# DeepNeuralAI313/Arabic-text-image-generation-RepText

Measured on AMD Instinct MI355X. Metric: images/sec (whole node), FLUX.1-dev+RepText CN, 1024^2, 28 steps, higher is better.
Workload: dtype bf16; 1 GPU; FLUX.1-dev (19+38 blocks) + RepText ControlNet (6+0), 1024x1024, 28 steps, 1 text line(s), batch 1/GPU on rank 0, denoise loop + VAE decode to uint8, random-init weights; tower blocks evaluated 5 of 6 (the last sample is never read, Q5); global_batch=1, conditioning=one prompt, hint and mask per image, parallelism=batch-shard x1, one broadcast

## Files before the change

### arabic-text-image-generation-reptext_amd/controlnet.py

```python
from __future__ import annotations

from dataclasses import dataclass
from typing import Any, Dict, List, Optional, Sequence, Tuple, Union

import torch
import torch.nn as nn

from . import mmdit, ops
from .config import Config
from .modules import Lin
from .ops import LinearProblem as P
from .transformer import StaticEmbeds, _MMDiTBase


@dataclass
class FluxControlNetOutput:
    controlnet_block_samples: Optional[List[torch.Tensor]]
    controlnet_single_block_samples: Optional[List[torch.Tensor]]

    def __iter__(self):
        yield self.controlnet_block_samples
        yield self.controlnet_single_block_samples


class FluxControlNetModel(_MMDiTBase):
    _supports_gradient_checkpointing = False

    def __init__(self, patch_size: int = 1, in_channels: int = 64, num_layers: int = 19, num_single_layers: int = 38,
                 attention_head_dim: int = 128, num_attention_heads: int = 24, joint_attention_dim: int = 4096,
                 pooled_projection_dim: int = 768, guidance_embeds: bool = False, axes_dims_rope=(16, 56, 56),
                 num_mode: Optional[int] = None, extra_conditioning_channels: int = 0, extra_condition_channels: int = 0,
                 device=None, dtype=None):
        super().__init__()
        self.config = Config(patch_size=patch_size, in_channels=in_channels, num_layers=num_layers,
                             num_single_layers=num_single_layers, attention_head_dim=attention_head_dim,
                             num_attention_heads=num_attention_heads, joint_attention_dim=joint_attention_dim,
                             pooled_projection_dim=pooled_projection_dim, guidance_embeds=guidance_embeds,
                             axes_dims_rope=list(axes_dims_rope), num_mode=num_mode,
                             extra_conditioning_channels=extra_conditioning_channels,
                             extra_condition_channels=extra_condition_channels)
        self.out_channels = in_channels
        self._build_trunk(self.config, device, dtype)
        d = self.inner_dim
        kw = dict(device=device, dtype=dtype)
        self.controlnet_blocks = nn.ModuleList([Lin(d, d, **kw) for _ in range(num_layers)])
        self.controlnet_single_blocks = nn.ModuleList([Lin(d, d, **kw) for _ in range(num_single_layers)])
        self.union = num_mode is not None
        if self.union:
            self.controlnet_mode_embedder = nn.Embedding(num_mode, d, **kw)
        self.controlnet_x_embedder = Lin(in_channels + extra_condition_channels, d, **kw)
        self.gradient_checkpointing = False

    def zero_init_controlnet_(self):
        for m in list(self.controlnet_blocks) + list(self.controlnet_single_blocks) + [self.controlnet_x_embedder]:
            m.weight.data.zero_()
            m.bias.data.zero_()
        return self

    @property
    def attn_processors(self) -> Dict[str, Any]:
        names = [f"transformer_blocks.{i}.attn.processor" for i in range(len(self.transformer_blocks))]
        names += [f"single_transformer_blocks.{i}.attn.processor" for i in range(len(self.single_transformer_blocks))]
        return {n: "HipFlashAttention" for n in names}

    def set_attn_processor(self, processor):
        count = len(self.attn_processors)
        if isinstance(processor, dict) and len(processor) != count:
            raise ValueError(
                f"A dict of processors was passed, but the number of processors {len(processor)} does not match the"
                f" number of attention layers: {count}. Please make sure to pass {count} processor classes.")
        raise NotImplementedError("the MI355X path has a single fused attention kernel; custom processors are not supported")

    @classmethod
    def from_transformer(cls, transformer, num_layers: int = 4, num_single_layers: int = 10, attention_head_dim: int = 128,
                         num_attention_heads: int = 24, extra_condition_channels: int = 0,
                         load_weights_from_transformer: bool = True):
        cfg = dict(transformer.config)
        cfg.pop("out_channels", None)
        cfg.update(num_layers=num_layers, num_single_layers=num_single_layers, attention_head_dim=attention_head_dim,
                   num_attention_heads=num_attention_heads, extra_condition_channels=extra_condition_channels)
        cn = cls(**cfg, device=transformer.device, dtype=transformer.dtype)
        if load_weights_from_transformer:
            src = transformer.state_dict()
            own = cn.state_dict()
            for k in own:
                if k in src and own[k].shape == src[k].shape:
                    own[k].copy_(src[k])
        cn.zero_init_controlnet_()
        return cn

    def _padded_hint(self, cond: torch.Tensor):
        cxw = self.controlnet_x_embedder.weight.data
        kin = cxw.shape[1]
        if kin % 64 == 0:
            return cond, cxw
        kp = (kin + 63) // 64 * 64
        if getattr(self, "_cx_pad", None) is None or self._cx_pad.device != cxw.device:
            wpad = torch.zeros(cxw.shape[0], kp, device=cxw.device, dtype=cxw.dtype)
            wpad[:, :kin] = cxw
            self._cx_pad = wpad
        return torch.nn.functional.pad(cond, (0, kp - kin)), self._cx_pad

    def _lora_unsupported(self, path: str, lin):
        why = super()._lora_unsupported(path, lin)
        if why is None and lin is self.controlnet_x_embedder and lin.in_features % 64:
            why = f"in-features {lin.in_features} are not a multiple of 64: the K-padded copy of _padded_hint would go stale"
        return why

    def _invalidate_derived(self):
        self._cx_pad = None

    def load_state_dict(self, sd, strict: bool = True, **kw):
        out = super().load_state_dict(sd, strict=strict, **kw)
        self._invalidate_derived()
        return out

    def random_init_(self, *a, **k):
        out = super().random_init_(*a, **k)
        self._invalidate_derived()
        return out

    def _apply(self, fn, *a, **k):
        self._invalidate_derived()
        return super()._apply(fn, *a, **k)

    @torch.no_grad()
    def forward(self, hidden_states: torch.Tensor, controlnet_cond: torch.Tensor, controlnet_mode: torch.Tensor = None,
                conditioning_scale: float = 1.0, encoder_hidden_states: torch.Tensor = None,
                pooled_projections: torch.Tensor = None, timestep: torch.Tensor = None, img_ids: torch.Tensor = None,
                txt_ids: torch.Tensor = None, guidance: torch.Tensor = None,
                joint_attention_kwargs: Optional[Dict[str, Any]] = None, return_dict: bool = True,
                _rowscale: Optional[torch.Tensor] = None, _accumulate_into: Optional[Sequence[torch.Tensor]] = None,
                _accumulate_single_into: Optional[Sequence[torch.Tensor]] = None, _mods: Optional["mmdit.StepMods"] = None,
                _overwrite: bool = False, _sample_events: Optional[Sequence["torch.cuda.Event"]] = None, _ws_tag: str = "",
                _static: Optional[StaticEmbeds] = None, _blocks_needed: Optional[Tuple[int, int]] = None):
        doubles, singles = self._ensure_plans()
        self._apply_lora_scale(joint_attention_kwargs)
        cfg = self.config
        if self.union:
            if controlnet_mode is None:
                raise ValueError("`controlnet_mode` cannot be `None` when applying ControlNet-Union")
            raise NotImplementedError("ControlNet-Union mode embedding is outside the RepText hot path (SURVEY.md §2 #11)")
        B, N, _ = hidden_states.shape
        Bc, T, _ = encoder_hidden_states.shape
        H, d = cfg.num_attention_heads, self.inner_dim
        ws = mmdit.workspace(Bc, T, N, d, hidden_states.device, need_single=len(singles) > 0, tag=_ws_tag)
        hs = hidden_states.to(torch.bfloat16)
        if hs.shape[0] != Bc:
            hs = hs.expand(Bc, -1, -1) if hs.shape[0] == 1 else hs.repeat(Bc // hs.shape[0], 1, 1)
        x_i, x_t = ws.x[:, T:], ws.x[:, :T]
        if _static is not None:
            x_t.copy_(_static.ctx)
            ops.linear(hs.contiguous(), self.x_embedder.weight.data, x_i, bias=self.x_embedder.bias.data, res=_static.hint)
        else:
            cond = controlnet_cond.to(torch.bfloat16)
            if cond.shape[0] != Bc:
                cond = cond.expand(Bc, -1, -1) if cond.shape[0] == 1 else cond.repeat(Bc // cond.shape[0], 1, 1)
            ops.linear_grouped([P(hs.contiguous(), self.x_embedder.weight.data, x_i, bias=self.x_embedder.bias.data),
                                P(encoder_hidden_states.to(torch.bfloat16).contiguous(), self.context_embedder.weight.data, x_t,
                                  bias=self.context_embedder.bias.data)])
            cond, cxw = self._padded_hint(cond)
            ops.linear(cond.contiguous(), cxw, x_i, bias=self.controlnet_x_embedder.bias.data, res=x_i)
        temb = None if _mods is not None else self._temb(ws, timestep, guidance, pooled_projections)
        cos, sin = self._rope(txt_ids, img_ids)

        scale = float(conditioning_scale)

        def head(lin, dst_list, i):
            a = mmdit.image_rows_bf16(ws)
            if dst_list is not None:
                out = dst_list[i]
                ops.linear(a, lin.weight.data, out, bias=lin.bias.data, alpha=scale, rowscale=_rowscale, res=None if _overwrite else out)
            else:
                out = torch.empty(Bc, N, d, device=hs.device, dtype=torch.bfloat16)
                ops.linear(a, lin.weight.data, out, bias=lin.bias.data, alpha=scale, rowscale=_rowscale)
            return out

        nd = len(doubles) if _blocks_needed is None else min(len(doubles), int(_blocks_needed[0]))
        ns = len(singles) if _blocks_needed is None else min(len(singles), int(_blocks_needed[1]))
        if ns > 0:
            nd = len(doubles)
        block_samples: List[Optional[torch.Tensor]] = []
        for i, pl in enumerate(doubles):
            if i >= nd:
                block_samples.append(None)
                continue
            mmdit.run_double(pl, ws, temb, cos, sin, H, mods=None if _mods is None else _mods.double[i])
            block_samples.append(head(self.controlnet_blocks[i], _accumulate_into, i))
            if _sample_events is not None:
                _sample_events[i].record(torch.cuda.current_stream())
        single_samples: List[Optional[torch.Tensor]] = []
        for i, pl in enumerate(singles):
            if i >= ns:
                single_samples.append(None)
                continue
            mmdit.run_single(pl, ws, temb, cos, sin, H, mods=None if _mods is None else _mods.single[i])
            single_samples.append(head(self.controlnet_single_blocks[i], _accumulate_single_into, i))

        bs = block_samples if block_samples else None
        ss = single_samples if single_samples else None
        if not return_dict:
            return (bs, ss)
        return FluxControlNetOutput(controlnet_block_samples=bs, controlnet_single_block_samples=ss)


class FluxMultiControlNetModel(nn.Module):

    def __init__(self, controlnets, union: bool = False):
        super().__init__()
        self.nets = nn.ModuleList(controlnets)
        self.union = union

    @torch.no_grad()
    def forward(self, hidden_states, controlnet_cond, controlnet_mode, conditioning_scale, encoder_hidden_states=None,
                pooled_projections=None, timestep=None, img_ids=None, txt_ids=None, guidance=None,
                joint_attention_kwargs=None, return_dict: bool = True):
        nets = [self.nets[0]] * len(controlnet_cond) if len(self.nets) == 1 else list(self.nets)
        total_b = total_s = None
        for net, image, mode, scale in zip(nets, controlnet_cond, controlnet_mode, conditioning_scale):
            b, s = net(hidden_states=hidden_states, controlnet_cond=image, controlnet_mode=None if mode is None else mode[:, None],
                       conditioning_scale=scale, timestep=timestep, guidance=guidance, pooled_projections=pooled_projections,
                       encoder_hidden_states=encoder_hidden_states, txt_ids=txt_ids, img_ids=img_ids,
                       joint_attention_kwargs=joint_attention_kwargs, return_dict=False)
            if total_b is None and total_s is None:
                total_b, total_s = b, s
                continue
            if b is not None and total_b is not None:
                for acc, t in zip(total_b, b):
                    ops.masked_accumulate_(acc, t, None, 1.0, True)
            if s is not None and total_s is not None:
                for acc, t in zip(total_s, s):
                    ops.masked_accumulate_(acc, t, None, 1.0, True)
        return total_b, total_s
```

### arabic-text-image-generation-reptext_amd/csrc/attention.hip

```cpp
#include "attention_split.h"
#include <cstdlib>
#include <type_traits>

namespace {

constexpr int DH = 128;
constexpr int BQ = 128;
constexpr int BKV = 64;
constexpr int TILE_B = BKV * DH * 2;
constexpr int ATT_THREADS = 256;
constexpr float RESCALE_THR = 6.0f;
constexpr int REC_WAVE_B = 64 * 64 * 4 + 64 * 8;
constexpr int REC_B = 4 * REC_WAVE_B;

__host__ __device__ inline int group_slots(const SplitGeom& G, int xcd) {
  const GroupCut c = group_cut(G, xcd);
  return c.nfull + (c.rem ? G.spx : 0);
}

__global__ __launch_bounds__(ATT_THREADS, 2) void attention_fwd_kernel(
    const bf16_t* __restrict__ Q, const bf16_t* __restrict__ K, const bf16_t* __restrict__ V, bf16_t* O,
    int64_t ld, int64_t stride_b, int64_t ldo, int64_t stride_ob, float scale_log2, const SplitGeom G,
    int* counters, char* records) {
  __shared__ __attribute__((aligned(16))) char smem[4 * TILE_B];
  const int tid = threadIdx.x;
  const int lane = tid & 63;
  const int wave = __builtin_amdgcn_readfirstlane(tid >> 6);
  const int l31 = lane & 31, hh = lane >> 5;
  const int S = G.S;
  const int ntiles = G.ntiles;

  const int xcd = (int)blockIdx.x & 7, slot = (int)blockIdx.x >> 3, b = (int)blockIdx.y;
  const GroupCut cut = group_cut(G, xcd);
  int run_lo, run_hi;
  int item0;
  int jpart = -1;
  if (slot < cut.nfull) {
    item0 = cut.start + slot;
    run_lo = 0;
    run_hi = ntiles;
  } else {
    jpart = slot - cut.nfull;
    if (cut.rem == 0 || jpart >= G.spx) return;
    const SplitRun run = split_run(G, cut, jpart);
    item0 = cut.start + cut.nfull + run.i0;
    run_lo = run.lo - run.i0 * ntiles;
    run_hi = run.hi - run.i0 * ntiles;
  }

  const int srow = lane >> 4;
  const int spc = lane & 15;
  uint32_t soff[4];
#pragma unroll
  for (int p = 0; p < 4; ++p) {
    const int row_t = (wave * 4 + p) * 4 + srow;
    soff[p] = ((uint32_t)row_t * (uint32_t)ld + (uint32_t)((spc ^ swz(row_t)) << 3)) * 2u;
  }
  lds_cptr kp[8];
  {
    const int ksw = swz(l31);
#pragma unroll
    for (int ks = 0; ks < 8; ++ks) kp[ks] = (lds_cptr)smem + (l31 * 256 + (((2 * ks + hh) ^ ksw) << 4));
  }
  const int tq = (lane >> 2) & 3, tp = lane & 3;
  const int tg1 = (lane >> 4) & 1;
  lds_cptr vp[2][4];
  {
    const int cl = tg1 * 2 + (tp >> 1);
    const int rl0 = 4 * hh + tq, rl1 = rl0 + 8;
#pragma unroll
    for (int dt = 0; dt < 4; ++dt) {
      vp[0][dt] = (lds_cptr)smem + TILE_B + rl0 * 256 + (((dt * 4 + cl) ^ swz(rl0)) << 4) + 8 * (tp & 1);
      vp[1][dt] = (lds_cptr)smem + TILE_B + rl1 * 256 + (((dt * 4 + cl) ^ swz(rl1)) << 4) + 8 * (tp & 1);
    }
  }

  using S0 = std::integral_constant<int, 0>;
  using S1 = std::integral_constant<int, 1>;

  for (int seg = 0; seg < 2; ++seg) {
    const int item = item0 + seg;
    const int tb = seg == 0 ? run_lo : 0;
    const int te = seg == 0 ? min(run_hi, ntiles) : run_hi - ntiles;
    if (te <= tb) break;
    const int head = item / G.nqb;
    const int q0 = (item - head * G.nqb) * BQ;
    const bf16_t* Qb = Q + b * stride_b + head * DH;
    const bf16_t* Kb = K + b * stride_b + head * DH;
    const bf16_t* Vb = V + b * stride_b + head * DH;

    const rt_srd_t rsrcK = rt_make_srd(Kb), rsrcV = rt_make_srd(Vb);
    const uint32_t lds0 = (uint32_t)(uintptr_t)LDS_PTR(smem);
    const int tile_stride_b = BKV * (int)ld * 2;
    auto stage = [&](int sl, int tix, bool clamp) {
      const uint32_t kb = lds0 + sl * 2 * TILE_B;
      if (RT_RARE(clamp)) {
        const int kv0 = tix * BKV;
#pragma unroll
        for (int p = 0; p < 4; ++p) {
          const int row_t = (wave * 4 + p) * 4 + srow;
          const uint32_t off = ((uint32_t)(min(kv0 + row_t, S - 1) - kv0) * (uint32_t)ld + (uint32_t)((spc ^ swz(row_t)) << 3)) * 2u;
          rt_dma16_asm(rsrcK, kb + (wave * 4 + p) * 1024, off, (uint32_t)(tix * tile_stride_b));
          rt_dma16_asm(rsrcV, kb + TILE_B + (wave * 4 + p) * 1024, off, (uint32_t)(tix * tile_stride_b));
        }
      } else {
#pragma unroll
        for (int p = 0; p < 4; ++p) {
          rt_dma16_asm(rsrcK, kb + (wave * 4 + p) * 1024, soff[p], (uint32_t)(tix * tile_stride_b));
          rt_dma16_asm(rsrcV, kb + TILE_B + (wave * 4 + p) * 1024, soff[p], (uint32_t)(tix * tile_stride_b));
        }
      }
    };

    __syncthreads();
    stage(0, tb, (tb + 1) * BKV > S);

    bf16x8 qf[8];
    {
      const int qrow = min(q0 + wave * 32 + l31, S - 1);
      const bf16_t* qp = Qb + (int64_t)qrow * ld + 8 * hh;
#pragma unroll
      for (int ks = 0; ks < 8; ++ks) qf[ks] = *reinterpret_cast<const bf16x8*>(qp + ks * 16);
#pragma unroll
      for (int ks = 0; ks < 8; ++ks) asm volatile("" : "+v"(qf[ks]));
    }

    f32x16 o_acc[4];
#pragma unroll
    for (int i = 0; i < 4; ++i)
#pragma unroll
      for (int r = 0; r < 16; ++r) o_acc[i][r] = 0.f;
    float m_run = -INFINITY, l_run = 0.f;

    auto half_max = [&](const f32x16& s) -> float {
      float ma = max3f(s[0], s[1], s[2]), mb = max3f(s[3], s[4], s[5]);
      ma = max3f(ma, s[6], s[7]);
      mb = max3f(mb, s[8], s[9]);
      ma = max3f(ma, s[10], s[11]);
      mb = max3f(mb, s[12], s[13]);
      return fmaxf(max3f(ma, s[14], s[15]), mb);
    };
    auto decide = [&](float mx, bool& pend) -> float {
      unsigned xa = __builtin_bit_cast(unsigned, mx), xb = xa;
      asm volatile("s_nop 1\n\tv_permlane32_swap_b32 %0, %1" : "+v"(xa), "+v"(xb));
      const float mxr = fmaxf(__builtin_bit_cast(float, xa), __builtin_bit_cast(float, xb)) * scale_log2;
      float alpha = 1.f;
      pend = false;
      if (RT_RARE(__any(mxr - m_run > RESCALE_THR))) {
        asm volatile("" ::: "memory");
        const float m_new = fmaxf(m_run, mxr);
        alpha = __builtin_amdgcn_exp2f(m_run - m_new);
        m_run = m_new;
        l_run *= alpha;
        pend = true;
      }
      return alpha;
    };
    auto rescale_o = [&](float alpha) __attribute__((always_inline)) {
#pragma unroll
      for (int i = 0; i < 4; ++i)
#pragma unroll
        for (int r = 0; r < 16; ++r) o_acc[i][r] *= alpha;
    };
    auto numer8 = [&](const f32x16& s, int s2, bf16x8& pf) {
      float ps = 0.f;
#pragma unroll
      for (int j = 0; j < 8; ++j) {
        const float p = __builtin_amdgcn_exp2f(__builtin_fmaf(s[8 * s2 + j], scale_log2, -m_run));
        ps += p;
        pf[j] = (__bf16)p;
      }
      l_run += ps;
    };

#define RT_WEAVE(n, nds, nva)                                          \
  _Pragma("unroll") for (int w_ = 0; w_ < (n); ++w_) {                 \
    __builtin_amdgcn_sched_group_barrier(0x008, 1, 0);                 \
    if ((nds) > 0) __builtin_amdgcn_sched_group_barrier(0x100, (nds), 0); \
    if ((nva) > 0) __builtin_amdgcn_sched_group_barrier(0x402, (nva), 0); \
  }

    auto tile = [&](auto slot_c, int t) {
      constexpr int SLOT = decltype(slot_c)::value;
      constexpr int SB = SLOT * 2 * TILE_B;
      const bool ragged = (t + 1) * BKV > S;
      auto kread = [&](int h, int ks) -> bf16x8 {
        return *(const __attribute__((address_space(3))) bf16x8*)(kp[ks] + SB + h * 8192); };
      auto vread = [&](int h, int s2, int dt) -> bf16x8 {
        const s16x4 lo = tr_read(vp[0][dt] + SB + h * 8192 + s2 * 4096);
        const s16x4 hi = tr_read(vp[1][dt] + SB + h * 8192 + s2 * 4096);
        return __builtin_shufflevector(__builtin_bit_cast(bf16x4, lo), __builtin_bit_cast(bf16x4, hi), 0, 1, 2, 3, 4, 5, 6, 7);
      };
      auto mask_half = [&](f32x16& s, int h) {
#pragma unroll
        for (int r = 0; r < 16; ++r)
          if (t * BKV + 32 * h + (r & 3) + 8 * (r >> 2) + 4 * hh >= S) s[r] = -INFINITY;
      };
      rt_dma_barrier();
      f32x16 s0, s1;
#pragma unroll
      for (int r = 0; r < 16; ++r) { s0[r] = 0.f; s1[r] = 0.f; }
      bf16x8 kA[8], kB[8], vA[4], vB[4];
      bf16x8 p00, p01, p10, p11;
      bool pend;
#pragma unroll
      for (int ks = 0; ks < 8; ++ks) kA[ks] = kread(0, ks);
      const bool next_ragged = (t + 2) * BKV > S;
      if (RT_RARE(t + 1 < te && next_ragged)) stage(SLOT ^ 1, t + 1, true);
      const bool weave = t + 1 < te && !next_ragged;
      {
        const uint32_t nb = lds0 + (SLOT ^ 1) * 2 * TILE_B, so = (uint32_t)((t + 1) * tile_stride_b);
#pragma unroll
        for (int ks = 0; ks < 8; ++ks) {
          s0 = __builtin_amdgcn_mfma_f32_32x32x16_bf16(kA[ks], qf[ks], s0, 0, 0, 0);
          if (RT_USUAL(weave)) rt_dma16_asm((ks & 1) ? rsrcV : rsrcK, nb + ((ks & 1) ? TILE_B : 0) + (wave * 4 + (ks >> 1)) * 1024, soff[ks >> 1], so);
          if (ks >= 4 && ks < 7) kB[ks - 4] = kread(1, ks - 4);
          RT_SB();
        }
      }
#pragma unroll
      for (int ks = 0; ks < 3; ++ks) s1 = __builtin_amdgcn_mfma_f32_32x32x16_bf16(kB[ks], qf[ks], s1, 0, 0, 0);
#pragma unroll
      for (int ks = 3; ks < 8; ++ks) kB[ks] = kread(1, ks);
      if (RT_RARE(ragged)) mask_half(s0, 0);
      float mx0 = half_max(s0);
      __builtin_amdgcn_sched_group_barrier(0x008, 1, 0);
      __builtin_amdgcn_sched_group_barrier(0x100, 3, 0);
      __builtin_amdgcn_sched_group_barrier(0x008, 1, 0);
      __builtin_amdgcn_sched_group_barrier(0x100, 2, 0);
      __builtin_amdgcn_sched_group_barrier(0x008, 1, 0);
      RT_SB();
      {
        const float alpha = decide(mx0, pend);
        if (RT_RARE(pend)) rescale_o(alpha);
      }
      RT_SB();
#pragma unroll
      for (int ks = 3; ks < 8; ++ks) s1 = __builtin_amdgcn_mfma_f32_32x32x16_bf16(kB[ks], qf[ks], s1, 0, 0, 0);
#pragma unroll
      for (int dt = 0; dt < 4; ++dt) vA[dt] = vread(0, 0, dt);
      numer8(s0, 0, p00);
      RT_WEAVE(5, 2, 6)
      RT_PIN(p00); RT_PIN(l_run);
      RT_SB();
#pragma unroll
      for (int dt = 0; dt < 4; ++dt) o_acc[dt] = __builtin_amdgcn_mfma_f32_32x32x16_bf16(vA[dt], p00, o_acc[dt], 0, 0, 0);
#pragma unroll
      for (int dt = 0; dt < 4; ++dt) vB[dt] = vread(0, 1, dt);
      numer8(s0, 1, p01);
      if (RT_RARE(ragged)) mask_half(s1, 1);
      float mx1 = half_max(s1);
      RT_WEAVE(4, 2, 9)
      RT_PIN(p01); RT_PIN(l_run); RT_PIN(mx1);
      RT_SB();
      const float alpha1 = decide(mx1, pend);
      RT_SB();
#pragma unroll
      for (int dt = 0; dt < 4; ++dt) o_acc[dt] = __builtin_amdgcn_mfma_f32_32x32x16_bf16(vB[dt], p01, o_acc[dt], 0, 0, 0);
#pragma unroll
      for (int dt = 0; dt < 4; ++dt) vA[dt] = vread(1, 0, dt);
      numer8(s1, 0, p10);
      RT_WEAVE(4, 2, 7)
      RT_PIN(p10); RT_PIN(l_run);
      RT_SB();
      if (RT_RARE(pend)) rescale_o(alpha1);
      RT_SB();
#pragma unroll
      for (int dt = 0; dt < 4; ++dt) o_acc[dt] = __builtin_amdgcn_mfma_f32_32x32x16_bf16(vA[dt], p10, o_acc[dt], 0, 0, 0);
#pragma unroll
      for (int dt = 0; dt < 4; ++dt) vB[dt] = vread(1, 1, dt);
      numer8(s1, 1, p11);
      RT_WEAVE(4, 2, 7)
      RT_PIN(p11); RT_PIN(l_run);
      RT_SB();
#pragma unroll
      for (int dt = 0; dt < 4; ++dt) o_acc[dt] = __builtin_amdgcn_mfma_f32_32x32x16_bf16(vB[dt], p11, o_acc[dt], 0, 0, 0);
    };

    int t = tb;
    for (; t + 1 < te; t += 2) {
      tile(S0{}, t);
      tile(S1{}, t + 1);
    }
    if (t < te) tile(S0{}, t);

    const int qrow = q0 + wave * 32 + l31;
    const bool whole = (tb == 0 && te == ntiles);
    if (!whole) {
      const int ritem = item - (cut.start + cut.nfull);
      char* rec = records + split_rec_index(G, b, xcd, jpart, seg) * (int64_t)REC_B + wave * REC_WAVE_B;
      const __amdgpu_buffer_rsrc_t rs = __builtin_amdgcn_make_buffer_rsrc(rec, 0, REC_WAVE_B, 0x00020000);
#pragma unroll
      for (int i = 0; i < 4; ++i)
#pragma unroll
        for (int g = 0; g < 4; ++g) {
          const f32x4 vv = {o_acc[i][4 * g + 0], o_acc[i][4 * g + 1], o_acc[i][4 * g + 2], o_acc[i][4 * g + 3]};
          const u32x4 w = __builtin_bit_cast(u32x4, vv);
          __builtin_amdgcn_raw_buffer_store_b128(w, rs, (i * 4 + g) * 1024 + lane * 16, 0, 16 );
        }
      {
        const float2 mlf = {m_run, l_run};
        const u32x2 ml = __builtin_bit_cast(u32x2, mlf);
        __builtin_amdgcn_raw_buffer_store_b64(ml, rs, 16384 + lane * 8, 0, 16);
      }
      int* cnt = counters + (int64_t)b * G.NI + item;
      const SplitParts parts = split_parts(G, cut, ritem);
      const bool last = split_ticket(cnt, parts.nparts, reinterpret_cast<volatile int*>(smem), tid);
      if (last) {
        auto rec_of = [&](int j) -> const char* {
          return records + split_rec_index(G, b, xcd, j, split_seg_of(G, parts, j)) * (int64_t)REC_B + wave * REC_WAVE_B;
        };
        float M = -INFINITY;
        for (int j = parts.j_first; j <= parts.j_last; ++j) {
          const char* rj = rec_of(__builtin_amdgcn_readfirstlane(j));
          M = fmaxf(M, *reinterpret_cast<const float*>(rj + 16384 + lane * 8));
        }
        float L = 0.f;
#pragma unroll
        for (int i = 0; i < 4; ++i)
#pragma unroll
          for (int r = 0; r < 16; ++r) o_acc[i][r] = 0.f;
        for (int j = parts.j_first; j <= parts.j_last; ++j) {
          const char* rj = rec_of(__builtin_amdgcn_readfirstlane(j));
          const float2 ml = *reinterpret_cast<const float2*>(rj + 16384 + lane * 8);
          const float wgt = __builtin_amdgcn_exp2f(ml.x - M);
          L = __builtin_fmaf(ml.y, wgt, L);
#pragma unroll
          for (int i = 0; i < 4; ++i)
#pragma unroll
            for (int g = 0; g < 4; ++g) {
              const f32x4 v = *reinterpret_cast<const f32x4*>(rj + (i * 4 + g) * 1024 + lane * 16);
#pragma unroll
              for (int e = 0; e < 4; ++e) o_acc[i][4 * g + e] = __builtin_fmaf(v[e], wgt, o_acc[i][4 * g + e]);
            }
        }
        l_run = L;
      }
      if (!last) continue;
    }

    const float l_tot = l_run + __shfl_xor(l_run, 32);
    const float inv = 1.0f / l_tot;
    const bool wide = (ldo % 8 == 0) && (stride_ob % 8 == 0) && ((reinterpret_cast<uintptr_t>(O) & 15) == 0);
    if (wide) {
      rt_store_o_rows(O + b * stride_ob + (int64_t)min(qrow, S - 1) * ldo + head * DH, qrow < S, hh, o_acc, inv);
    } else if (qrow < S) {
      bf16_t* op = O + b * stride_ob + (int64_t)qrow * ldo + head * DH + 4 * hh;
#pragma unroll
      for (int dt = 0; dt < 4; ++dt)
#pragma unroll
        for (int g = 0; g < 4; ++g) {
          u32x2 w;
          w[0] = pack_bf16x2(o_acc[dt][4 * g + 0] * inv, o_acc[dt][4 * g + 1] * inv);
          w[1] = pack_bf16x2(o_acc[dt][4 * g + 2] * inv, o_acc[dt][4 * g + 3] * inv);
          *reinterpret_cast<u32x2*>(op + dt * 32 + 8 * g) = w;
        }
    }
  }
}

int g_slots_per_xcd = 0;

int slots_per_xcd() {
  if (g_slots_per_xcd == 0) {
    const char* e = getenv("RT_ATTN_SLOTS_PER_XCD");
    g_slots_per_xcd = e ? atoi(e) : (split_cu_count() / 8) * 2;
    if (g_slots_per_xcd < 1) g_slots_per_xcd = 1;
  }
  return g_slots_per_xcd;
}

SplitGeom make_geom(int S, int H, bool want_split) { return split_geom(S, H, BQ, BKV, slots_per_xcd(), want_split); }

}

extern "C" int64_t rt_attention_ws_bytes(int32_t B, int32_t S, int32_t H) {
  if (B < 1 || S < 1 || H < 1) return 0;
  static const bool off = getenv("RT_ATTN_SPLIT") && getenv("RT_ATTN_SPLIT")[0] == '0';
  if (off) return 0;
  const int64_t need3 = rt_attention_v3_ws_bytes(B, S, H);
  const int64_t need = split_ws_bytes(B, make_geom(S, H, true), REC_B);
  return need > need3 ? need : need3;
}

extern "C" int rt_attention_variant(int32_t mode) { return rt_attention_v3_mode(mode); }

extern "C" int rt_attention_fwd(const void* q, const void* k, const void* v, void* o, int64_t ld, int64_t stride_b,
                                int64_t ldo, int64_t stride_ob, int32_t B, int32_t S, int32_t H, float scale,
                                void* ws, int64_t ws_bytes, void* stream) {
  if (!q || !k || !v || !o || B < 1 || S < 1 || H < 1) return RT_E_BADARG;
  if (!RT_ALIGNED(q, 16) || !RT_ALIGNED(k, 16) || !RT_ALIGNED(v, 16) || !RT_ALIGNED(o, 8) || ld % 8 || stride_b % 8 ||
      ldo % 4 || stride_ob % 4)
    return RT_E_ALIGN;
  if (ld < (int64_t)H * DH || ldo < (int64_t)H * DH) return RT_E_SHAPE;
  if ((int64_t)(S + BKV) * ld * 2 >= (int64_t)1 << 31) return RT_E_SHAPE;
  if (!split_fits_32bit(make_geom(S, H, true))) return RT_E_SHAPE;
  {
    int taken = 0;
    const int st = rt_attention_v3_try(q, k, v, o, ld, stride_b, ldo, stride_ob, B, S, H, scale, ws, ws_bytes, stream, &taken);
    if (taken || st != RT_OK) return st;
  }
  const int64_t need = rt_attention_ws_bytes(B, S, H);
  const bool split = ws != nullptr && need > 0;
  if (split && (ws_bytes < need || !RT_ALIGNED(ws, 256))) return RT_E_BADARG;
  const SplitGeom G = make_geom(S, H, split);
  int wmax = 0;
  for (int x = 0; x < 8; ++x) wmax = group_slots(G, x) > wmax ? group_slots(G, x) : wmax;
  const dim3 grid(8 * wmax, B);
  hipLaunchKernelGGL(attention_fwd_kernel, grid, dim3(ATT_THREADS), 0, (hipStream_t)stream, (const bf16_t*)q,
                     (const bf16_t*)k, (const bf16_t*)v, (bf16_t*)o, ld, stride_b, ldo, stride_ob,
                     scale * 1.4426950408889634f, G, split ? (int*)ws : nullptr,
                     split ? (char*)ws + split_cnt_bytes(B, S, H) : nullptr);
  return rt_hip_status();
}
```

### arabic-text-image-generation-reptext_amd/csrc/attention_split.h

```cpp
#pragma once
#include "rt_common.h"

constexpr int CNT_ALIGN = 256;
constexpr int SPLIT_MIN_TILES = 8;

struct SplitGeom {
  int S, H, nqb, ntiles, NI;
  int spx;
  int split;
};

struct GroupCut {
  int start, cnt;
  int nfull;
  int rem;
};
__host__ __device__ inline GroupCut group_cut(const SplitGeom& G, int xcd) {
  GroupCut c;
  const int base = G.NI >> 3, extra = G.NI & 7;
  c.cnt = base + (xcd < extra ? 1 : 0);
  c.start = xcd * base + (xcd < extra ? xcd : extra);
  c.nfull = c.cnt;
  c.rem = 0;
  if (G.split) {
    const int nf = (c.cnt / G.spx) * G.spx, rem = c.cnt - nf;
    if (rem > 0 && rem * 16 < G.spx * 15 && (int64_t)rem * G.ntiles >= (int64_t)G.spx * SPLIT_MIN_TILES) {
      c.nfull = nf;
      c.rem = rem;
    }
  }
  return c;
}

struct SplitRun { int lo, hi, i0; };
__device__ __forceinline__ SplitRun split_run(const SplitGeom& G, const GroupCut& cut, int j) {
  const unsigned U = (unsigned)cut.rem * (unsigned)G.ntiles;
  SplitRun r;
  r.lo = (int)((unsigned)j * U / (unsigned)G.spx);
  r.hi = (int)((unsigned)(j + 1) * U / (unsigned)G.spx);
  r.i0 = r.lo / G.ntiles;
  return r;
}

struct SplitParts {
  unsigned U, a;
  int j_first, j_last, nparts;
};
__device__ __forceinline__ SplitParts split_parts(const SplitGeom& G, const GroupCut& cut, int ritem) {
  const unsigned U = (unsigned)cut.rem * (unsigned)G.ntiles, spx = (unsigned)G.spx;
  const unsigned a = (unsigned)ritem * (unsigned)G.ntiles, bnd = a + (unsigned)G.ntiles;
  SplitParts p;
  p.U = U;
  p.a = a;
  p.j_first = (int)(((a + 1) * spx + U - 1) / U) - 1;
  p.j_last = min(G.spx - 1, (int)((bnd * spx + U - 1) / U) - 1);
  p.nparts = p.j_last - p.j_first + 1;
  return p;
}
__device__ __forceinline__ int split_seg_of(const SplitGeom& G, const SplitParts& p, int j) {
  const unsigned lo_j = (unsigned)j * p.U / (unsigned)G.spx;
  return (p.a > lo_j) ? 1 : 0;
}
__device__ __forceinline__ int64_t split_rec_index(const SplitGeom& G, int b, int xcd, int j, int seg) {
  return (((int64_t)b * 8 + xcd) * G.spx + j) * 2 + seg;
}

__device__ __forceinline__ bool split_ticket(int* cnt, int nparts, volatile int* flag, int tid) {
  asm volatile("s_waitcnt vmcnt(0)" ::: "memory");
  __syncthreads();
  if (tid == 0) {
    const int old = __hip_atomic_fetch_add(cnt, 1, __ATOMIC_RELAXED, __HIP_MEMORY_SCOPE_AGENT);
    const int last = (old == nparts - 1) ? 1 : 0;
    if (last) {
      __hip_atomic_store(cnt, 0, __ATOMIC_RELAXED, __HIP_MEMORY_SCOPE_AGENT);
      __builtin_amdgcn_fence(__ATOMIC_ACQUIRE, "agent");
      asm volatile("s_waitcnt vmcnt(0)" ::: "memory");
    }
    *flag = last;
  }
  __syncthreads();
  return __builtin_amdgcn_readfirstlane(*flag) != 0;
}

inline int split_cu_count() {
  int dev = 0, cus = 256;
  if (hipGetDevice(&dev) == hipSuccess) {
    int v = 0;
    if (hipDeviceGetAttribute(&v, hipDeviceAttributeMultiprocessorCount, dev) == hipSuccess && v > 0) cus = v;
  }
  return cus;
}
inline SplitGeom split_geom(int S, int H, int bq, int bkv, int spx, bool split) {
  const int nqb = (S + bq - 1) / bq;
  return SplitGeom{S, H, nqb, (S + bkv - 1) / bkv, H * nqb, spx > 0 ? spx : 1, split ? 1 : 0};
}
inline bool split_fits_32bit(const SplitGeom& G) { return (int64_t)G.NI * (G.ntiles + 1) * G.spx < ((int64_t)1 << 31); }
inline bool split_any(const SplitGeom& G) {
  bool any = false;
  for (int x = 0; x < 8; ++x) any = any || group_cut(G, x).rem > 0;
  return any;
}
inline int64_t split_cnt_bytes(int B, int S, int H) {
  return (((int64_t)B * H * ((S + 127) / 128) * 4 + CNT_ALIGN - 1) / CNT_ALIGN) * CNT_ALIGN;
}
inline int64_t split_ws_bytes(int B, const SplitGeom& G, int64_t rec_bytes) {
  if (!split_any(G)) return 0;
  return split_cnt_bytes(B, G.S, G.H) + (int64_t)B * 8 * G.spx * 2 * rec_bytes;
}

int64_t rt_attention_v3_ws_bytes(int32_t B, int32_t S, int32_t H);
int rt_attention_v3_try(const void* q, const void* k, const void* v, void* o, int64_t ld, int64_t stride_b, int64_t ldo, int64_t stride_ob,
                        int32_t B, int32_t S, int32_t H, float scale, void* ws, int64_t ws_bytes, void* stream, int* taken);
int rt_attention_v3_mode(int mode);
```

### arabic-text-image-generation-reptext_amd/csrc/attention_v3.hip

```cpp
#include "attention_split.h"
#include <cstdlib>
#include <type_traits>

namespace {

constexpr int DH = 128;
constexpr int BQ3 = 256;
constexpr int BKV = 64;
constexpr int TILE_B = BKV * DH * 2;
constexpr int STAGE_B = 2 * TILE_B;
constexpr int NSTAGE = 3;
constexpr int V3_THREADS = 256;
constexpr float RESCALE_THR = 6.0f;

#include "attention_v3_regs.h"
#define V3_EACH8(M) M(0) M(1) M(2) M(3) M(4) M(5) M(6) M(7)
#define V3_EACH10(M) V3_EACH8(M) M(8) M(9)
#define V3_EACH16(M) M(0) M(1) M(2) M(3) M(4) M(5) M(6) M(7) M(8) M(9) M(10) M(11) M(12) M(13) M(14) M(15)
__device__ __forceinline__ void mfma_o(int f, const bf16x8& v, const bf16x8& p) {
  switch (f) {
#define V3_C(F) case F: asm volatile("v_mfma_f32_32x32x16_bf16 " V3_OREG_##F ", %0, %1, " V3_OREG_##F ::"v"(v), "v"(p) : V3_ALL_CL); break;
    V3_EACH8(V3_C)
#undef V3_C
  }
}
__device__ __forceinline__ void mfma_l(int qb, const bf16x8& p) {
  if (qb) asm volatile("v_mfma_f32_32x32x16_bf16 " V3_OREG_9 ", " V3_ONES_REG ", %0, " V3_OREG_9 ::"v"(p) : V3_ALL_CL);
  else asm volatile("v_mfma_f32_32x32x16_bf16 " V3_OREG_8 ", " V3_ONES_REG ", %0, " V3_OREG_8 ::"v"(p) : V3_ALL_CL);
}
__device__ __forceinline__ void ones_write() {
  asm volatile("v_accvgpr_write_b32 a224, %0\n\tv_accvgpr_write_b32 a225, %0\n\tv_accvgpr_write_b32 a226, %0\n\tv_accvgpr_write_b32 a227, %0" ::"v"(0x3F803F80u) : V3_ALL_CL);
}
__device__ __forceinline__ void mfma_s0(f32x16& c, const bf16x8& k, int i) {
  switch (i) {
#define V3_C(I) case I: asm volatile("v_mfma_f32_32x32x16_bf16 %0, %1, " V3_QREG_##I ", 0" : "=&v"(c) : "v"(k) : V3_ALL_CL); break;
    V3_EACH16(V3_C)
#undef V3_C
  }
}
__device__ __forceinline__ void mfma_s(f32x16& c, const bf16x8& k, int i) {
  switch (i) {
#define V3_C(I) case I: asm volatile("v_mfma_f32_32x32x16_bf16 %0, %1, " V3_QREG_##I ", %0" : "+v"(c) : "v"(k) : V3_ALL_CL); break;
    V3_EACH16(V3_C)
#undef V3_C
  }
}
__device__ __forceinline__ void q_write(int i, const bf16x8& q) {
  const u32x4 w = __builtin_bit_cast(u32x4, q);
  switch (i) {
#define V3_C(I) case I: asm volatile(V3_QWRITE_##I ::"v"(w[0]), "v"(w[1]), "v"(w[2]), "v"(w[3]) : V3_ALL_CL); break;
    V3_EACH16(V3_C)
#undef V3_C
  }
}
__device__ __forceinline__ void o_zero(int f) {
  switch (f) {
#define V3_C(F) case F: asm volatile(V3_OZERO_##F ::: V3_ALL_CL); break;
    V3_EACH10(V3_C)
#undef V3_C
  }
}
__device__ __forceinline__ void o_scale(int f, float alpha) {
  float tmp;
  switch (f) {
#define V3_C(F) case F: asm volatile(V3_OSCALE_##F : "=&v"(tmp) : "v"(alpha) : V3_ALL_CL); break;
    V3_EACH10(V3_C)
#undef V3_C
  }
}
__device__ __forceinline__ f32x16 o_read(int f) {
  float x0, x1, x2, x3, x4, x5, x6, x7, x8, x9, x10, x11, x12, x13, x14, x15;
  switch (f) {
#define V3_C(F) case F: asm volatile(V3_OREAD_##F : "=v"(x0), "=v"(x1), "=v"(x2), "=v"(x3), "=v"(x4), "=v"(x5), "=v"(x6), "=v"(x7), "=v"(x8), "=v"(x9), "=v"(x10), "=v"(x11), "=v"(x12), "=v"(x13), "=v"(x14), "=v"(x15) : : V3_ALL_CL); break;
    V3_EACH10(V3_C)
#undef V3_C
  }
  return f32x16{x0, x1, x2, x3, x4, x5, x6, x7, x8, x9, x10, x11, x12, x13, x14, x15};
}

constexpr int REC3_WAVE_B = 8 * 16 * 64 * 4 + 64 * 16;
constexpr int REC3_B = 4 * REC3_WAVE_B;

__global__ __launch_bounds__(V3_THREADS, 1) void attention_v3_kernel(const bf16_t* __restrict__ Q, const bf16_t* __restrict__ K,
                                                                     const bf16_t* __restrict__ V, bf16_t* O, int64_t ld, int64_t stride_b,
                                                                     int64_t ldo, int64_t stride_ob, float scale_log2, const SplitGeom G,
                                                                     int* counters, char* records) {
  extern __shared__ __attribute__((aligned(16))) char smem[];
  const int tid = threadIdx.x;
  const int lane = tid & 63;
  const int wave = __builtin_amdgcn_readfirstlane(tid >> 6);
  const int l31 = lane & 31, hh = lane >> 5;
  const int ntiles = G.ntiles;
  const int xcd = (int)blockIdx.x & 7, slot = (int)blockIdx.x >> 3, b = (int)blockIdx.y;
  const GroupCut cut = group_cut(G, xcd);
  const uint32_t lds0 = (uint32_t)(uintptr_t)LDS_PTR(smem);

  const int srow = lane >> 4, spc = lane & 15;
  uint32_t soff[4];
#pragma unroll
  for (int p = 0; p < 4; ++p) {
    const int row_t = (wave * 4 + p) * 4 + srow;
    soff[p] = ((uint32_t)row_t * (uint32_t)ld + (uint32_t)((spc ^ swz(row_t)) << 3)) * 2u;
  }
  const int tile_stride_b = BKV * (int)ld * 2;

  const int nwhole = slot < cut.nfull ? (cut.nfull - slot + G.spx - 1) / G.spx : 0;
  SplitRun run = {0, 0, 0};
  if (cut.rem && slot < G.spx) run = split_run(G, cut, slot);
  const int nseg = nwhole + (cut.rem && slot < G.spx ? 2 : 0);

  for (int si = 0; si < nseg; ++si) {
    int item, tb, te, seg = 0;
    if (si < nwhole) {
      item = cut.start + slot + si * G.spx;
      tb = 0;
      te = ntiles;
    } else {
      seg = si - nwhole;
      item = cut.start + cut.nfull + run.i0 + seg;
      tb = seg == 0 ? run.lo - run.i0 * ntiles : 0;
      te = seg == 0 ? min(run.hi - run.i0 * ntiles, ntiles) : run.hi - (run.i0 + 1) * ntiles;
      if (te <= tb) continue;
    }
    const int head = item / G.nqb;
    const int q0 = (item - head * G.nqb) * BQ3;
    const bf16_t* Qb = Q + b * stride_b + head * DH;
    const rt_srd_t rsrcK = rt_make_srd(K + b * stride_b + head * DH), rsrcV = rt_make_srd(V + b * stride_b + head * DH);
    const uint32_t wdst = lds0 + wave * 4096;
    auto dma_piece = [&](int sbase, uint32_t soffs, int i) __attribute__((always_inline)) {
      rt_dma16_asm((i & 4) ? rsrcV : rsrcK, wdst + sbase + ((i & 4) ? TILE_B : 0) + (i & 3) * 1024, soff[i & 3], soffs);
    };

    asm volatile("s_waitcnt vmcnt(0)" ::: "memory");
    __syncthreads();
#pragma unroll
    for (int i = 0; i < 8; ++i) dma_piece(0, (uint32_t)(tb * tile_stride_b), i);
    if (tb + 1 < te) {
#pragma unroll
      for (int i = 0; i < 8; ++i) dma_piece(STAGE_B, (uint32_t)((tb + 1) * tile_stride_b), i);
    }
    {
      const bf16_t* qp = Qb + (int64_t)(q0 + wave * 64 + l31) * ld + 8 * hh;
      bf16x8 qa[8], qb[8];
#pragma unroll
      for (int ks = 0; ks < 8; ++ks) {
        qa[ks] = *reinterpret_cast<const bf16x8*>(qp + ks * 16);
        qb[ks] = *reinterpret_cast<const bf16x8*>(qp + 32 * ld + ks * 16);
      }
#pragma unroll
      for (int ks = 0; ks < 8; ++ks) { q_write(ks, qa[ks]); q_write(8 + ks, qb[ks]); }
#pragma unroll
      for (int f = 0; f < 10; ++f) o_zero(f);
      ones_write();
      asm volatile("s_nop 7" ::: "memory");
    }
    float mA = -INFINITY, mB = -INFINITY;

    f32x16 sAa, sAb, sBa, sBb;
    bf16x8 pA[2][2], pB[2][2];
    bf16x8 kf[8], vf[8];
    float mxa0, mxa1, mxb0, mxb1;
    float tf[2], pp[2];
    int pend1 = -1, pend2 = -1;

    auto elem_f = [&](int o, const f32x16& Sa, const f32x16& Sb) __attribute__((always_inline)) {
      const int ks = o >> 4, qb = (o >> 3) & 1, j = o & 7, r = 8 * ks + j;
      float t = __builtin_fmaf(qb ? Sb[r] : Sa[r], scale_log2, qb ? -mB : -mA);
      asm volatile("" : "+v"(t));
      tf[o & 1] = t;
    };
    auto elem_x = [&](int o) __attribute__((always_inline)) {
      float p = __builtin_amdgcn_exp2f(tf[o & 1]);
      asm volatile("" : "+v"(p));
      pp[o & 1] = p;
    };
    auto elem_c = [&](int o, bf16x8 (&P)[2][2]) __attribute__((always_inline)) {
      const int ks = o >> 4, qb = (o >> 3) & 1, j = o & 7;
      P[qb][ks][j] = (__bf16)pp[o & 1];
      if (j & 1) asm volatile("" : "+v"(P[qb][ks]));
    };
    auto elem = [&](int o, const f32x16& Sa, const f32x16& Sb, bf16x8 (&P)[2][2]) __attribute__((always_inline)) {
      if (pend2 >= 0) elem_c(pend2, P);
      if (pend1 >= 0) elem_x(pend1);
      elem_f(o, Sa, Sb);
      pend2 = pend1;
      pend1 = o;
    };
    auto elem_flush = [&](bf16x8 (&P)[2][2]) __attribute__((always_inline)) {
      if (pend2 >= 0) elem_c(pend2, P);
      if (pend1 >= 0) { elem_x(pend1); elem_c(pend1, P); }
      pend1 = pend2 = -1;
    };
    auto maxstep = [&](int k, const f32x16& s, float& m0, float& m1) __attribute__((always_inline)) {
      if (k == 0) m0 = max3f(s[0], s[1], s[2]);
      else if (k == 1) m1 = max3f(s[3], s[4], s[5]);
      else if (k == 2) m0 = max3f(m0, s[6], s[7]);
      else if (k == 3) m1 = max3f(m1, s[8], s[9]);
      else if (k == 4) m0 = max3f(m0, s[10], s[11]);
      else if (k == 5) m1 = max3f(m1, s[12], s[13]);
      else if (k == 6) m0 = max3f(m0, s[14], s[15]);
      else m0 = fmaxf(m0, m1);
    };
    auto exchange = [&](float mx) __attribute__((always_inline)) -> float {
      unsigned xa = __builtin_bit_cast(unsigned, mx), xb = xa;
      asm volatile("s_nop 1\n\tv_permlane32_swap_b32 %0, %1" : "+v"(xa), "+v"(xb));
      return fmaxf(__builtin_bit_cast(float, xa), __builtin_bit_cast(float, xb)) * scale_log2;
    };
    auto decide = [&](float mxra, float mxrb, const f32x16& Sa, const f32x16& Sb, bf16x8 (&P)[2][2]) __attribute__((always_inline)) {
      if (__builtin_expect(!!__any((mxra - mA > RESCALE_THR) | (mxrb - mB > RESCALE_THR)), 0)) {
        asm volatile("s_nop 15\n\ts_nop 15" ::: "memory");
        const float nA = fmaxf(mA, mxra), nB = fmaxf(mB, mxrb);
        const float alA = __builtin_amdgcn_exp2f(mA - nA), alB = __builtin_amdgcn_exp2f(mB - nB);
        mA = nA; mB = nB;
#pragma unroll
        for (int f = 0; f < 10; ++f) o_scale(f, (f & 1) ? alB : alA);
#pragma unroll
        for (int o = 0; o < 16; ++o) { elem_f(o, Sa, Sb); elem_x(o); elem_c(o, P); }
      }
    };
    int ka[8];
    {
      const int ksw = swz(l31);
  #pragma unroll
      for (int ks = 0; ks < 8; ++ks) ka[ks] = (int)lds0 + l31 * 256 + (((2 * ks + hh) ^ ksw) << 4);
    }
    const int tq = (lane >> 2) & 3, tp = lane & 3, tg1 = (lane >> 4) & 1;
    int va[8];
    {
      const int cl = tg1 * 2 + (tp >> 1);
      const int rl0 = 4 * hh + tq, rl1 = rl0 + 8;
  #pragma unroll
      for (int dt = 0; dt < 4; ++dt) {
        va[dt] = (int)lds0 + TILE_B + rl0 * 256 + (((dt * 4 + cl) ^ swz(rl0)) << 4) + 8 * (tp & 1);
        va[4 + dt] = (int)lds0 + TILE_B + rl1 * 256 + (((dt * 4 + cl) ^ swz(rl1)) << 4) + 8 * (tp & 1);
      }
    }
    auto mov_ka = [&](int i, int delta) __attribute__((always_inline)) { ka[i] += delta; asm volatile("" : "+v"(ka[i])); };
    auto mov_va = [&](int i, int delta) __attribute__((always_inline)) { va[i] += delta; asm volatile("" : "+v"(va[i])); };
    auto kread = [&](int kb, int ks) __attribute__((always_inline)) -> bf16x8 {
      return *(const __attribute__((address_space(3))) bf16x8*)((lds_cptr)(uintptr_t)(uint32_t)(ka[ks] + kb * 8192));
    };
    auto vread = [&](int kb, int s2, int dt) __attribute__((always_inline)) -> bf16x8 {
      const s16x4 lo = tr_read((lds_cptr)(uintptr_t)(uint32_t)(va[dt] + kb * 8192 + s2 * 4096));
      const s16x4 hi = tr_read((lds_cptr)(uintptr_t)(uint32_t)(va[4 + dt] + kb * 8192 + s2 * 4096));
      return __builtin_shufflevector(__builtin_bit_cast(bf16x4, lo), __builtin_bit_cast(bf16x4, hi), 0, 1, 2, 3, 4, 5, 6, 7);
    };
    auto qk_group = [&](f32x16& Sa, f32x16& Sb, auto&& filler) __attribute__((always_inline)) {
      asm volatile("" ::"v"(kf[0]), "v"(kf[1]), "v"(kf[2]), "v"(kf[3]), "v"(kf[4]), "v"(kf[5]), "v"(kf[6]), "v"(kf[7]));
#pragma unroll
      for (int g = 0; g < 16; ++g) {
        const int ks = g >> 1;
        if (g == 0) mfma_s0(Sa, kf[0], 0);
        else if (g == 1) mfma_s0(Sb, kf[0], 8);
        else if (g & 1) mfma_s(Sb, kf[ks], 8 + ks);
        else mfma_s(Sa, kf[ks], ks);
        filler(g);
        RT_SB();
      }
    };
    auto pv_group = [&](bf16x8 (&P)[2][2], auto&& filler) __attribute__((always_inline)) {
      asm volatile("" ::"v"(vf[0]), "v"(vf[1]), "v"(vf[2]), "v"(vf[3]), "v"(vf[4]), "v"(vf[5]), "v"(vf[6]), "v"(vf[7]));
#pragma unroll
      for (int g = 0; g < 20; ++g) {
        const int s2 = g / 10, h = g % 10;
        if (h < 8) mfma_o((h >> 1) * 2 + (h & 1), vf[s2 * 4 + (h >> 1)], P[h & 1][s2]);
        else mfma_l(h & 1, P[h & 1][s2]);
        filler(g);
        RT_SB();
      }
    };
    auto second_half = [&](int g, const f32x16& Sa, const f32x16& Sb, bf16x8 (&P)[2][2], float ra, float rb, float& ea, float& eb)
        __attribute__((always_inline)) {
      if (g == 0) ea = exchange(ra);
      if (g == 1) eb = exchange(rb);
      if (g == 2) decide(ea, eb, Sa, Sb, P);
      if (g >= 3 && g <= 12) elem(13 + g, Sa, Sb, P);
      if (g >= 13) { elem(26 + 2 * (g - 13), Sa, Sb, P); elem(27 + 2 * (g - 13), Sa, Sb, P); }
      if (g == 15) elem_flush(P);
// ... 29 lines not shown
        asm volatile("s_nop 15\n\ts_nop 15" ::: "memory");
        RT_PIN(sAa); RT_PIN(sAb);
#pragma unroll
        for (int g = 0; g < 8; ++g) { maxstep(g, sAa, mxa0, mxa1); maxstep(g, sAb, mxb0, mxb1); }
#pragma unroll
        for (int ks = 0; ks < 8; ++ks) kf[ks] = kread(1, ks);
      }
      rka = mxa0; rkb = mxb0;
      RT_SB();
      qk_group(sBa, sBb, [&](int g) __attribute__((always_inline)) {
        if constexpr (first) {
          if (g == 0) ea = exchange(rka);
          if (g == 1) { eb = exchange(rkb); mA = fmaxf(mA, ea); mB = fmaxf(mB, eb); }
          if (g >= 2) { elem(2 * (g - 2), sAa, sAb, pA); elem(2 * (g - 2) + 1, sAa, sAb, pA); }
          if (g == 14) { elem(28, sAa, sAb, pA); elem(29, sAa, sAb, pA); }
          if (g == 15) { elem(30, sAa, sAb, pA); elem(31, sAa, sAb, pA); elem_flush(pA); }
        } else {
          second_half(g, sAa, sAb, pA, rka, rkb, ea, eb);
        }
        if ((g & 1) == 0) { const int i = g >> 1; vf[(i >> 2) * 4 + (i & 3)] = vread(0, i >> 2, i & 3); } else { mov_ka(g >> 1, sbn - sb); }
      });
      if constexpr (!last) {
        asm volatile("s_waitcnt vmcnt(0)" ::: "memory");
        __builtin_amdgcn_s_barrier();
        RT_SB();
      }
      pv_group(pA, [&](int g) __attribute__((always_inline)) {
        first_half(g, sBa, sBb, pB);
        if constexpr (!last) {
          if (g < 16 && (g & 1)) kf[g >> 1] = kread(0, g >> 1);
          if (g >= 2 && g < 18 && (g & 1) == 0) dma_piece(sbp, so2, (g - 2) >> 1);
        }
      });
      { const int r_ = st_cur; st_cur = st_nxt; st_nxt = st_prv; st_prv = r_; }
      rka = mxa0; rkb = mxb0;
      if constexpr (last) {
        RT_SB();
        const float ea2 = exchange(rka), eb2 = exchange(rkb);
        decide(ea2, eb2, sBa, sBb, pB);
#pragma unroll
        for (int o = 16; o < 32; ++o) elem(o, sBa, sBb, pB);
        elem_flush(pB);
#pragma unroll
        for (int i = 0; i < 8; ++i) vf[(i >> 2) * 4 + (i & 3)] = vread(1, i >> 2, i & 3);
        RT_SB();
        pv_group(pB, [&](int) __attribute__((always_inline)) {});
      }
    };
    using TT = std::true_type;
    using FF = std::false_type;
    __syncthreads();
#pragma unroll
    for (int ks = 0; ks < 8; ++ks) kf[ks] = kread(0, ks);
    if (te - tb == 1) {
      tile(TT{}, TT{}, tb);
    } else {
      tile(TT{}, FF{}, tb);
      for (int t = tb + 1; t + 1 < te; ++t) tile(FF{}, FF{}, t);
      tile(FF{}, TT{}, te - 1);
    }

    asm volatile("s_nop 15\n\ts_nop 15" ::: "memory");
    const bool whole = (tb == 0 && te == ntiles);
    const float lA = o_read(8)[0], lB = o_read(9)[0];
    bf16_t* orow = O + b * stride_ob + (int64_t)(q0 + wave * 64 + l31) * ldo + head * DH;
    if (whole) {
#pragma unroll
      for (int qb = 0; qb < 2; ++qb) {
        f32x16 t4[4];
#pragma unroll
        for (int dt = 0; dt < 4; ++dt) t4[dt] = o_read(dt * 2 + qb);
        rt_store_o_rows(orow + qb * 32 * ldo, true, hh, t4, 1.0f / (qb ? lB : lA));
      }
      continue;
    }
    const int jpart = slot;
    const int ritem = item - (cut.start + cut.nfull);
    {
      char* rec = records + split_rec_index(G, b, xcd, jpart, seg) * (int64_t)REC3_B + wave * REC3_WAVE_B;
      const __amdgpu_buffer_rsrc_t rs = __builtin_amdgcn_make_buffer_rsrc(rec, 0, REC3_WAVE_B, 0x00020000);
#pragma unroll
      for (int f = 0; f < 8; ++f) {
        const f32x16 x = o_read(f);
#pragma unroll
        for (int g = 0; g < 4; ++g) {
          const f32x4 vv = {x[4 * g + 0], x[4 * g + 1], x[4 * g + 2], x[4 * g + 3]};
          __builtin_amdgcn_raw_buffer_store_b128(__builtin_bit_cast(u32x4, vv), rs, (f * 4 + g) * 1024 + lane * 16, 0, 16 );
        }
      }
      const f32x4 ml = {mA, lA, mB, lB};
      __builtin_amdgcn_raw_buffer_store_b128(__builtin_bit_cast(u32x4, ml), rs, 32768 + lane * 16, 0, 16);
    }
    int* cnt = counters + (int64_t)b * G.NI + item;
    const SplitParts parts = split_parts(G, cut, ritem);
    if (!split_ticket(cnt, parts.nparts, reinterpret_cast<volatile int*>(smem), tid)) continue;
    auto rec_of = [&](int j) -> const char* {
      return records + split_rec_index(G, b, xcd, j, split_seg_of(G, parts, j)) * (int64_t)REC3_B + wave * REC3_WAVE_B;
    };
    float MA = -INFINITY, MB = -INFINITY;
    for (int j = parts.j_first; j <= parts.j_last; ++j) {
      const f32x4 ml = *reinterpret_cast<const f32x4*>(rec_of(__builtin_amdgcn_readfirstlane(j)) + 32768 + lane * 16);
      MA = fmaxf(MA, ml[0]);
      MB = fmaxf(MB, ml[2]);
    }
    float LA = 0.f, LB = 0.f;
    for (int j = parts.j_first; j <= parts.j_last; ++j) {
      const f32x4 ml = *reinterpret_cast<const f32x4*>(rec_of(__builtin_amdgcn_readfirstlane(j)) + 32768 + lane * 16);
      LA = __builtin_fmaf(ml[1], __builtin_amdgcn_exp2f(ml[0] - MA), LA);
      LB = __builtin_fmaf(ml[3], __builtin_amdgcn_exp2f(ml[2] - MB), LB);
    }
#pragma unroll
    for (int qb = 0; qb < 2; ++qb) {
      f32x16 t4[4];
#pragma unroll
      for (int dt = 0; dt < 4; ++dt)
#pragma unroll
        for (int r = 0; r < 16; ++r) t4[dt][r] = 0.f;
      for (int j = parts.j_first; j <= parts.j_last; ++j) {
        const char* rj = rec_of(__builtin_amdgcn_readfirstlane(j));
        const f32x4 ml = *reinterpret_cast<const f32x4*>(rj + 32768 + lane * 16);
        const float w = __builtin_amdgcn_exp2f(qb ? ml[2] - MB : ml[0] - MA);
#pragma unroll
        for (int dt = 0; dt < 4; ++dt)
#pragma unroll
          for (int g = 0; g < 4; ++g) {
            const f32x4 v = *reinterpret_cast<const f32x4*>(rj + ((dt * 2 + qb) * 4 + g) * 1024 + lane * 16);
#pragma unroll
            for (int e = 0; e < 4; ++e) t4[dt][4 * g + e] = __builtin_fmaf(v[e], w, t4[dt][4 * g + e]);
          }
      }
      rt_store_o_rows(orow + qb * 32 * ldo, true, hh, t4, 1.0f / (qb ? LB : LA));
    }
  }
}

int g_v3_mode = -1;
int v3_mode_now() {
  if (g_v3_mode < 0) {
    const char* e = getenv("RT_ATTN_V3");
    g_v3_mode = e ? atoi(e) : 1;
  }
  return g_v3_mode;
}
SplitGeom v3_geom(int S, int H, bool split) { return split_geom(S, H, BQ3, BKV, split_cu_count() / 8, split); }

}

int64_t rt_attention_v3_ws_bytes(int32_t B, int32_t S, int32_t H) {
  if (S % BQ3 != 0) return 0;
  return split_ws_bytes(B, v3_geom(S, H, true), REC3_B);
}

int rt_attention_v3_try(const void* q, const void* k, const void* v, void* o, int64_t ld, int64_t stride_b, int64_t ldo, int64_t stride_ob,
                        int32_t B, int32_t S, int32_t H, float scale, void* ws, int64_t ws_bytes, void* stream, int* taken) {
  *taken = 0;
  if (!v3_mode_now() || S % BQ3 != 0 || (ldo % 8) || (stride_ob % 8) || !RT_ALIGNED(o, 16)) return RT_OK;
  if (v3_mode_now() == 1 && S < 1536) return RT_OK;
  const int64_t need = rt_attention_v3_ws_bytes(B, S, H);
  const bool split = ws != nullptr && need > 0 && ws_bytes >= need && RT_ALIGNED(ws, 256);
  const SplitGeom G = v3_geom(S, H, split);
  if (!split_fits_32bit(G)) return RT_OK;
  *taken = 1;
  const int lds = NSTAGE * STAGE_B;
  static bool attr_done = false;
  if (!attr_done) {
    hipError_t e = hipFuncSetAttribute(reinterpret_cast<const void*>(attention_v3_kernel), hipFuncAttributeMaxDynamicSharedMemorySize, lds);
    if (e != hipSuccess) return (int)e;
    attr_done = true;
  }
  int slots = 0;
  for (int x = 0; x < 8; ++x) {
    const GroupCut c = group_cut(G, x);
    const int s = c.rem ? G.spx : (c.nfull < G.spx ? c.nfull : G.spx);
    slots = s > slots ? s : slots;
  }
  hipLaunchKernelGGL(attention_v3_kernel, dim3(8 * slots, B), dim3(V3_THREADS), lds, (hipStream_t)stream, (const bf16_t*)q, (const bf16_t*)k,
                     (const bf16_t*)v, (bf16_t*)o, ld, stride_b, ldo, stride_ob, scale * 1.4426950408889634f, G, split ? (int*)ws : nullptr,
                     split ? (char*)ws + split_cnt_bytes(B, S, H) : nullptr);
  return rt_hip_status();
}

int rt_attention_v3_mode(int mode) {
  const int prev = v3_mode_now();
  if (mode >= 0) g_v3_mode = mode;
  return prev;
}
```

### arabic-text-image-generation-reptext_amd/mmdit.py

```python
from __future__ import annotations

from dataclasses import dataclass
from typing import List, Optional

import torch

from . import native, ops
from .ops import LinearProblem as P

import os

BF16, F32 = torch.bfloat16, torch.float32
RESIDUAL_F32 = os.environ.get("RT_RESIDUAL_F32", "1") == "1"

FUSED_QK_ROPE = os.environ.get("RT_FUSED_QK_ROPE", "1") == "1"

REF_BF16_SCALARS = False


def reference_bf16_scalars(on: bool = True) -> None:
    global REF_BF16_SCALARS
    REF_BF16_SCALARS = bool(on)


# ... 134 lines not shown
        self.x = e(B, S, d, dt=F32 if RESIDUAL_F32 else BF16)
        self.xn = e(B, S, d)
        self.qkv = e(B, S, 3 * d)
        self.ffh = e(B, S, 4 * d)
        self.big = e(B, S, 7 * d) if need_single else None
        self.mod_a = e(B, 6 * d, dt=F32)
        self.mod_b = e(B, 6 * d, dt=F32)
        self.temb = e(B, d, dt=F32)
        self.tmp = e(B, d, dt=F32)
        self._device = device
        self.xn8 = None
        self.xs_t = self.xs_i = self.xs_all = None

    def ip_buffer(self) -> torch.Tensor:
        if getattr(self, "_ip", None) is None:
            self._ip = torch.empty(self.B, self.N, self.d, device=self._device, dtype=BF16)
        return self._ip

    def ip_buffer_joint(self) -> torch.Tensor:
        if getattr(self, "_ip_s", None) is None:
            self._ip_s = torch.empty(self.B, self.S, self.d, device=self._device, dtype=BF16)
        return self._ip_s

    def fp8_buffers(self):
        if self.xn8 is None:
            B, T, N, S, d = self.B, self.T, self.N, self.S, self.d
            self.xn8 = torch.empty(B, S, d, device=self._device, dtype=ops.FP8)
            self.xs_t = torch.empty(B * T, device=self._device, dtype=F32)
            self.xs_i = torch.empty(B * N, device=self._device, dtype=F32)
            self.xs_all = torch.empty(B * S, device=self._device, dtype=F32)
        return self.xn8

    def fp8_attn_buffers(self, H: int):
        if getattr(self, "_qk8", None) is None:
            self._qk8 = torch.empty(self.B, self.S, 2 * H * 128, device=self._device, dtype=ops.FP8)
            self._vt8 = torch.empty(int(native.load().rt_attention_fp8_vt_bytes(self.B, self.S, H)), device=self._device, dtype=ops.FP8)
        return self._qk8, self._vt8

    def fp8_wide(self, width: int) -> torch.Tensor:
        if getattr(self, "_a8", None) is None or self._a8.shape[2] < width:
            self._a8 = torch.empty(self.B, self.S, max(width, 5 * self.d), device=self._device, dtype=ops.FP8)
        return self._a8[:, :, :width]


    def mx_scales(self) -> "ops.BlockScales":
        if getattr(self, "_a8s", None) is None:
            self._a8s = ops.BlockScales.empty(self.B, self.S, 5 * self.d, self._device)
        return self._a8s


_WS_CACHE = {}
CAPTURE_KEEP: Optional[list] = None


def workspace(B, T, N, d, device, need_single, tag: str = "") -> Workspace:
    key = (B, T, N, d, str(device), RESIDUAL_F32, tag)
    ws = _WS_CACHE.get(key)
    if ws is None or (need_single and ws.big is None):
        if len(_WS_CACHE) > 6:
            _WS_CACHE.clear()
        ws = Workspace(B, T, N, d, device, need_single)
        _WS_CACHE[key] = ws
    if CAPTURE_KEEP is not None:
        CAPTURE_KEEP.append(ws)
    return ws


def time_text_embed(tte, ws: Workspace, t1000: torch.Tensor, g1000: Optional[torch.Tensor], pooled: torch.Tensor) -> torch.Tensor:
    def mlp(m, x_f32, accumulate):
        ops.gemv(x_f32, m.linear_1.weight.data, m.linear_1.bias.data, ws.tmp, silu_out=True)
        ops.gemv(ws.tmp, m.linear_2.weight.data, m.linear_2.bias.data, ws.temb, accumulate=accumulate)

    mlp(tte.timestep_embedder, ops.timestep_embedding(t1000, 256), False)
    if g1000 is not None:
        mlp(tte.guidance_embedder, ops.timestep_embedding(g1000, 256), True)
    pooled_f32 = pooled if pooled.dtype == F32 else ops.to_f32(pooled)
    mlp(tte.text_embedder, pooled_f32.contiguous(), True)
    return ws.temb


def time_text_embed_all(tte, t1000_all: torch.Tensor, g1000: Optional[torch.Tensor], pooled: torch.Tensor, B: int) -> torch.Tensor:
    dev = pooled.device
    d = tte.timestep_embedder.linear_2.weight.shape[0]

    def mlp(m, x_f32):
        h = torch.empty(x_f32.shape[0], m.linear_1.weight.shape[0], device=dev, dtype=F32)
        y = torch.empty(x_f32.shape[0], d, device=dev, dtype=F32)
        ops.gemv(x_f32, m.linear_1.weight.data, m.linear_1.bias.data, h, silu_out=True)
        ops.gemv(h, m.linear_2.weight.data, m.linear_2.bias.data, y)
        return y

    temb_all = mlp(tte.timestep_embedder, ops.timestep_embedding(t1000_all, 256))
    pooled_f32 = pooled if pooled.dtype == F32 else ops.to_f32(pooled)
    p = mlp(tte.text_embedder, pooled_f32.contiguous())
    if g1000 is not None:
        ops.add_rows_(temb_all, mlp(tte.guidance_embedder, ops.timestep_embedding(g1000, 256)), p)
    else:
        ops.add_rows_(temb_all, p)
    return temb_all


@dataclass
class StepMods:

    double: List[tuple]
    single: List[torch.Tensor]
    out: Optional[torch.Tensor]


class ModulationTable:

    def __init__(self, temb_all: torch.Tensor, n_steps: int, B: int, doubles, singles, out_lin=None):
        self.n, self.B = n_steps, B
        hi, lo = ops.silu_split(temb_all, apply_silu=True)
        dev = temb_all.device
        M = temb_all.shape[0]

        def out_buf(w):
            return torch.empty(M, w.shape[0], device=dev, dtype=F32)

        self.double, self.single, self.out = [], [], None
        skinny = M <= 32 and temb_all.shape[1] % 256 == 0 and all(w.shape[0] % 16 == 0 for w in self._widths(doubles, singles, out_lin))

        def table(problems):
            if skinny:
                ops.linear_skinny(hi, lo, problems)
            else:
                ops.linear_grouped([P(hi, w, o, bias=b) for w, b, o in problems])
                ops.linear_grouped([P(lo, w, o, res=o) for w, b, o in problems])

        for pl in doubles:
            oi, ot = out_buf(pl.ada_img_w), out_buf(pl.ada_txt_w)
            table([(pl.ada_img_w, pl.ada_img_b, oi), (pl.ada_txt_w, pl.ada_txt_b, ot)])
            self.double.append((oi, ot))
        for pl in singles:
            o = out_buf(pl.ada_w)
            table([(pl.ada_w, pl.ada_b, o)])
            self.single.append(o)
        if out_lin is not None:
            o = out_buf(out_lin.weight.data)
            table([(out_lin.weight.data, out_lin.bias.data, o)])
            self.out = o

    @staticmethod
    def _widths(doubles, singles, out_lin):
        return [w for pl in doubles for w in (pl.ada_img_w, pl.ada_txt_w)] + [pl.ada_w for pl in singles] + ([out_lin.weight.data] if out_lin is not None else [])

    def step(self, i: int) -> StepMods:
        r = slice(i * self.B, (i + 1) * self.B)
        return StepMods([(a[r], b[r]) for a, b in self.double], [s[r] for s in self.single], None if self.out is None else self.out[r])


def run_double(pl: DoublePlan, ws: Workspace, temb: torch.Tensor, cos, sin, H: int, inject: Optional[torch.Tensor] = None,
               mods: Optional[tuple] = None, ip: Optional[tuple] = None, ip_inside: bool = False) -> None:
    T, d = ws.T, ws.d
    x_t, x_i = ws.x[:, :T], ws.x[:, T:]
    xn_t, xn_i = ws.xn[:, :T], ws.xn[:, T:]
    if mods is not None:
        mi, mt = mods
    else:
        mi, mt = ws.mod_a, ws.mod_b
        ops.gemv(temb, pl.ada_img_w, pl.ada_img_b, mi, silu_in=True)
        ops.gemv(temb, pl.ada_txt_w, pl.ada_txt_b, mt, silu_in=True)
    ch = lambda m, i: m[:, i * d : (i + 1) * d]
    fp8 = pl.qkv_img_w8 is not None
    fused_rope = False
    if fp8:
        xn8 = ws.fp8_buffers()
        xn8_t, xn8_i = xn8[:, :T], xn8[:, T:]
    if fp8:
        ops.layernorm_modulate_fp8(x_i, xn8_i, ws.xs_i, ch(mi, 0), ch(mi, 1))
        ops.layernorm_modulate_fp8(x_t, xn8_t, ws.xs_t, ch(mt, 0), ch(mt, 1))
        ops.linear_grouped([P(xn8_i, pl.qkv_img_w8, ws.qkv[:, T:], bias=pl.qkv_img_b, a_scale=ws.xs_i, w_scale=pl.qkv_img_ws),
                            P(xn8_t, pl.qkv_txt_w8, ws.qkv[:, :T], bias=pl.qkv_txt_b, a_scale=ws.xs_t, w_scale=pl.qkv_txt_ws)])
    else:
        ops.layernorm_modulate_pair(x_i, xn_i, ch(mi, 0), ch(mi, 1), x_t, xn_t, ch(mt, 0), ch(mt, 1))
        fused_rope = FUSED_QK_ROPE and ip is None and not pl.fp8_attention and ops.QKRope.covers(d)
        ri = ops.QKRope(0, d, d, pl.nq_img, pl.nk_img, cos, sin, pos0=T) if fused_rope else None
        rt = ops.QKRope(0, d, d, pl.nq_txt, pl.nk_txt, cos, sin, pos0=0) if fused_rope else None
        ops.linear_grouped([P(xn_i, pl.qkv_img_w, ws.qkv[:, T:], bias=pl.qkv_img_b, rope=ri), P(xn_t, pl.qkv_txt_w, ws.qkv[:, :T], bias=pl.qkv_txt_b, rope=rt)])
    q, k, v = ws.qkv[..., :d], ws.qkv[..., d : 2 * d], ws.qkv[..., 2 * d :]
    if ip is not None and ip_inside:
        ops.ip_attention_gated(q[:, T:], pl.nq_img, ip[0], ip[1], x_i, H, ip_scale=ip[2], gate=ch(mi, 2), accumulate=True)
        ip = None
    if ip is not None:
        ip_out = ws.ip_buffer()
        ops.ip_attention(q[:, T:], pl.nq_img, ip[0], ip[1], ip_out, H, ip_scale=ip[2])
        if inject is None:
            inject, ip = ip_out, None
    if pl.fp8_attention:
        qk8, vt8 = ws.fp8_attn_buffers(H)
        ops.attention_fp8_prep(ws.qkv, 0, d, 2 * d, H, T, pl.nq_txt, pl.nk_txt, pl.nq_img, pl.nk_img, cos, sin, qk8, vt8)
        if pl.mx:
            ops.attention_fp8_mx(qk8, vt8, ws.fp8_wide(d), ws.mx_scales(), H)
        else:
            ops.attention_fp8(qk8, vt8, q, H)
    else:
        if not fused_rope:
            ops.qk_rmsnorm_rope(ws.qkv, 0, d, H, T, pl.nq_txt, pl.nk_txt, pl.nq_img, pl.nk_img, cos, sin)
        ops.attention(q, k, v, q, H)
    if pl.mx:
        a8, sc = ws.fp8_wide(d), ws.mx_scales()
        if not pl.fp8_attention:
            ops.quantize_mx_fp8_into(q, a8, sc)
        ops.linear_grouped([P(a8[:, T:], pl.out_img_w8, x_i, bias=pl.out_img_b, gate=ch(mi, 2), res=x_i, a_bscale=sc.rows(T), w_scale=pl.out_img_ws),
                            P(a8[:, :T], pl.out_txt_w8, x_t, bias=pl.out_txt_b, gate=ch(mt, 2), res=x_t, a_bscale=sc.rows(0), w_scale=pl.out_txt_ws)])
    elif pl.out_img_w8 is not None:
        a8 = ws.fp8_wide(d)
        ops.quantize_rows_fp8_into(q[:, T:], a8[:, T:], ws.xs_i)
        ops.quantize_rows_fp8_into(q[:, :T], a8[:, :T], ws.xs_t)
        ops.linear_grouped([P(a8[:, T:], pl.out_img_w8, x_i, bias=pl.out_img_b, gate=ch(mi, 2), res=x_i, a_scale=ws.xs_i, w_scale=pl.out_img_ws),
                            P(a8[:, :T], pl.out_txt_w8, x_t, bias=pl.out_txt_b, gate=ch(mt, 2), res=x_t, a_scale=ws.xs_t, w_scale=pl.out_txt_ws)])
    else:
        ops.linear_grouped([P(q[:, T:], pl.out_img_w, x_i, bias=pl.out_img_b, gate=ch(mi, 2), res=x_i),
                            P(q[:, :T], pl.out_txt_w, x_t, bias=pl.out_txt_b, gate=ch(mt, 2), res=x_t)])
    if fp8:
        ops.layernorm_modulate_fp8(x_i, xn8_i, ws.xs_i, ch(mi, 3), ch(mi, 4))
        ops.layernorm_modulate_fp8(x_t, xn8_t, ws.xs_t, ch(mt, 3), ch(mt, 4))
        h8, hs = (ws.fp8_wide(4 * d), ws.mx_scales()) if pl.mx else (None, None)
        o8 = lambda r0, r1: dict(out8=h8[:, r0:r1], out8_scales=hs.rows(r0), out8_from=0) if pl.mx else {}
        ops.linear_grouped([P(xn8_i, pl.ff1_img_w8, ws.ffh[:, T:], bias=pl.ff1_img_b, gelu_from=0, a_scale=ws.xs_i, w_scale=pl.ff1_img_ws, **o8(T, ws.S)),
                            P(xn8_t, pl.ff1_txt_w8, ws.ffh[:, :T], bias=pl.ff1_txt_b, gelu_from=0, a_scale=ws.xs_t, w_scale=pl.ff1_txt_ws, **o8(0, T))])
    else:
        ops.layernorm_modulate_pair(x_i, xn_i, ch(mi, 3), ch(mi, 4), x_t, xn_t, ch(mt, 3), ch(mt, 4))
        ops.linear_grouped([P(xn_i, pl.ff1_img_w, ws.ffh[:, T:], bias=pl.ff1_img_b, gelu_from=0),
                            P(xn_t, pl.ff1_txt_w, ws.ffh[:, :T], bias=pl.ff1_txt_b, gelu_from=0)])
    if pl.mx:
        ops.linear_grouped([P(h8[:, T:], pl.ff2_img_w8, x_i, bias=pl.ff2_img_b, gate=ch(mi, 5), res=x_i, add2=inject, a_bscale=hs.rows(T), w_scale=pl.ff2_img_ws),
                            P(h8[:, :T], pl.ff2_txt_w8, x_t, bias=pl.ff2_txt_b, gate=ch(mt, 5), res=x_t, a_bscale=hs.rows(0), w_scale=pl.ff2_txt_ws)])
    elif pl.ff2_img_w8 is not None:
        a8 = ws.fp8_wide(4 * d)
        ops.quantize_rows_fp8_into(ws.ffh[:, T:], a8[:, T:], ws.xs_i)
        ops.quantize_rows_fp8_into(ws.ffh[:, :T], a8[:, :T], ws.xs_t)
        ops.linear_grouped([P(a8[:, T:], pl.ff2_img_w8, x_i, bias=pl.ff2_img_b, gate=ch(mi, 5), res=x_i, add2=inject, a_scale=ws.xs_i, w_scale=pl.ff2_img_ws),
                            P(a8[:, :T], pl.ff2_txt_w8, x_t, bias=pl.ff2_txt_b, gate=ch(mt, 5), res=x_t, a_scale=ws.xs_t, w_scale=pl.ff2_txt_ws)])
    else:
        ops.linear_grouped([P(ws.ffh[:, T:], pl.ff2_img_w, x_i, bias=pl.ff2_img_b, gate=ch(mi, 5), res=x_i, add2=inject),
                            P(ws.ffh[:, :T], pl.ff2_txt_w, x_t, bias=pl.ff2_txt_b, gate=ch(mt, 5), res=x_t)])
    if ip is not None:
        for b in range(ws.B):
            ops.masked_accumulate_(ws.x[b, T:].unsqueeze(0), ip_out[b : b + 1], None, 1.0, True)


def run_single(pl: SinglePlan, ws: Workspace, temb: torch.Tensor, cos, sin, H: int, inject: Optional[torch.Tensor] = None,
               mods: Optional[torch.Tensor] = None, ip: Optional[tuple] = None) -> None:
    T, d = ws.T, ws.d
    if mods is not None:
        m = mods
    else:
        m = ws.mod_a[:, : 3 * d]
        ops.gemv(temb, pl.ada_w, pl.ada_b, m, silu_in=True)
    big = ws.big
    fused_rope = False
    if pl.fused_w8 is not None:
        xn8 = ws.fp8_buffers()
        ops.layernorm_modulate_fp8(ws.x, xn8, ws.xs_all, m[:, :d], m[:, d : 2 * d])
        o8 = dict(out8=ws.fp8_wide(5 * d)[..., d:], out8_scales=ws.mx_scales().cols(d), out8_from=3 * d) if pl.mx else {}
        ops.linear(xn8, pl.fused_w8, big, bias=pl.fused_b, gelu_from=3 * d, a_scale=ws.xs_all, w_scale=pl.fused_ws, **o8)
    else:
        ops.layernorm_modulate(ws.x, ws.xn, m[:, :d], m[:, d : 2 * d])
        fused_rope = FUSED_QK_ROPE and ip is None and not pl.fp8_attention and ops.QKRope.covers(d)
        ops.linear(ws.xn, pl.fused_w, big, bias=pl.fused_b, gelu_from=3 * d,
                   rope=ops.QKRope(2 * d, 0, d, pl.nq, pl.nk, cos, sin) if fused_rope else None)
    q = big[..., 2 * d : 3 * d]
    if ip is not None:
        ip_out = ws.ip_buffer_joint()
        ops.ip_attention_gated(q, pl.nq, ip[0], ip[1], ip_out, H, ip_scale=ip[2])
    if pl.fp8_attention:
        qk8, vt8 = ws.fp8_attn_buffers(H)
        ops.attention_fp8_prep(big, 2 * d, 0, d, H, 0, None, None, pl.nq, pl.nk, cos, sin, qk8, vt8)
        if pl.mx and ip is None:
            ops.attention_fp8_mx(qk8, vt8, ws.fp8_wide(5 * d)[..., :d], ws.mx_scales(), H)
        else:
            ops.attention_fp8(qk8, vt8, q, H)
    else:
        if not fused_rope:
            ops.qk_rmsnorm_rope(big, 2 * d, 0, H, 0, None, None, pl.nq, pl.nk, cos, sin)
        ops.attention(q, big[..., :d], big[..., d : 2 * d], q, H)
    if ip is not None:
        ops.add_bf16_(q, ip_out)
    if pl.mx:
        a8, sc = ws.fp8_wide(5 * d), ws.mx_scales()
        if not pl.fp8_attention or ip is not None:
            ops.quantize_mx_fp8_into(q, a8[..., :d], sc)
        ops.linear(a8, pl.out_w8, ws.x, bias=pl.out_b, gate=m[:, 2 * d : 3 * d], res=ws.x, a_bscale=sc, w_scale=pl.out_ws)
    elif pl.out_w8 is not None:
        a8 = ws.fp8_wide(5 * d)
        ops.quantize_rows_fp8_into(big[..., 2 * d :], a8, ws.xs_all)
        ops.linear(a8, pl.out_w8, ws.x, bias=pl.out_b, gate=m[:, 2 * d : 3 * d], res=ws.x, a_scale=ws.xs_all, w_scale=pl.out_ws)
    else:
        ops.linear(big[..., 2 * d :], pl.out_w, ws.x, bias=pl.out_b, gate=m[:, 2 * d : 3 * d], res=ws.x)
    if inject is not None:
        for b in range(ws.B):
            ops.masked_accumulate_(ws.x[b, T:].unsqueeze(0), inject[b : b + 1].contiguous(), None, 1.0, True)


def image_rows_bf16(ws: Workspace) -> torch.Tensor:
    T = ws.T
    if ws.x.dtype == BF16:
        return ws.x[:, T:]
    for b in range(ws.B):
        src, dst = ws.x[b, T:], ws.xn[b, T:]
        native.check("rt_cast_f32_to_bf16", native.load().rt_cast_f32_to_bf16(src.data_ptr(), dst.data_ptr(), src.numel(), ops._stream()))
    return ws.xn[:, T:]
```

### arabic-text-image-generation-reptext_amd/native.py

```python
from __future__ import annotations

import ctypes as C
import os

_HERE = os.path.dirname(os.path.abspath(__file__))
LIB_NAME = "librt_reptext_hip.so"
LIB_PATH = os.path.join(_HERE, LIB_NAME)

RT_GEMM_MAX_GROUPS = 4
ABI_VERSION = 15
RT_LORA_MAX_TERMS = 8


class NativeLibraryMissing(RuntimeError):
    pass


class NativeCallError(RuntimeError):
    def __init__(self, fn: str, code: int):
        names = {-1: "RT_E_BADARG", -2: "RT_E_ALIGN", -3: "RT_E_SHAPE"}
        super().__init__(f"{fn} failed: {names.get(code, 'hipError ' + str(code))} ({code})")
        self.code = code


class GemmGroup(C.Structure):

    _fields_ = [
        ("A", C.c_void_p), ("W", C.c_void_p), ("C", C.c_void_p), ("bias", C.c_void_p),
        ("gate", C.c_void_p), ("res", C.c_void_p), ("add2", C.c_void_p), ("rowscale", C.c_void_p),
        ("lda", C.c_int64), ("ldw", C.c_int64), ("ldc", C.c_int64), ("ldr", C.c_int64),
        ("ld2", C.c_int64), ("gate_ld", C.c_int64),
        ("strideA", C.c_int64), ("strideC", C.c_int64), ("strideR", C.c_int64), ("stride2", C.c_int64),
        ("M", C.c_int32), ("N", C.c_int32), ("K", C.c_int32), ("batch", C.c_int32),
        ("rows_per_batch", C.c_int32), ("gelu_from", C.c_int32), ("out_f32", C.c_int32),
        ("alpha", C.c_float),
        ("a_scale", C.c_void_p), ("w_scale", C.c_void_p),
        ("stride_rowscale", C.c_int64),
        ("a_bscale", C.c_void_p), ("a_bscale_plane", C.c_int64), ("a_bscale_rows", C.c_int64),
        ("c8", C.c_void_p), ("c_bscale", C.c_void_p),
        ("ldc8", C.c_int64), ("stride_c8", C.c_int64), ("c_bscale_plane", C.c_int64), ("c_bscale_rows", C.c_int64),
        ("c8_from", C.c_int32), ("c_bscale_k0", C.c_int32),
        ("conv_ks", C.c_int32), ("conv_cin", C.c_int32), ("conv_w2", C.c_int32), ("conv_h2", C.c_int32),
        ("conv_inv_w2", C.c_float), ("conv_inv_h2", C.c_float),
        ("rope_cos", C.c_void_p), ("rope_sin", C.c_void_p), ("rope_wq", C.c_void_p), ("rope_wk", C.c_void_p),
        ("rope_q0", C.c_int32), ("rope_k0", C.c_int32), ("rope_w", C.c_int32), ("rope_pos0", C.c_int32),
        ("rope_eps", C.c_float), ("rope_reserved", C.c_int32),
    ]


class SkinnyGroup(C.Structure):

    _fields_ = [("W", C.c_void_p), ("bias", C.c_void_p), ("C", C.c_void_p), ("ldw", C.c_int64), ("ldc", C.c_int64), ("N", C.c_int32), ("reserved", C.c_int32)]


class LnSegment(C.Structure):

    _fields_ = [("x", C.c_void_p), ("out", C.c_void_p), ("shift", C.c_void_p), ("scale", C.c_void_p),
                ("ldx", C.c_int64), ("stride_xb", C.c_int64), ("ldo", C.c_int64), ("stride_ob", C.c_int64), ("mod_ld", C.c_int64),
                ("batch", C.c_int32), ("rows_per_batch", C.c_int32)]


class LoraTerm(C.Structure):

    _fields_ = [("B", C.c_void_p), ("At", C.c_void_p), ("ldb", C.c_int64), ("lda", C.c_int64), ("r_pad", C.c_int32), ("scale", C.c_float)]


_i32, _i64, _f32, _vp = C.c_int32, C.c_int64, C.c_float, C.c_void_p

SIGNATURES = {
    "rt_abi_version": [],
    "rt_gemm_bf16": [C.POINTER(GemmGroup), _i32, _vp],
    "rt_gemm_fp8": [C.POINTER(GemmGroup), _i32, _vp],
    "rt_quantize_rows_fp8": [_vp, _i64, _i32, _vp, _i64, _vp, _i32, _i32, _vp],
    "rt_quantize_mx_fp8": [_vp, _i64, _i32, _vp, _i64, _vp, _i64, _i32, _i32, _vp],
    "rt_layernorm_modulate_fp8": [_vp, _i64, _i64, _i32, _vp, _i64, _i64, _vp, _vp, _vp, _i64, _i32, _i32, _i32, _f32, _vp],
    "rt_gemv_bf16w": [_vp, _i64, _vp, _i64, _vp, _vp, _i64, _i32, _i32, _i32, _i32, _i32, _i32, _vp],
    "rt_timestep_embedding": [_vp, _vp, _i32, _i32, _vp],
    "rt_rope_table": [_vp, _vp, _vp, _i32, C.POINTER(_i32), _f32, _vp],
    "rt_layernorm_modulate": [_vp, _i64, _i64, _i32, _vp, _i64, _i64, _vp, _vp, _i64, _i32, _i32, _i32, _f32, _vp],
    "rt_qk_rmsnorm_rope": [_vp, _i64, _i64, _i64, _i64, _vp, _vp, _vp, _vp, _vp, _vp, _i32, _i32, _i32, _i32, _f32, _vp],
    "rt_attention_ws_bytes": [_i32, _i32, _i32],
    "rt_attention_variant": [_i32],
    "rt_attention_fwd": [_vp, _vp, _vp, _vp, _i64, _i64, _i64, _i64, _i32, _i32, _i32, _f32, _vp, _i64, _vp],
    "rt_attention_fp8_vt_bytes": [_i32, _i32, _i32],
    "rt_attention_fp8_prep": [_vp, _i64, _i64, _i64, _i64, _i64, _vp, _vp, _vp, _vp, _vp, _vp, _vp, _vp, _i32, _i32, _i32, _i32, _f32, _vp],
    "rt_attention_fp8_fwd": [_vp, _vp, _vp, _i64, _i64, _i32, _i32, _i32, _f32, _vp],
    "rt_attention_fp8_fwd_mx": [_vp, _vp, _vp, _i64, _i64, _vp, _i64, _i64, _i32, _i32, _i32, _i32, _f32, _vp],
    "rt_embedding_gather": [_vp, _i64, _vp, _vp, _i64, _i32, _i32, _i32, _vp],
    "rt_rmsnorm_rows": [_vp, _i64, _i32, _vp, _vp, _i64, _i32, _i32, _f32, _vp],
    "rt_softmax_rows_bias": [_vp, _i64, _vp, _i64, _vp, _i64, _i32, _i32, _i32, _f32, _vp],
    "rt_gated_mul": [_vp, _i64, _vp, _i64, _i32, _i32, _vp],
    "rt_quick_gelu": [_vp, _i64, _vp],
    "rt_euler_step": [_vp, _vp, _f32, _i64, _vp],
    "rt_euler_step_f32": [_vp, _vp, _vp, _f32, _i64, _vp],
    "rt_cfg_mix": [_vp, _vp, _vp, _f32, _i64, _vp],
    "rt_pack_latents": [_vp, _vp, _i32, _i32, _i32, _i32, _vp],
    "rt_unpack_latents": [_vp, _vp, _i32, _i32, _i32, _i32, _f32, _f32, _vp],
    "rt_cast_f32_to_bf16": [_vp, _vp, _i64, _vp],
    "rt_cast_bf16_to_f32": [_vp, _vp, _i64, _vp],
    "rt_silu_split_bf16": [_vp, _vp, _vp, _i64, _i32, _vp],
    "rt_masked_accumulate": [_vp, _vp, _vp, _f32, _i32, _i32, _i32, _i32, _i32, _vp],
}
SIGNATURES.update({
    "rt_groupnorm_ws_bytes": [_i32, _i32, _i32, _i32],
    "rt_groupnorm_silu_nhwc": [_vp, _vp, _vp, _vp, _vp, _i32, _i32, _i32, _i32, _i32, _f32, _i32, _vp],
    "rt_conv2d_nhwc": [_vp, _vp, _vp, _vp, _vp, _i32, _i32, _i32, _i32, _i32, _i32, _i32, _i32, _i32, _vp],
    "rt_softmax_rows": [_vp, _vp, _i32, _i32, _f32, _vp],
    "rt_vae_attention": [_vp, _vp, _vp, _vp, _i64, _i64, _i64, _i64, _i32, _i32, _i32, _f32, _vp],
    "rt_transpose_bf16": [_vp, _vp, _i32, _i32, _i64, _i64, _vp],
    "rt_image_out": [_vp, _vp, _vp, _i32, _i32, _i32, _i32, _i32, _vp],
    "rt_nchw_to_haloed_nhwc": [_vp, _vp, _i32, _i32, _i32, _i32, _i32, _vp],
    "rt_haloed_nhwc_to_nchw": [_vp, _vp, _i32, _i32, _i32, _i32, _i32, _vp],
    "rt_unpack_latents_haloed": [_vp, _vp, _i32, _i32, _i32, _i32, _i32, _f32, _f32, _vp],
    "rt_resize2d": [_vp, _i32, _f32, _vp, _i32, _i32, _i32, _i32, _i32, _f32, _f32, _i32, _vp],
    "rt_glyph_blend": [_vp, _vp, _vp, _vp, _i32, _i32, _i32, _i32, _i32, _i32, _i32, _vp],
})
SIGNATURES.update({
    "rt_conv2d_variant": [_i32],
    "rt_canny_ws_bytes": [_i32, _i32],
    "rt_canny_u8": [_vp, _i32, _i32, _i32, _f32, _f32, _vp, _i32, _i32, _vp, _i64, _vp],
    "rt_preprocess_u8": [_vp, _vp, _i32, _i32, _i32, _i32, _i32, _vp],
})

SIGNATURES["rt_lora_merge_bf16"] = [C.POINTER(LoraTerm), _i32, _vp, _i64, _vp, _i64, _i32, _i32, _vp]

SIGNATURES["rt_ip_attention"] = [_vp, _i64, _i64, _vp, _vp, _vp, _i64, _i64, _vp, _i64, _i64, _i32, _i32, _i32, _i32, _i32, _i32, _f32, _f32, _f32, _vp]

SIGNATURES["rt_ip_attention_gated"] = [_vp, _i64, _i64, _vp, _vp, _vp, _i64, _i64, _vp, _i64, _vp, _i64, _i64, _i32, _i32, _i32, _i32, _i32, _i32,
                                       _f32, _f32, _f32, _vp]
SIGNATURES["rt_gelu_erf_bf16"] = [_vp, _vp, _i64, _vp]
SIGNATURES["rt_add_bf16_2d"] = [_vp, _i64, _i64, _vp, _i64, _i64, _i32, _i32, _i32, _vp]

RT_ATTENTION_HD64_MAX_S = 4096
SIGNATURES["rt_attention_hd64"] = [_vp, _vp, _vp, _i64, _i64, _vp, _i64, _i64, _i32, _i32, _i32, _f32, _vp]
SIGNATURES["rt_patchify_nchw"] = [_vp, _i32, _vp, _i32, _i32, _i32, _i32, _vp]

RT_ATTENTION_HD72_MAX_S = 1024
SIGNATURES["rt_attention_hd72"] = [_vp, _i64, _i64, _vp, _vp, _i64, _i64, _vp, _i64, _i64, _i32, _i32, _i32, _i32, _f32, _vp]

SIGNATURES["rt_gemm_skinny_bf16"] = [_vp, _vp, _i64, _i32, _i32, C.POINTER(SkinnyGroup), _i32, _vp]
SIGNATURES["rt_layernorm_modulate_pair"] = [C.POINTER(LnSegment), _i32, _i32, _f32, _vp]
SIGNATURES["rt_add_rows_f32"] = [_vp, _vp, _vp, _i32, _i32, _i32, _vp]

RESTYPES = {"rt_canny_ws_bytes": C.c_int64, "rt_groupnorm_ws_bytes": C.c_int64, "rt_attention_fp8_vt_bytes": C.c_int64, "rt_attention_ws_bytes": C.c_int64}

_lib = None


def library_present() -> bool:
    return os.path.isfile(LIB_PATH)


def load():
    global _lib
    if _lib is not None:
        return _lib
    if not library_present():
        raise NativeLibraryMissing(
            f"{LIB_PATH} not found. Build it with `python -c 'import __graft_entry__ as g; g.build()'` "
            "(hipcc --offload-arch=gfx950). There is no CPU fallback for the HIP path."
        )
    lib = C.CDLL(LIB_PATH)
    lib.rt_version.restype = C.c_char_p
    lib.rt_version.argtypes = []
    for name, argtypes in SIGNATURES.items():
        fn = getattr(lib, name)
        fn.argtypes = argtypes
        fn.restype = RESTYPES.get(name, C.c_int)
    if lib.rt_abi_version() != ABI_VERSION:
        raise NativeLibraryMissing(f"{LIB_NAME} ABI {lib.rt_abi_version()} != binding ABI {ABI_VERSION}; rebuild")
    _lib = lib
    return lib


def check(fn: str, code: int) -> None:
    if code != 0:
        raise NativeCallError(fn, code)
```

### arabic-text-image-generation-reptext_amd/ops.py

```python
from __future__ import annotations

import ctypes as C
from dataclasses import dataclass
from typing import Optional, Sequence

import torch

from . import native

BF16 = torch.bfloat16
F32 = torch.float32
FP8 = torch.float8_e4m3fn


def _stream() -> int:
    return torch.cuda.current_stream().cuda_stream


def _dev(t: torch.Tensor, name: str, dtype=None) -> int:
    if not isinstance(t, torch.Tensor):
        raise TypeError(f"{name}: expected a tensor, got {type(t)}")
    if not t.is_cuda:
        raise RuntimeError(f"{name}: tensor is on {t.device}; the HIP path has no CPU fallback")
    if dtype is not None and t.dtype != dtype:
# ... 301 lines not shown
        _dev(x, "x"), x.stride(1), x.stride(0), int(x.dtype == F32), _dev(out, "out", BF16), out.stride(1), out.stride(0),
        _opt(shift, "shift", F32), _opt(scale, "scale", F32), mod_ld, B, R, D, float(eps), _stream()))
    return out


def layernorm_modulate_pair(x0, out0, shift0, scale0, x1, out1, shift1, scale1, eps: float = 1e-6) -> None:
    segs = (native.LnSegment * 2)()
    D = x0.shape[2]
    for g, (x, out, shift, scale) in zip(segs, ((x0, out0, shift0, scale0), (x1, out1, shift1, scale1))):
        if x.dim() != 3 or out.dim() != 3 or x.shape != out.shape or x.stride(2) != 1 or out.stride(2) != 1 or x.shape[2] != D or x.dtype != x0.dtype:
            raise ValueError("layernorm_modulate_pair: x/out must be [B,R,D] with unit inner stride, one D and one dtype of x")
        B, R, _ = x.shape
        if scale is not None:
            if scale.shape != (B, D) or shift.shape != (B, D) or scale.stride(1) != 1 or shift.stride(1) != 1 or scale.stride(0) != shift.stride(0):
                raise ValueError("shift/scale must be [B,D] views with equal row stride")
            g.mod_ld = scale.stride(0)
        g.x, g.out, g.shift, g.scale = _dev(x, "x"), _dev(out, "out", BF16), _opt(shift, "shift", F32), _opt(scale, "scale", F32)
        g.ldx, g.stride_xb, g.ldo, g.stride_ob, g.batch, g.rows_per_batch = x.stride(1), x.stride(0), out.stride(1), out.stride(0), B, R
    if x0.dtype not in (BF16, F32):
        raise TypeError("x must be bf16 or f32")
    native.check("rt_layernorm_modulate_pair", native.load().rt_layernorm_modulate_pair(segs, int(x0.dtype == F32), D, float(eps), _stream()))


def layernorm_modulate_fp8(x: torch.Tensor, out: torch.Tensor, row_scale: torch.Tensor, shift: Optional[torch.Tensor],
                           scale: Optional[torch.Tensor], eps: float = 1e-6) -> torch.Tensor:
    if x.dim() != 3 or out.dim() != 3 or x.shape != out.shape or x.stride(2) != 1 or out.stride(2) != 1:
        raise ValueError("layernorm_modulate_fp8: x/out must be [B,R,D] with unit inner stride")
    B, R, D = x.shape
    if row_scale.numel() != B * R or not row_scale.is_contiguous():
        raise ValueError("row_scale must be contiguous with B*R elements")
    mod_ld = 0
    if scale is not None:
        if scale.shape != (B, D) or shift.shape != (B, D) or scale.stride(1) != 1 or shift.stride(1) != 1 or scale.stride(0) != shift.stride(0):
            raise ValueError("shift/scale must be [B,D] views with equal row stride")
        mod_ld = scale.stride(0)
    if x.dtype not in (BF16, F32):
        raise TypeError("x must be bf16 or f32")
    native.check("rt_layernorm_modulate_fp8", native.load().rt_layernorm_modulate_fp8(
        _dev(x, "x"), x.stride(1), x.stride(0), int(x.dtype == F32), _dev(out, "out", FP8), out.stride(1), out.stride(0),
        _dev(row_scale, "row_scale", F32), _opt(shift, "shift", F32), _opt(scale, "scale", F32), mod_ld, B, R, D, float(eps), _stream()))
    return out


def quantize_rows_fp8(x: torch.Tensor):
    rows, D, ldx = _rowmajor2d(x, "x")
    if x.dtype not in (BF16, F32):
        raise TypeError("x must be bf16 or f32")
    q = torch.empty(rows, D, device=x.device, dtype=FP8)
    sc = torch.empty(rows, device=x.device, dtype=F32)
    native.check("rt_quantize_rows_fp8", native.load().rt_quantize_rows_fp8(
        _dev(x, "x"), ldx, int(x.dtype == F32), q.data_ptr(), D, sc.data_ptr(), rows, D, _stream()))
    return q, sc


def quantize_rows_fp8_into(x: torch.Tensor, out: torch.Tensor, scale: torch.Tensor) -> None:
    if x.dim() != 3 or out.dim() != 3 or x.shape != out.shape or x.stride(2) != 1 or out.stride(2) != 1:
        raise ValueError("quantize_rows_fp8_into: x/out must be [B,R,D] views with unit inner stride")
    B, R, D = x.shape
    if scale.numel() != B * R or not scale.is_contiguous():
        raise ValueError("scale must be contiguous with B*R elements")
    if x.dtype not in (BF16, F32):
        raise TypeError("x must be bf16 or f32")
    lib, st = native.load(), _stream()
    esz = x.element_size()
    _dev(out, "out", FP8), _dev(scale, "scale", F32), _dev(x, "x")
    for b in range(B):
        native.check("rt_quantize_rows_fp8", lib.rt_quantize_rows_fp8(
            x.data_ptr() + b * x.stride(0) * esz, x.stride(1), int(x.dtype == F32), out.data_ptr() + b * out.stride(0), out.stride(1),
            scale.data_ptr() + b * R * 4, R, D, st))


def quantize_mx_fp8_into(x: torch.Tensor, out: torch.Tensor, scales: BlockScales) -> None:
    if x.dim() != 3 or out.dim() != 3 or x.shape != out.shape or x.stride(2) != 1 or out.stride(2) != 1:
        raise ValueError("quantize_mx_fp8_into: x/out must be [B,R,D] views with unit inner stride")
    B, R, D = x.shape
    if x.dtype not in (BF16, F32):
        raise TypeError("x must be bf16 or f32")
    if D % 256 or scales.k0 != 0 or scales.columns_left() < D:
        raise ValueError("D % 256 == 0, written from column 0 of a scale tensor that covers D")
    lib, st = native.load(), _stream()
    esz = x.element_size()
    _dev(out, "out", FP8), _dev(x, "x")
    for b in range(B):
        native.check("rt_quantize_mx_fp8", lib.rt_quantize_mx_fp8(
            x.data_ptr() + b * x.stride(0) * esz, x.stride(1), int(x.dtype == F32), out.data_ptr() + b * out.stride(0), out.stride(1),
            scales.ptr() + b * (scales.R // 64) * 2048, scales.plane, R, D, st))


def dequantize_mx(q: torch.Tensor, scales: BlockScales) -> torch.Tensor:
    B, R, D = q.shape
    e = scales.rowmajor(B, R, D).to(torch.float32) - 127.0
    return (q.to(torch.float32).view(B, R, D // 32, 32) * torch.exp2(e).unsqueeze(-1)).view(B, R, D)


def lora_merge_(w: torch.Tensor, w0: torch.Tensor, terms: Sequence[tuple]) -> torch.Tensor:
    N, K, ldw = _rowmajor2d(w, "w")
    N0, K0, ld0 = _rowmajor2d(w0, "w0")
    if (N0, K0) != (N, K):
        raise ValueError(f"lora_merge_: w {tuple(w.shape)} and w0 {tuple(w0.shape)} differ")
    if len(terms) > native.RT_LORA_MAX_TERMS:
        raise ValueError(f"lora_merge_: at most {native.RT_LORA_MAX_TERMS} terms per weight, got {len(terms)}")
    if K % 8 or ldw % 8 or ld0 % 8:
        raise ValueError("lora_merge_: K and the row strides must be multiples of 8")
    pw, p0 = _dev(w, "w", BF16), _dev(w0, "w0", BF16)
    arr = (native.LoraTerm * max(1, len(terms)))()
    for t, (b, at, c) in enumerate(terms):
        rb, r_pad, ldb = _rowmajor2d(b, "B")
        ka, ra, lda = _rowmajor2d(at, "At")
        if rb != N or ka != K or ra != r_pad or r_pad % 32:
            raise ValueError(f"lora_merge_: term {t}: B {tuple(b.shape)} / At {tuple(at.shape)} do not fit w [{N}, {K}] with r_pad % 32 == 0")
        if b.device != w.device or at.device != w.device:
            raise RuntimeError("lora_merge_: factors and weight must be on the same device")
        arr[t] = native.LoraTerm(_dev(b, "B", BF16), _dev(at, "At", BF16), ldb, lda, r_pad, float(c))
    native.check("rt_lora_merge_bf16", native.load().rt_lora_merge_bf16(arr, len(terms), p0, ld0, pw, ldw, N, K, _stream()))
    return w


def qk_rmsnorm_rope(buf: torch.Tensor, q_off: int, k_off: int, H: int, T: int, wq_txt, wk_txt, wq_img, wk_img,
                    cos: torch.Tensor, sin: torch.Tensor, eps: float = 1e-6) -> None:
    if buf.dim() != 3 or buf.stride(2) != 1:
        raise ValueError("buf must be [B,S,ld] with unit inner stride")
    B, S, _ = buf.shape
    if cos.shape != (S, 128) or sin.shape != (S, 128) or not cos.is_contiguous() or not sin.is_contiguous():
        raise ValueError("cos/sin must be contiguous [S,128]")
    native.check("rt_qk_rmsnorm_rope", native.load().rt_qk_rmsnorm_rope(
        _dev(buf, "buf", BF16), buf.stride(1), buf.stride(0), q_off, k_off, _opt(wq_txt, "wq_txt", BF16), _opt(wk_txt, "wk_txt", BF16),
        _dev(wq_img, "wq_img", BF16), _dev(wk_img, "wk_img", BF16), _dev(cos, "cos", F32), _dev(sin, "sin", F32), B, S, T, H, float(eps), _stream()))


_ATTN_WS = {}
CAPTURE_KEEP: Optional[list] = None


def _attention_workspace(B: int, S: int, H: int, device) -> Optional[torch.Tensor]:
    key = (B, S, H, str(device), _stream())
    ws = _ATTN_WS.get(key, False)
    if ws is False:
        n = int(native.load().rt_attention_ws_bytes(B, S, H))
        ws = torch.zeros(n, device=device, dtype=torch.uint8) if n > 0 else None
        if len(_ATTN_WS) > 16:
            _ATTN_WS.clear()
        _ATTN_WS[key] = ws
    if CAPTURE_KEEP is not None and ws is not None:
        CAPTURE_KEEP.append(ws)
    return ws


def drop_attention_workspaces(keys) -> None:
    for k in list(keys):
        _ATTN_WS.pop(k, None)


def attention(q: torch.Tensor, k: torch.Tensor, v: torch.Tensor, out: torch.Tensor, H: int, scale: Optional[float] = None,
              split: bool = True) -> torch.Tensor:
    for name, t in (("q", q), ("k", k), ("v", v), ("out", out)):
        if t.dim() != 3 or t.stride(2) != 1 or t.shape[2] != H * 128:
            raise ValueError(f"{name}: need [B,S,{H*128}] with unit inner stride")
    B, S, _ = q.shape
    if not (q.stride() == k.stride() == v.stride()) or k.shape != q.shape or v.shape != q.shape or out.shape != q.shape:
        raise ValueError("q,k,v must share shape and strides")
    sc = (128 ** -0.5) if scale is None else float(scale)
    ws = _attention_workspace(B, S, H, q.device) if split else None
    native.check("rt_attention_fwd", native.load().rt_attention_fwd(
        _dev(q, "q", BF16), _dev(k, "k", BF16), _dev(v, "v", BF16), _dev(out, "out", BF16), q.stride(1), q.stride(0),
        out.stride(1), out.stride(0), B, S, H, sc, None if ws is None else ws.data_ptr(), 0 if ws is None else ws.numel(), _stream()))
    return out


def ip_attention(q: torch.Tensor, wq: torch.Tensor, k: torch.Tensor, v: torch.Tensor, out: torch.Tensor, H: int, ip_scale: float = 1.0,
                 accumulate: bool = False, scale: Optional[float] = None, eps: float = 1e-6) -> torch.Tensor:
    d = H * 128
    for name, t in (("q", q), ("k", k), ("v", v), ("out", out)):
        if t.dim() != 3 or t.stride(2) != 1 or t.shape[2] != d:
            raise ValueError(f"{name}: need [B,rows,{d}] with unit inner stride, got {tuple(t.shape)} / {t.stride()}")
    B, N, _ = q.shape
    if out.shape != q.shape or out.dtype not in (BF16, F32):
        raise ValueError("out must match q in shape and be bf16 or f32")
    if k.shape != v.shape or k.stride() != v.stride() or k.shape[0] not in (1, B):
        raise ValueError("k and v must share shape and strides, with batch 1 or B")
    n = k.shape[1]
    if not 1 <= n <= 128:
        raise ValueError(f"ip_attention: 1..128 image-prompt tokens, got {n}")
    if wq.numel() != 128 or not wq.is_contiguous():
        raise ValueError("wq must be contiguous with 128 elements")
    sc = (128 ** -0.5) if scale is None else float(scale)
    native.check("rt_ip_attention", native.load().rt_ip_attention(
        _dev(q, "q", BF16), q.stride(1), q.stride(0), _dev(wq, "wq", BF16), _dev(k, "k", BF16), _dev(v, "v", BF16), k.stride(1),
        k.stride(0) if k.shape[0] == B and B > 1 else 0, _dev(out, "out"), out.stride(1), out.stride(0), int(out.dtype == F32),
        int(accumulate), B, N, H, n, sc, float(ip_scale), float(eps), _stream()))
    return out


def ip_attention_gated(q: torch.Tensor, wq: torch.Tensor, k: torch.Tensor, v: torch.Tensor, out: torch.Tensor, H: int, ip_scale: float = 1.0,
                       gate: Optional[torch.Tensor] = None, accumulate: bool = False, scale: Optional[float] = None, eps: float = 1e-6) -> torch.Tensor:
    d = H * 128
    for name, t in (("q", q), ("k", k), ("v", v), ("out", out)):
        if t.dim() != 3 or t.stride(2) != 1 or t.shape[2] != d:
            raise ValueError(f"{name}: need [B,rows,{d}] with unit inner stride, got {tuple(t.shape)} / {t.stride()}")
    B, N, _ = q.shape
    if out.shape != q.shape or out.dtype not in (BF16, F32):
        raise ValueError("out must match q in shape and be bf16 or f32")
    if k.shape != v.shape or k.stride() != v.stride() or k.shape[0] not in (1, B):
        raise ValueError("k and v must share shape and strides, with batch 1 or B")
    n = k.shape[1]
    if not 1 <= n <= 128:
        raise ValueError(f"ip_attention_gated: 1..128 image-prompt tokens, got {n}")
    if wq.numel() != 128 or not wq.is_contiguous():
        raise ValueError("wq must be contiguous with 128 elements")
    if gate is not None and (gate.dim() != 2 or gate.shape != (B, d) or gate.stride(1) != 1):
        raise ValueError(f"gate must be a [B,{d}] view with unit inner stride")
    sc = (128 ** -0.5) if scale is None else float(scale)
    native.check("rt_ip_attention_gated", native.load().rt_ip_attention_gated(
        _dev(q, "q", BF16), q.stride(1), q.stride(0), _dev(wq, "wq", BF16), _dev(k, "k", BF16), _dev(v, "v", BF16), k.stride(1),
        k.stride(0) if k.shape[0] == B and B > 1 else 0, _opt(gate, "gate", F32), 0 if gate is None else gate.stride(0),
        _dev(out, "out"), out.stride(1), out.stride(0), int(out.dtype == F32), int(accumulate), B, N, H, n, sc, float(ip_scale), float(eps), _stream()))
    return out


def gelu_erf(x: torch.Tensor) -> torch.Tensor:
    if not x.is_contiguous():
        raise ValueError("gelu_erf: contiguous input")
    out = torch.empty(x.shape, device=x.device, dtype=BF16)
    native.check("rt_gelu_erf_bf16", native.load().rt_gelu_erf_bf16(_dev(x, "x", F32), out.data_ptr(), x.numel(), _stream()))
    return out


def add_bf16_(y: torch.Tensor, x: torch.Tensor) -> torch.Tensor:
    if x.shape != y.shape or x.dim() != 3 or x.stride(2) != 1 or y.stride(2) != 1:
        raise ValueError("add_bf16_: [B,R,D] views of equal shape with unit inner stride")
    B, R, D = x.shape
    native.check("rt_add_bf16_2d", native.load().rt_add_bf16_2d(_dev(x, "x", BF16), x.stride(1), x.stride(0), _dev(y, "y", BF16), y.stride(1),
                                                                y.stride(0), B, R, D, _stream()))
    return y


def rmsnorm_heads_(x: torch.Tensor, out: torch.Tensor, ones: torch.Tensor, eps: float) -> torch.Tensor:
    if x.shape != out.shape or not x.is_contiguous() or not out.is_contiguous() or x.numel() % 128 or ones.numel() != 128:
        raise ValueError("rmsnorm_heads_: contiguous tensors of equal shape, a multiple of 128 elements")
    native.check("rt_rmsnorm_rows", native.load().rt_rmsnorm_rows(_dev(x, "x", F32), 128, 1, _dev(ones, "ones", BF16), _dev(out, "out", BF16), 128,
                                                                  x.numel() // 128, 128, float(eps), _stream()))
    return out


def _attention_small_head(hd: int, entry: str, max_s: int, q: torch.Tensor, k: torch.Tensor, v: torch.Tensor, out: torch.Tensor, H: int,
                          scale: Optional[float]) -> torch.Tensor:
    d = H * hd
    for tn, t in (("q", q), ("k", k), ("v", v), ("out", out)):
        if t.dim() != 3 or t.stride(2) != 1 or t.shape[2] != d:
            raise ValueError(f"{tn}: need [B,S,{d}] with unit inner stride, got {tuple(t.shape)} / {t.stride()}")
    B, Sk, _ = k.shape
    Sq = q.shape[1]
    sc = float(scale if scale is not None else (64 ** -0.5 if hd == 64 else 72 ** -0.5))
    if hd == 64:
        if not (q.stride() == k.stride() == v.stride()) or k.shape != q.shape or v.shape != q.shape or out.shape != q.shape:
            raise ValueError("q,k,v must share shape and strides; out must have their shape")
        if not 1 <= Sq <= max_s:
            raise ValueError(f"{entry[3:]}: 1..{max_s} rows, got {Sq}")
        code = native.load().rt_attention_hd64(_dev(q, "q", BF16), _dev(k, "k", BF16), _dev(v, "v", BF16), q.stride(1), q.stride(0),
                                               _dev(out, "out", BF16), out.stride(1), out.stride(0), B, Sq, H, sc, _stream())
    else:
        if k.stride() != v.stride() or v.shape != k.shape:
            raise ValueError("k,v must share shape and strides")
        if q.shape[0] not in (1, B) or out.shape != (B, Sq, d):
            raise ValueError(f"q must be [{B} or 1, Sq, {d}] and out [{B}, Sq, {d}], got {tuple(q.shape)} and {tuple(out.shape)}")
        if not (1 <= Sq <= max_s and 1 <= Sk <= max_s):
            raise ValueError(f"{entry[3:]}: 1..{max_s} rows, got {Sq} queries and {Sk} keys")
        code = native.load().rt_attention_hd72(_dev(q, "q", BF16), q.stride(1), q.stride(0) if q.shape[0] == B and B > 1 else 0, _dev(k, "k", BF16),
                                               _dev(v, "v", BF16), k.stride(1), k.stride(0), _dev(out, "out", BF16), out.stride(1), out.stride(0), B,
                                               Sq, Sk, H, sc, _stream())
    native.check(entry, code)
    return out


def attention_hd64(q: torch.Tensor, k: torch.Tensor, v: torch.Tensor, out: torch.Tensor, H: int, scale: Optional[float] = None) -> torch.Tensor:
    return _attention_small_head(64, "rt_attention_hd64", native.RT_ATTENTION_HD64_MAX_S, q, k, v, out, H, scale)


def attention_hd72(q: torch.Tensor, k: torch.Tensor, v: torch.Tensor, out: torch.Tensor, H: int, scale: Optional[float] = None) -> torch.Tensor:
    return _attention_small_head(72, "rt_attention_hd72", native.RT_ATTENTION_HD72_MAX_S, q, k, v, out, H, scale)


def patchify_nchw(x: torch.Tensor, patch: int, Kp: Optional[int] = None) -> torch.Tensor:
    if x.dim() != 4 or x.shape[1] != 3 or x.shape[2] != x.shape[3] or x.shape[2] % patch or x.dtype not in (BF16, F32):
        raise ValueError(f"patchify_nchw: need a square f32 or bf16 [B,3,G*{patch},G*{patch}] image, got {tuple(x.shape)} {x.dtype}")
    x = x.contiguous()
    B, G = x.shape[0], x.shape[2] // patch
    Kp = (3 * patch * patch + 63) // 64 * 64 if Kp is None else int(Kp)
    out = torch.empty(B, G * G, Kp, device=x.device, dtype=BF16)
    native.check("rt_patchify_nchw", native.load().rt_patchify_nchw(_dev(x, "x"), int(x.dtype == F32), out.data_ptr(), B, G, patch, Kp, _stream()))
    return out


def attention_fp8_prep(buf: torch.Tensor, q_off: int, k_off: int, v_off: int, H: int, T: int, wq_txt, wk_txt, wq_img, wk_img,
                       cos: torch.Tensor, sin: torch.Tensor, qk8: torch.Tensor, vt8: torch.Tensor, eps: float = 1e-6) -> None:
    if buf.dim() != 3 or buf.stride(2) != 1:
        raise ValueError("buf must be [B,S,ld] with unit inner stride")
    B, S, _ = buf.shape
    if cos.shape != (S, 128) or sin.shape != (S, 128) or not cos.is_contiguous() or not sin.is_contiguous():
        raise ValueError("cos/sin must be contiguous [S,128]")
    lib = native.load()
    if qk8.shape != (B, S, 2 * H * 128) or not qk8.is_contiguous() or vt8.numel() < int(lib.rt_attention_fp8_vt_bytes(B, S, H)):
        raise ValueError("qk8 must be contiguous [B,S,2*H*128]; vt8 must hold rt_attention_fp8_vt_bytes(B,S,H) bytes")
    native.check("rt_attention_fp8_prep", lib.rt_attention_fp8_prep(
        _dev(buf, "buf", BF16), buf.stride(1), buf.stride(0), q_off, k_off, v_off, _opt(wq_txt, "wq_txt", BF16), _opt(wk_txt, "wk_txt", BF16),
        _dev(wq_img, "wq_img", BF16), _dev(wk_img, "wk_img", BF16), _dev(cos, "cos", F32), _dev(sin, "sin", F32),
        _dev(qk8, "qk8", FP8), _dev(vt8, "vt8", FP8), B, S, T, H, float(eps), _stream()))


def attention_fp8(qk8: torch.Tensor, vt8: torch.Tensor, out: torch.Tensor, H: int, scale: Optional[float] = None) -> torch.Tensor:
    B, S, _ = qk8.shape
    if out.dim() != 3 or out.shape[0] != B or out.shape[1] != S or out.stride(2) != 1:
        raise ValueError("out must be [B,S,*] with unit inner stride")
    native.check("rt_attention_fp8_fwd", native.load().rt_attention_fp8_fwd(
        _dev(qk8, "qk8", FP8), _dev(vt8, "vt8", FP8), _dev(out, "out", BF16), out.stride(1), out.stride(0), B, S, H,
        float(scale if scale is not None else 128 ** -0.5), _stream()))
    return out


# ... 149 lines not shown
```

### arabic-text-image-generation-reptext_amd/pipeline.py

```python
from __future__ import annotations

import contextlib
import functools
import inspect
import json
import os
from dataclasses import dataclass
from typing import Any, Callable, Dict, List, Optional, Tuple, Union

import numpy as np
import torch
import torch.nn.functional as F

from . import ops
from .controlnet import FluxControlNetModel, FluxMultiControlNetModel
from .image_processor import PipelineImageInput, VaeImageProcessor
from .scheduler import FlowMatchEulerDiscreteScheduler, calculate_shift
from .transformer import FluxTransformer2DModel
from .utils import randn_tensor
from .vae import AutoencoderKL


@dataclass
class FluxPipelineOutput:
    images: Any


def retrieve_latents(encoder_output, generator: Optional[torch.Generator] = None, sample_mode: str = "sample"):
    if hasattr(encoder_output, "latent_dist") and sample_mode == "sample":
        return encoder_output.latent_dist.sample(generator)
    if hasattr(encoder_output, "latent_dist") and sample_mode == "argmax":
        return encoder_output.latent_dist.mode()
    if hasattr(encoder_output, "latents"):
        return encoder_output.latents
    raise AttributeError("Could not access latents of provided encoder_output")


def retrieve_timesteps(scheduler, num_inference_steps: Optional[int] = None, device=None, timesteps: Optional[List[int]] = None,
                       sigmas: Optional[List[float]] = None, **kwargs):
    if timesteps is not None and sigmas is not None:
        raise ValueError("Only one of `timesteps` or `sigmas` can be passed. Please choose one to set custom values")
    accepted = set(inspect.signature(scheduler.set_timesteps).parameters.keys())
    if timesteps is not None:
        if "timesteps" not in accepted:
            raise ValueError(f"The current scheduler class {scheduler.__class__}'s `set_timesteps` does not support custom"
                             f" timestep schedules. Please check whether you are using the correct scheduler.")
        scheduler.set_timesteps(timesteps=timesteps, device=device, **kwargs)
    elif sigmas is not None:
        if "sigmas" not in accepted:
            raise ValueError(f"The current scheduler class {scheduler.__class__}'s `set_timesteps` does not support custom"
                             f" sigmas schedules. Please check whether you are using the correct scheduler.")
        scheduler.set_timesteps(sigmas=sigmas, device=device, **kwargs)
    else:
        scheduler.set_timesteps(num_inference_steps, device=device, **kwargs)
    return scheduler.timesteps, len(scheduler.timesteps)


class _Progress:
    def __init__(self, total, disable=False):
        self.bar = None
        if not disable:
            try:
                from tqdm.auto import tqdm

                self.bar = tqdm(total=total)
            except Exception:
                self.bar = None

    def __enter__(self):
        return self

    def __exit__(self, *a):
        if self.bar is not None:
            self.bar.close()

    def update(self, n=1):
        if self.bar is not None:
            self.bar.update(n)


OVERLAP_TOWER = os.environ.get("RT_OVERLAP_TOWER", "1") == "1"
GRAPH_CAPTURE = os.environ.get("RT_GRAPH", "1") == "1"
GRAPH_CACHE_MAX = 2


def accepts_ip_adapter_arguments(call):
    @functools.wraps(call)
    def wrapper(self, *args, ip_adapter_image=None, ip_adapter_image_embeds=None, **kwargs):
        self._ip_call_args = (ip_adapter_image, ip_adapter_image_embeds)
        try:
            return call(self, *args, **kwargs)
        finally:
            self._ip_call_args, self._ip_embeds = (None, None), None
    return wrapper


class FluxControlNetPipeline:
    model_cpu_offload_seq = "text_encoder->text_encoder_2->transformer->vae"
    _optional_components: List[str] = []
    _callback_tensor_inputs = ["latents", "prompt_embeds"]

    def __init__(self, scheduler: FlowMatchEulerDiscreteScheduler, vae: AutoencoderKL, text_encoder, tokenizer, text_encoder_2,
                 tokenizer_2, transformer: FluxTransformer2DModel,
                 controlnet: Union[FluxControlNetModel, List[FluxControlNetModel], Tuple[FluxControlNetModel], FluxMultiControlNetModel]):
        self.vae, self.text_encoder, self.text_encoder_2 = vae, text_encoder, text_encoder_2
        self.tokenizer, self.tokenizer_2 = tokenizer, tokenizer_2
        self.transformer, self.scheduler, self.controlnet = transformer, scheduler, controlnet
        self.vae_scale_factor = 2 ** len(self.vae.config.block_out_channels) if self.vae is not None else 16
        self.image_processor = VaeImageProcessor(vae_scale_factor=self.vae_scale_factor)
        self.tokenizer_max_length = self.tokenizer.model_max_length if self.tokenizer is not None else 77
        self.default_sample_size = 64
        self._guidance_scale, self._joint_attention_kwargs, self._interrupt, self._num_timesteps = 1.0, None, False, 0
        self._progress_disabled = False
        self._ip_call_args, self._ip_embeds = (None, None), None
        self.image_encoder, self.feature_extractor = None, None

    @property
    def components(self) -> Dict[str, Any]:
        return dict(scheduler=self.scheduler, vae=self.vae, text_encoder=self.text_encoder, tokenizer=self.tokenizer,
                    text_encoder_2=self.text_encoder_2, tokenizer_2=self.tokenizer_2, transformer=self.transformer,
                    controlnet=self.controlnet)

    @classmethod
    def from_pretrained(cls, pretrained_model_name_or_path: str, controlnet=None, torch_dtype=None, **kwargs):
        from .modules import resolve_model_path

        root = resolve_model_path(pretrained_model_name_or_path, kwargs.pop("revision", None))
        dt = torch_dtype or torch.bfloat16
        index = {}
        ip = os.path.join(root, "model_index.json")
        if os.path.isfile(ip):
            with open(ip) as f:
                index = {k: v for k, v in json.load(f).items() if not k.startswith("_")}
        listed = lambda name: (not index) or (index.get(name) not in (None, [None, None]))
        for required in ("transformer", "vae"):
            if required not in kwargs and not (listed(required) and os.path.isdir(os.path.join(root, required))):
                raise OSError(f"{cls.__name__}.from_pretrained: component '{required}' is neither passed nor present under {root}")
        sched_cfg = {}
        sp = os.path.join(root, "scheduler", "scheduler_config.json")
        if os.path.isfile(sp):
            with open(sp) as f:
                sched_cfg = {k: v for k, v in json.load(f).items() if not k.startswith("_")}
        known = set(FlowMatchEulerDiscreteScheduler().config.keys())
        scheduler = kwargs.pop("scheduler", None) or FlowMatchEulerDiscreteScheduler(**{k: v for k, v in sched_cfg.items() if k in known})
        transformer = kwargs.pop("transformer", None) or FluxTransformer2DModel.from_pretrained(root, torch_dtype=dt, subfolder="transformer")
        vae = kwargs.pop("vae", None) or AutoencoderKL.from_pretrained(root, torch_dtype=dt, subfolder="vae")
        te, te2 = kwargs.pop("text_encoder", None), kwargs.pop("text_encoder_2", None)
        tok, tok2 = kwargs.pop("tokenizer", None), kwargs.pop("tokenizer_2", None)
        image_encoder, feature_extractor = kwargs.pop("image_encoder", None), kwargs.pop("feature_extractor", None)
        if image_encoder is None and index.get("image_encoder") not in (None, [None, None]) and os.path.isdir(os.path.join(root, "image_encoder")):
            from .image_encoder import image_encoder_class

            image_encoder = image_encoder_class(os.path.join(root, "image_encoder")).from_pretrained(root, subfolder="image_encoder", torch_dtype=dt)
        try:
            if te is None and listed("text_encoder") and os.path.isdir(os.path.join(root, "text_encoder")):
                from .text_encoders import CLIPTextModel

                te = CLIPTextModel.from_pretrained(root, subfolder="text_encoder", torch_dtype=dt)
            if te2 is None and listed("text_encoder_2") and os.path.isdir(os.path.join(root, "text_encoder_2")):
                from .text_encoders import T5EncoderModel

                te2 = T5EncoderModel.from_pretrained(root, subfolder="text_encoder_2", torch_dtype=dt)
            if tok is None and listed("tokenizer") and os.path.isdir(os.path.join(root, "tokenizer")):
                from transformers import CLIPTokenizer

                tok = CLIPTokenizer.from_pretrained(os.path.join(root, "tokenizer"))
            if tok2 is None and listed("tokenizer_2") and os.path.isdir(os.path.join(root, "tokenizer_2")):
                from transformers import T5TokenizerFast

                tok2 = T5TokenizerFast.from_pretrained(os.path.join(root, "tokenizer_2"))
        except Exception as e:
            raise OSError(f"could not load text encoders from {root}: {e}") from e
        if isinstance(controlnet, str):
            controlnet = FluxControlNetModel.from_pretrained(controlnet, torch_dtype=dt)
        extra = {k: kwargs[k] for k in ("controlnet_inpaint",) if k in kwargs}
        pipe = cls(scheduler=scheduler, vae=vae, text_encoder=te, tokenizer=tok, text_encoder_2=te2, tokenizer_2=tok2,
                   transformer=transformer, controlnet=controlnet, **extra)
        pipe.image_encoder, pipe.feature_extractor = image_encoder, feature_extractor
        return pipe

    def save_pretrained(self, root: str, max_shard_bytes: int = 10 << 30) -> None:
        os.makedirs(root, exist_ok=True)
        index = {"_class_name": type(self).__name__, "_diffusers_version": "0.36.0"}
        for name in ("transformer", "vae", "text_encoder", "text_encoder_2"):
            m = getattr(self, name, None)
            if m is not None and hasattr(m, "save_pretrained"):
                m.save_pretrained(os.path.join(root, name), max_shard_bytes=max_shard_bytes) if name in ("transformer", "vae") else m.save_pretrained(os.path.join(root, name))
                index[name] = ["reptext_amd", type(m).__name__]
            else:
                index[name] = [None, None]
        for name in ("tokenizer", "tokenizer_2"):
            t = getattr(self, name, None)
            if t is not None and hasattr(t, "save_pretrained"):
                t.save_pretrained(os.path.join(root, name))
                index[name] = ["transformers", type(t).__name__]
            else:
                index[name] = [None, None]
        os.makedirs(os.path.join(root, "scheduler"), exist_ok=True)
        with open(os.path.join(root, "scheduler", "scheduler_config.json"), "w") as f:
            json.dump(dict(_class_name="FlowMatchEulerDiscreteScheduler", **dict(self.scheduler.config)), f, indent=2)
        index["scheduler"] = ["reptext_amd", "FlowMatchEulerDiscreteScheduler"]
        with open(os.path.join(root, "model_index.json"), "w") as f:
            json.dump(index, f, indent=2)

    def to(self, device=None, dtype=None):
        for m in list(self.components.values()) + [self.image_encoder]:
            if isinstance(m, torch.nn.Module):
                m.to(device=device, dtype=dtype) if dtype is not None else m.to(device)
        return self

    @property
    def _execution_device(self):
        return self.transformer.device

    @property
    def device(self):
        return self.transformer.device

    def maybe_free_model_hooks(self):
        """Offload hooks belong to accelerate-based CPU offload, which this single-device path does not use (no-op)."""

    def set_progress_bar_config(self, disable: bool = False, **kw):
        self._progress_disabled = disable

    def progress_bar(self, total=None):
        return _Progress(total, disable=self._progress_disabled)

    @property
    def do_classifier_free_guidance(self):
        return self._guidance_scale > 1

    @property
    def guidance_scale(self):
        return self._guidance_scale

# ... 279 lines not shown
        if e.shape[1] != adapter.E:
            raise ValueError(f"ip_adapter_image_embeds: width {e.shape[1]} != the adapter's image embedding width {adapter.E}")
        if not adapter.active:
            return None, kw
        return e.to(device=device, dtype=torch.bfloat16).contiguous(), kw

    def encode_image(self, image, device=None, num_images_per_prompt: int = 1) -> torch.Tensor:
        if self.image_encoder is None:
            raise ValueError("encode_image: this pipeline has no image_encoder")
        device = device or self._execution_device
        from .image_encoder import SiglipVisionModel

        siglip = isinstance(self.image_encoder, SiglipVisionModel)
        if isinstance(image, torch.Tensor):
            pixel_values = image if image.dim() == 4 else image[None]
        elif self.feature_extractor is not None:
            pixel_values = self.feature_extractor(images=image, return_tensors="pt").pixel_values
        else:
            from .image_encoder import clip_preprocess, siglip_preprocess

            pixel_values = (siglip_preprocess if siglip else clip_preprocess)(image, size=self.image_encoder.config.image_size)
        out = self.image_encoder(pixel_values.to(device))
        embeds = out.pooler_output if siglip else out.image_embeds
        return embeds.repeat_interleave(num_images_per_prompt, dim=0) if num_images_per_prompt != 1 else embeds

    def _lora_models(self) -> list:
        cn = self.controlnet
        nets = list(cn.nets) if isinstance(cn, FluxMultiControlNetModel) else [cn]
        models = [self.transformer] + nets + [getattr(self, "controlnet_inpaint", None)]
        return [m for m in models if m is not None and getattr(m, "_lora", None) is not None]

    def _apply_lora_scale(self) -> None:
        for m in self._lora_models():
            m._apply_lora_scale(self.joint_attention_kwargs)

    def _graph_safe_kwargs(self) -> bool:
        kw = self.joint_attention_kwargs
        return kw is None or (set(kw) == {"scale"} and bool(self._lora_models()))

    @accepts_ip_adapter_arguments
    @torch.no_grad()
    def __call__(self, prompt: Union[str, List[str]] = None, prompt_2: Optional[Union[str, List[str]]] = None,
                 height: Optional[int] = None, width: Optional[int] = None, num_inference_steps: int = 28,
                 timesteps: List[int] = None, guidance_scale: float = 7.0,
                 control_guidance_start: Union[float, List[float]] = 0.0, control_guidance_end: Union[float, List[float]] = 1.0,
                 control_image: PipelineImageInput = None, control_mode: Optional[Union[int, List[int]]] = None,
                 controlnet_conditioning_scale: Union[float, List[float]] = 1.0, controlnet_conditioning_step: int = 30,
                 num_images_per_prompt: Optional[int] = 1,
                 generator: Optional[Union[torch.Generator, List[torch.Generator]]] = None,
                 latents: Optional[torch.FloatTensor] = None, prompt_embeds: Optional[torch.FloatTensor] = None,
                 pooled_prompt_embeds: Optional[torch.FloatTensor] = None, output_type: Optional[str] = "pil",
                 return_dict: bool = True, joint_attention_kwargs: Optional[Dict[str, Any]] = None,
                 callback_on_step_end: Optional[Callable[[int, int, Dict], None]] = None,
                 callback_on_step_end_tensor_inputs: List[str] = ["latents"], max_sequence_length: int = 512,
                 control_mask: Optional[torch.FloatTensor] = None, control_position: Optional[torch.FloatTensor] = None,
                 control_glyph: Optional[torch.FloatTensor] = None):
        height = height or self.default_sample_size * self.vae_scale_factor
        width = width or self.default_sample_size * self.vae_scale_factor
        self.check_inputs(prompt, prompt_2, height, width, prompt_embeds=prompt_embeds, pooled_prompt_embeds=pooled_prompt_embeds,
                          callback_on_step_end_tensor_inputs=callback_on_step_end_tensor_inputs, max_sequence_length=max_sequence_length)
        self._guidance_scale, self._joint_attention_kwargs, self._interrupt = guidance_scale, joint_attention_kwargs, False
        batch_size = self._batch_size(prompt, prompt_embeds)
        device, dtype = self._execution_device, self.transformer.dtype
        total = batch_size * num_images_per_prompt
        self._ip_embeds, self._joint_attention_kwargs = self._resolve_ip_embeds(*self._ip_call_args, joint_attention_kwargs, batch_size,
                                                                                num_images_per_prompt, device)

        prompt_embeds, pooled_prompt_embeds, text_ids = self.encode_prompt(
            prompt=prompt, prompt_2=prompt_2, prompt_embeds=prompt_embeds, pooled_prompt_embeds=pooled_prompt_embeds, device=device,
            num_images_per_prompt=num_images_per_prompt, max_sequence_length=max_sequence_length)
        prompt_embeds = prompt_embeds.to(device=device)
        pooled_prompt_embeds = pooled_prompt_embeds.to(device=device)

        hints, height, width = self._collect_hints(control_image, control_position, height, width, total, num_images_per_prompt, device, dtype)
        timesteps, num_inference_steps = self._schedule(height, width, num_inference_steps, timesteps, device)
        latents, latent_image_ids = self._initial_latents(control_glyph, total, height, width, prompt_embeds.dtype, device, generator, latents)
        masks = self._region_masks(control_mask, latents.device, latents.dtype)

        self._apply_lora_scale()
        latents = self._denoise(latents, prompt_embeds, pooled_prompt_embeds, text_ids, latent_image_ids, timesteps, hints, masks,
                                guidance_scale, controlnet_conditioning_scale, controlnet_conditioning_step, control_mode,
                                callback_on_step_end, callback_on_step_end_tensor_inputs, num_inference_steps)
        return self._finish(latents, height, width, output_type, return_dict)

    @staticmethod
    def _batch_size(prompt, prompt_embeds) -> int:
        if isinstance(prompt, str):
            return 1
        return len(prompt) if isinstance(prompt, list) else prompt_embeds.shape[0]

    def _collect_hints(self, control_image, control_position, height, width, total, num_images_per_prompt, device, dtype, cfg=False):
        hints: List[torch.Tensor] = []
        if isinstance(self.controlnet, FluxControlNetModel) and control_image is not None:
            positions = control_position if control_position is not None else [None] * len(control_image)
            for img, pos in zip(control_image, positions):
                if self._is_packed_hint(img):
                    h = img.to(device=device, dtype=dtype)
                    hints.append(torch.cat([h] * 2) if (cfg and h.shape[0] == total) else h)
                else:
                    h, height, width = self.prepare_image(image=img, image_position=pos, width=width, height=height, batch_size=total,
                                                          num_images_per_prompt=num_images_per_prompt, device=device, dtype=dtype,
                                                          do_classifier_free_guidance=cfg)
                    hints.append(h)
        return hints, height, width

    def _schedule(self, height, width, num_inference_steps, timesteps, device):
        sigmas = np.linspace(1.0, 1 / num_inference_steps, num_inference_steps)
        image_seq_len = (int(height) // self.vae_scale_factor) * (int(width) // self.vae_scale_factor)
        sc = self.scheduler.config
        mu = calculate_shift(image_seq_len, sc.base_image_seq_len, sc.max_image_seq_len, sc.base_shift, sc.max_shift)
        timesteps, num_inference_steps = retrieve_timesteps(self.scheduler, num_inference_steps, device, timesteps, sigmas, mu=mu)
        self._num_timesteps = len(timesteps)
        return timesteps, num_inference_steps

    def _initial_latents(self, control_glyph, total, height, width, dtype, device, generator, latents):
        num_channels_latents = self.transformer.config.in_channels // 4
        if control_glyph is None:
            return self.prepare_latents(total, num_channels_latents, height, width, dtype, device, generator, latents)
        init_image = self.image_processor.preprocess(control_glyph, height=height, width=width).to(dtype=torch.float32)
        return self.prepare_latents_reptext(init_image, total, num_channels_latents, height, width, dtype, device, generator, None)

    def _finish(self, latents, height, width, output_type, return_dict):
        if output_type == "latent":
            image = self._master_latents
        else:
            h2 = 2 * (int(height) // self.vae_scale_factor)
            w2 = 2 * (int(width) // self.vae_scale_factor)
            if output_type in ("pil", "np"):
                u8 = self.vae.decode_packed(latents, h2, w2, output_u8=True)
                image = self.image_processor.postprocess_u8(u8, output_type)
            elif output_type == "pt":
                image = (self.vae.decode_packed(latents, h2, w2) / 2 + 0.5).clamp(0, 1)
            else:
                raise ValueError(f"unsupported output_type {output_type}")
        self.maybe_free_model_hooks()
        if not return_dict:
            return (image,)
        return FluxPipelineOutput(images=image)

    reference_bf16_scalars = False

    def _model_timestep(self, t: float) -> float:
        from . import mmdit

        mmdit.reference_bf16_scalars(self.reference_bf16_scalars)
        if not self.reference_bf16_scalars:
            return t / 1000.0
        return float((torch.tensor(t, dtype=torch.float32).to(torch.bfloat16) / 1000).to(torch.float32))

    def _denoise(self, latents, prompt_embeds, pooled, text_ids, image_ids, timesteps, hints, masks, guidance_scale,
                 cn_scale, cn_steps, control_mode, callback, callback_inputs, num_inference_steps):
        tvals = timesteps.to(torch.float32).cpu().tolist()
        ipe = getattr(self, "_ip_embeds", None)

        def eager(callback=None):
            return self._denoise_eager(latents, prompt_embeds, pooled, text_ids, image_ids, tvals, hints, masks, guidance_scale, cn_scale,
                                       cn_steps, control_mode, callback, callback_inputs, num_inference_steps, timesteps, _ip_embeds=ipe)

        use_graph = (GRAPH_CAPTURE and getattr(self, "capture_graphs", True) and callback is None and latents.is_cuda
                     and not self.interrupt and isinstance(self.controlnet, (FluxControlNetModel, type(None)))
                     and (control_mode is None) and self._graph_safe_kwargs())
        if not use_graph:
            return eager(callback)
        from . import mmdit as _mm
        _mm.reference_bf16_scalars(self.reference_bf16_scalars)
        sig = lambda t: (tuple(t.shape), str(t.dtype), tuple(t.stride()))
        models = tuple((id(m), id(m._ensure_plans()), id(getattr(m, "_cx_pad", None)), bool(getattr(m, "_fp8_linears", False)),
                        bool(getattr(m, "_fp8_attention", False))) for m in (self.transformer, self.controlnet) if m is not None)
        key = (sig(latents), sig(prompt_embeds), sig(pooled), sig(text_ids), sig(image_ids), tuple(sig(h) for h in hints), tuple(sig(m) for m in masks),
               tuple(tvals), tuple(self.scheduler.sigmas.tolist()), float(guidance_scale), repr(cn_scale), int(cn_steps), int(num_inference_steps),
               str(latents.device), models, bool(self.reference_bf16_scalars), bool(_mm.RESIDUAL_F32), bool(OVERLAP_TOWER), bool(_mm.FUSED_QK_ROPE))
        if ipe is not None:
            adapter = self.transformer._ip_adapter
            key += (sig(ipe), adapter.version, tuple(adapter.scales))
        cache = self.__dict__.setdefault("_graph_cache", {})
        ent = cache.get(key)
        if ent is None:
            if len(cache) >= GRAPH_CACHE_MAX:
                cache.pop(next(iter(cache)))
            cache[key] = "seen"
            return eager()
        if ent == "failed":
            return eager()
        ins = [latents, prompt_embeds, pooled, text_ids, image_ids] + list(hints) + list(masks) + ([ipe] if ipe is not None else [])
        if ent == "seen":
            static = [t.clone() for t in ins]
            nh, nm = len(hints), len(masks)
            keep = [m._ensure_plans() for m in (self.transformer, self.controlnet) if m is not None] + [getattr(self.controlnet, "_cx_pad", None)]
            keep.append(getattr(self.transformer, "_ip_adapter", None) if ipe is not None else None)
            graph = torch.cuda.CUDAGraph()
            step_index = self.scheduler._step_index
            attn_keys = set(ops._ATTN_WS)
            _mm.CAPTURE_KEEP, ops.CAPTURE_KEEP = keep, keep
            try:
                with torch.cuda.graph(graph, capture_error_mode="thread_local"):
                    out = self._denoise_eager(static[0], static[1], static[2], static[3], static[4], tvals, static[5 : 5 + nh], static[5 + nh : 5 + nh + nm],
                                              guidance_scale, cn_scale, cn_steps, control_mode, None, callback_inputs, num_inference_steps, timesteps,
                                              _quiet=True, _ip_embeds=static[-1] if ipe is not None else None)
                    out32 = self._master_latents
            except Exception as e:
                import sys
                print(f"[reptext_amd] hipGraph capture of the denoise loop failed ({type(e).__name__}: {e}); staying eager", file=sys.stderr, flush=True)
                cache[key] = "failed"
                _mm.CAPTURE_KEEP = ops.CAPTURE_KEEP = None
                ops.drop_attention_workspaces(set(ops._ATTN_WS) - attn_keys)
                torch.cuda.synchronize()
                self.scheduler._step_index = step_index
                return eager()
            _mm.CAPTURE_KEEP = ops.CAPTURE_KEEP = None
            keep.append(getattr(self, "_sample_cache", None))
            keep.extend(dict(m._rope_cache) for m in (self.transformer, self.controlnet) if m is not None and hasattr(m, "_rope_cache"))
            self.scheduler._step_index = step_index
            ent = cache[key] = {"graph": graph, "static": static, "out": out, "out32": out32, "keep": keep}
        for dst, src in zip(ent["static"], ins):
            if dst.data_ptr() != src.data_ptr():
                dst.copy_(src)
        ent["graph"].replay()
        self.scheduler._step_index = (self.scheduler._step_index or 0) + len(tvals)
        self._master_latents = ent["out32"].clone()
        with self.progress_bar(total=num_inference_steps) as bar:
            bar.update(num_inference_steps)
        return ent["out"].clone()

    def _denoise_eager(self, latents, prompt_embeds, pooled, text_ids, image_ids, tvals, hints, masks, guidance_scale,
                       cn_scale, cn_steps, control_mode, callback, callback_inputs, num_inference_steps, timesteps, _quiet=False,
                       _ip_embeds=None, _extra_towers=(), _velocity=None):
        device = latents.device
        B = latents.shape[0]
        guidance = torch.full((B,), float(guidance_scale), device=device, dtype=torch.float32) if self.transformer.config.guidance_embeds else None
        rowscales = [m.to(torch.float32).reshape(-1).contiguous() if m.shape[0] == 1 else m.to(torch.float32).reshape(m.shape[0], -1).contiguous() for m in masks]
        num_warmup = max(len(timesteps) - num_inference_steps * self.scheduler.order, 0)
        model_ts = [self._model_timestep(t) for t in tvals]
        g_tab = guidance if guidance is None or pooled.shape[0] == B else guidance.expand(pooled.shape[0]).contiguous()
        tab_t = self.transformer.build_modulation_table(model_ts, g_tab, pooled)
        fused_cn = isinstance(self.controlnet, FluxControlNetModel) and len(hints) > 0
        towers = []
        if fused_cn and cn_steps > 0:
            ts_c = model_ts[: min(len(model_ts), cn_steps)]
            tab_c = self.controlnet.build_modulation_table(ts_c, g_tab, pooled)
            towers = [(self.controlnet, h, cn_scale, rowscales[line] if rowscales else None, tab_c) for line, h in enumerate(hints)]
            towers += [(m, h, s, None, m.build_modulation_table(ts_c, g_tab, pooled)) for m, h, s in _extra_towers]

        def prepare_static(pe):
            return self.transformer.prepare_static(pe), [tw[0].prepare_static(pe, tw[1]) for tw in towers]

        static_t, static_c = prepare_static(prompt_embeds)
        ip_prep = self.transformer._ip_adapter.prepare(_ip_embeds) if _ip_embeds is not None else None
        blocks_needed, sample_buf, single_buf = None, None, None
        if fused_cn:
            cnet = self.controlnet
            n_cd, n_cs = len(cnet.transformer_blocks), len(cnet.single_transformer_blocks)
            n_td, n_ts = len(self.transformer.transformer_blocks), len(self.transformer.single_transformer_blocks)
            if all((len(m.transformer_blocks), len(m.single_transformer_blocks)) == (n_cd, n_cs) for m, _, _ in _extra_towers):
                need_d = 0 if n_cd == 0 else (n_td - 1) // int(np.ceil(n_td / n_cd)) + 1
                need_s = 0 if n_cs == 0 or n_ts == 0 else (n_ts - 1) // int(np.ceil(n_ts / n_cs)) + 1
                blocks_needed = (min(need_d, n_cd), min(need_s, n_cs))
            Bc, N_, d_ = prompt_embeds.shape[0], latents.shape[1], cnet.inner_dim
            key = (Bc, N_, d_, n_cd, n_cs, str(device))
            if getattr(self, "_sample_cache", None) is None or self._sample_cache[0] != key:
                mk = lambda n: [torch.empty(Bc, N_, d_, device=device, dtype=torch.bfloat16) for _ in range(n)]
                self._sample_cache = (key, mk(n_cd), mk(n_cs))
            sample_buf, single_buf = self._sample_cache[1], self._sample_cache[2]
        lat32 = latents.to(torch.float32).contiguous()
        latents = latents.to(torch.bfloat16).contiguous().clone()
        overlap = (OVERLAP_TOWER and bool(towers) and not _extra_towers and device.type == "cuda"
                   and len(self.controlnet.single_transformer_blocks) == 0)
        side = sample_ev = None
        if overlap:
            if getattr(self, "_side_stream", None) is None or self._side_stream.device != device:
                self._side_stream = torch.cuda.Stream(device=device)
            side = self._side_stream
            sample_ev = [torch.cuda.Event() for _ in range(len(self.controlnet.transformer_blocks))]
        with (_Progress(num_inference_steps, disable=True) if _quiet else self.progress_bar(total=num_inference_steps)) as bar:
            for i, t in enumerate(tvals):
                if self.interrupt:
                    continue
                timestep = torch.full((B,), self._model_timestep(t), device=device, dtype=torch.float32)
                merged = merged_single = events = None
                if towers and i < cn_steps:
                    if overlap:
                        side.wait_stream(torch.cuda.current_stream())
                        events = sample_ev
                    with torch.cuda.stream(side) if overlap else contextlib.nullcontext():
                        for k, ((model, hint, scale, rowscale, table), static) in enumerate(zip(towers, static_c)):
                            samples = model(
                                hidden_states=latents, controlnet_cond=hint, controlnet_mode=control_mode, conditioning_scale=scale,
                                timestep=timestep, guidance=guidance, pooled_projections=pooled, encoder_hidden_states=prompt_embeds,
                                txt_ids=text_ids, img_ids=image_ids, joint_attention_kwargs=self.joint_attention_kwargs,
                                return_dict=False, _rowscale=rowscale, _accumulate_into=sample_buf, _accumulate_single_into=single_buf,
                                _overwrite=(k == 0), _sample_events=events if k == len(towers) - 1 else None, _mods=table.step(i),
                                _ws_tag="tower" if overlap else "", _static=static, _blocks_needed=blocks_needed)
                            if k == 0:
                                merged, merged_single = samples
                noise_pred = self.transformer(
                    hidden_states=latents, timestep=timestep, guidance=guidance, pooled_projections=pooled,
                    encoder_hidden_states=prompt_embeds, controlnet_block_samples=merged, controlnet_single_block_samples=merged_single,
                    txt_ids=text_ids, img_ids=image_ids, joint_attention_kwargs=self.joint_attention_kwargs, return_dict=False,
                    _mods=tab_t.step(i), _sample_events=events, _static=static_t, _ip=ip_prep)[0]
                if events is not None:
                    torch.cuda.current_stream().wait_stream(side)
                if _velocity is not None:
                    noise_pred = _velocity(i, noise_pred)
                self.scheduler.step_master_(noise_pred, lat32, latents)
                if callback is not None:
                    env = {"latents": latents, "prompt_embeds": prompt_embeds}
                    out = callback(self, i, timesteps[i], {k: env[k] for k in callback_inputs})
                    if "latents" in out:
                        latents = out.pop("latents").to(torch.bfloat16).contiguous()
                        lat32 = latents.to(torch.float32)
                    if "prompt_embeds" in out:
                        prompt_embeds = out.pop("prompt_embeds")
                        static_t, static_c = prepare_static(prompt_embeds)
                if i == len(tvals) - 1 or ((i + 1) > num_warmup and (i + 1) % self.scheduler.order == 0):
                    bar.update()
        self._master_latents = lat32
        return latents
```

### arabic-text-image-generation-reptext_amd/torch_ops.py

```python
from __future__ import annotations

import os
from typing import Optional

import torch

from . import ops

_LIB = "reptext_amd"
_direct = {}


def _register():
    if getattr(torch.ops, _LIB, None) is not None and hasattr(torch.ops.reptext_amd, "linear"):
        return
    co = torch.library.custom_op

    @co(f"{_LIB}::linear", mutates_args=("out",), device_types="cuda")
    def linear(a: torch.Tensor, w: torch.Tensor, out: torch.Tensor, bias: Optional[torch.Tensor] = None,
               gate: Optional[torch.Tensor] = None, res: Optional[torch.Tensor] = None, add2: Optional[torch.Tensor] = None,
               rowscale: Optional[torch.Tensor] = None, gelu_from: int = -1, alpha: float = 1.0) -> None:
        _direct["linear"](a, w, out, bias=bias, gate=gate, res=res, add2=add2, rowscale=rowscale,
                          gelu_from=None if gelu_from < 0 else gelu_from, alpha=alpha)

    @co(f"{_LIB}::attention", mutates_args=("out",), device_types="cuda")
    def attention(q: torch.Tensor, k: torch.Tensor, v: torch.Tensor, out: torch.Tensor, heads: int, scale: float = 0.0) -> None:
        _direct["attention"](q, k, v, out, heads, None if scale == 0.0 else scale)

    @co(f"{_LIB}::layernorm_modulate", mutates_args=("out",), device_types="cuda")
    def layernorm_modulate(x: torch.Tensor, out: torch.Tensor, shift: Optional[torch.Tensor] = None, scale: Optional[torch.Tensor] = None,
                           eps: float = 1e-6) -> None:
        _direct["layernorm_modulate"](x, out, shift, scale, eps)

    @co(f"{_LIB}::qk_rmsnorm_rope", mutates_args=("buf",), device_types="cuda")
    def qk_rmsnorm_rope(buf: torch.Tensor, q_off: int, k_off: int, heads: int, text_rows: int, wq_txt: Optional[torch.Tensor],
                        wk_txt: Optional[torch.Tensor], wq_img: torch.Tensor, wk_img: torch.Tensor, cos: torch.Tensor, sin: torch.Tensor,
                        eps: float = 1e-6) -> None:
        _direct["qk_rmsnorm_rope"](buf, q_off, k_off, heads, text_rows, wq_txt, wk_txt, wq_img, wk_img, cos, sin, eps)

    @co(f"{_LIB}::gemv", mutates_args=("out",), device_types="cuda")
    def gemv(x: torch.Tensor, w: torch.Tensor, bias: Optional[torch.Tensor], out: torch.Tensor, silu_in: bool = False,
             silu_out: bool = False, accumulate: bool = False) -> None:
        _direct["gemv"](x, w, bias, out, silu_in=silu_in, silu_out=silu_out, accumulate=accumulate)

    @co(f"{_LIB}::euler_step_f32", mutates_args=("x32", "x_bf16"), device_types="cuda")
    def euler_step_f32(x32: torch.Tensor, v: torch.Tensor, dsigma: float, x_bf16: Optional[torch.Tensor] = None) -> None:
        _direct["euler_step_f32_"](x32, v, dsigma, x_bf16)


for _name in ("linear", "attention", "layernorm_modulate", "qk_rmsnorm_rope", "gemv", "euler_step_f32_"):
    _direct[_name] = getattr(ops, _name)
_register()


def enable_dispatch(on: bool = True) -> None:
    t = torch.ops.reptext_amd
    if on:
        def linear(a, w, out, bias=None, gate=None, res=None, add2=None, rowscale=None, rows_per_batch=0, gelu_from=None, alpha=1.0, **kw):
            if rows_per_batch or any(v is not None for v in kw.values()):
                return _direct["linear"](a, w, out, bias=bias, gate=gate, res=res, add2=add2, rowscale=rowscale, rows_per_batch=rows_per_batch,
                                         gelu_from=gelu_from, alpha=alpha, **kw)
            t.linear(a, w, out, bias, gate, res, add2, rowscale, -1 if gelu_from is None else int(gelu_from), float(alpha))
            return out

        ops.linear = linear
        ops.attention = lambda q, k, v, out, H, scale=None, split=True: (t.attention(q, k, v, out, H, 0.0 if scale is None else float(scale)) if split
                                                                          else _direct["attention"](q, k, v, out, H, scale, split=False)) or out
        ops.layernorm_modulate = lambda x, out, shift, scale, eps=1e-6: t.layernorm_modulate(x, out, shift, scale, eps) or out
        ops.qk_rmsnorm_rope = lambda buf, q_off, k_off, H, T, a, b, c, d, cos, sin, eps=1e-6: t.qk_rmsnorm_rope(buf, q_off, k_off, H, T, a, b, c, d, cos, sin, eps)
    else:
        for name in ("linear", "attention", "layernorm_modulate", "qk_rmsnorm_rope"):
            setattr(ops, name, _direct[name])


if os.environ.get("RT_USE_TORCH_OPS", "0") == "1":
    enable_dispatch(True)
```

### include/reptext_hip.h

```cpp
#ifndef REPTEXT_HIP_H
#define REPTEXT_HIP_H

#include <stdint.h>

#ifdef __cplusplus
extern "C" {
#endif

#define RT_OK 0
#define RT_E_BADARG (-1)
#define RT_E_ALIGN (-2)
#define RT_E_SHAPE (-3)

const char* rt_version(void);
int rt_abi_version(void);

#define RT_GEMM_MAX_GROUPS 4

typedef struct rt_gemm_group {
  const void* A;
  const void* W;
  void* C;
  const void* bias;
  const float* gate;
  const void* res;
  const void* add2;
  const float* rowscale;
  int64_t lda, ldw, ldc, ldr, ld2, gate_ld;
  int64_t strideA, strideC, strideR, stride2;
  int32_t M, N, K;
  int32_t batch;
  int32_t rows_per_batch;
  int32_t gelu_from;
  int32_t out_f32;
  float alpha;
  const float* a_scale;
  const float* w_scale;
  int64_t stride_rowscale;
  const uint8_t* a_bscale;
  int64_t a_bscale_plane, a_bscale_rows;
  uint8_t* c8;
  uint8_t* c_bscale;
  int64_t ldc8, stride_c8, c_bscale_plane, c_bscale_rows;
  int32_t c8_from, c_bscale_k0;
  int32_t conv_ks, conv_cin, conv_w2, conv_h2;
  float conv_inv_w2, conv_inv_h2;
  const float* rope_cos;
  const float* rope_sin;
  const void* rope_wq;
  const void* rope_wk;
  int32_t rope_q0, rope_k0, rope_w, rope_pos0;
  float rope_eps;
  int32_t rope_reserved;
} rt_gemm_group;

int rt_gemm_bf16(const rt_gemm_group* groups , int32_t ngroups, void* stream);

typedef struct rt_skinny_group {
  const void* W;
  const void* bias;
  float* C;
  int64_t ldw, ldc;
  int32_t N;
  int32_t reserved;
} rt_skinny_group;
int rt_gemm_skinny_bf16(const void* hi, const void* lo, int64_t lda, int32_t M, int32_t K,
                        const rt_skinny_group* groups , int32_t ngroups, void* stream);

int rt_gemm_fp8(const rt_gemm_group* groups , int32_t ngroups, void* stream);

int rt_quantize_rows_fp8(const void* x, int64_t ldx, int32_t x_f32, void* out, int64_t ldo, float* scale,
                         int32_t rows, int32_t D, void* stream);

int rt_quantize_mx_fp8(const void* x, int64_t ldx, int32_t x_f32, void* out, int64_t ldo, uint8_t* bscale, int64_t plane,
                       int32_t rows, int32_t D, void* stream);

int rt_gemv_bf16w(const float* x, int64_t ldx, const void* W, int64_t ldw, const void* bias,
                  float* y, int64_t ldy, int32_t B, int32_t N, int32_t K,
                  int32_t silu_in, int32_t silu_out, int32_t accumulate, void* stream);

int rt_add_rows_f32(float* y, const float* a, const float* b, int32_t rows, int32_t B, int32_t D, void* stream);

int rt_timestep_embedding(const float* t, float* out, int32_t B, int32_t dim, void* stream);

int rt_rope_table(const float* ids, float* cos_out, float* sin_out, int32_t S,
                  const int32_t* axes_dim , float theta, void* stream);

int rt_layernorm_modulate(const void* x, int64_t ldx, int64_t stride_xb, int32_t x_f32,
                          void* out, int64_t ldo, int64_t stride_ob,
                          const float* shift, const float* scale, int64_t mod_ld,
                          int32_t batch, int32_t rows_per_batch, int32_t D, float eps, void* stream);
typedef struct rt_ln_segment {
  const void* x;
  void* out;
  const float* shift;
  const float* scale;
  int64_t ldx, stride_xb, ldo, stride_ob, mod_ld;
  int32_t batch, rows_per_batch;
} rt_ln_segment;
int rt_layernorm_modulate_pair(const rt_ln_segment* segs , int32_t x_f32, int32_t D, float eps, void* stream);
int rt_layernorm_modulate_fp8(const void* x, int64_t ldx, int64_t stride_xb, int32_t x_f32,
                              void* out, int64_t ldo, int64_t stride_ob, float* row_scale,
                              const float* shift, const float* scale, int64_t mod_ld,
                              int32_t batch, int32_t rows_per_batch, int32_t D, float eps, void* stream);

int rt_qk_rmsnorm_rope(void* buf, int64_t ld, int64_t stride_b, int64_t q_off, int64_t k_off,
                       const void* wq_txt, const void* wk_txt, const void* wq_img, const void* wk_img,
                       const float* cosv, const float* sinv,
                       int32_t B, int32_t S, int32_t T, int32_t H, float eps, void* stream);

int64_t rt_attention_ws_bytes(int32_t B, int32_t S, int32_t H);
int rt_attention_fwd(const void* q, const void* k, const void* v, void* o,
                     int64_t ld, int64_t stride_b, int64_t ldo, int64_t stride_ob,
                     int32_t B, int32_t S, int32_t H, float scale,
                     void* ws, int64_t ws_bytes, void* stream);

int rt_attention_variant(int32_t mode);

int64_t rt_attention_fp8_vt_bytes(int32_t B, int32_t S, int32_t H);
int rt_attention_fp8_prep(const void* buf, int64_t ld, int64_t stride_b, int64_t q_off, int64_t k_off, int64_t v_off,
                          const void* wq_txt, const void* wk_txt, const void* wq_img, const void* wk_img,
                          const float* cosv, const float* sinv, void* qk8, void* vt8,
                          int32_t B, int32_t S, int32_t T, int32_t H, float eps, void* stream);
int rt_attention_fp8_fwd(const void* qk8, const void* vt8, void* o, int64_t ldo, int64_t stride_ob,
                         int32_t B, int32_t S, int32_t H, float scale, void* stream);
int rt_attention_fp8_fwd_mx(const void* qk8, const void* vt8, void* o8, int64_t ldo8, int64_t stride_ob8, uint8_t* bscale,
                            int64_t plane, int64_t bscale_rows, int32_t bscale_k0, int32_t B, int32_t S, int32_t H, float scale,
                            void* stream);

typedef struct rt_lora_term {
  const void* B;
  const void* At;
  int64_t ldb, lda;
  int32_t r_pad;
  float scale;
} rt_lora_term;
#define RT_LORA_MAX_TERMS 8
int rt_lora_merge_bf16(const rt_lora_term* terms , int32_t nterms, const void* W0, int64_t ld0,
                       void* W, int64_t ldw, int32_t N, int32_t K, void* stream);

int rt_ip_attention(const void* q, int64_t ldq, int64_t stride_qb, const void* wq,
                    const void* k, const void* v, int64_t ldkv, int64_t stride_kvb,
                    void* o, int64_t ldo, int64_t stride_ob, int32_t o_f32, int32_t accumulate,
                    int32_t B, int32_t N, int32_t H, int32_t n_ip, float sm_scale, float ip_scale, float eps, void* stream);
int rt_ip_attention_gated(const void* q, int64_t ldq, int64_t stride_qb, const void* wq,
                          const void* k, const void* v, int64_t ldkv, int64_t stride_kvb,
                          const float* gate, int64_t stride_gb,
                          void* o, int64_t ldo, int64_t stride_ob, int32_t o_f32, int32_t accumulate,
                          int32_t B, int32_t N, int32_t H, int32_t n_ip, float sm_scale, float ip_scale, float eps, void* stream);
int rt_gelu_erf_bf16(const float* x, void* y, int64_t n, void* stream);
int rt_add_bf16_2d(const void* x, int64_t ldx, int64_t stride_xb, void* y, int64_t ldy, int64_t stride_yb,
                   int32_t batch, int32_t rows, int32_t D, void* stream);

int rt_embedding_gather(const void* table, int64_t ld, const int32_t* ids, void* out, int64_t ldo,
                        int32_t n, int32_t D, int32_t vocab, void* stream);
int rt_rmsnorm_rows(const void* x, int64_t ldx, int32_t x_f32, const void* w, void* out, int64_t ldo,
                    int32_t rows, int32_t D, float eps, void* stream);
int rt_softmax_rows_bias(const float* s, int64_t lds, const float* bias, int64_t ldb, void* p, int64_t ldp,
                         int32_t rows, int32_t cols, int32_t cols_out, float scale, void* stream);
int rt_gated_mul(const void* x, int64_t ldx, void* out, int64_t ldo, int32_t rows, int32_t F, void* stream);
int rt_quick_gelu(void* x, int64_t n, void* stream);

#define RT_ATTENTION_HD64_MAX_S 4096
int rt_attention_hd64(const void* q, const void* k, const void* v, int64_t ld, int64_t stride_b,
                      void* o, int64_t ldo, int64_t stride_ob,
                      int32_t B, int32_t S, int32_t H, float scale, void* stream);
int rt_patchify_nchw(const void* x, int32_t x_f32, void* out, int32_t B, int32_t G, int32_t p, int32_t Kp, void* stream);

#define RT_ATTENTION_HD72_MAX_S 1024
int rt_attention_hd72(const void* q, int64_t ldq, int64_t stride_qb,
                      const void* k, const void* v, int64_t ldkv, int64_t stride_kvb,
                      void* o, int64_t ldo, int64_t stride_ob,
                      int32_t B, int32_t Sq, int32_t Sk, int32_t H, float scale, void* stream);

int rt_euler_step(void* x, const void* v, float dsigma, int64_t n, void* stream);

int rt_euler_step_f32(float* x, const void* v, void* x_bf16 , float dsigma, int64_t n, void* stream);

int rt_cfg_mix(const void* v_uncond, const void* v_text, void* out, float s, int64_t n, void* stream);

int rt_pack_latents(const void* nchw, void* packed, int32_t B, int32_t C, int32_t H2, int32_t W2, void* stream);
int rt_unpack_latents(const void* packed, void* nhwc, int32_t B, int32_t C, int32_t H2, int32_t W2,
                      float inv_scale, float shift, void* stream);

int rt_cast_f32_to_bf16(const float* x, void* y, int64_t n, void* stream);
int rt_cast_bf16_to_f32(const void* x, float* y, int64_t n, void* stream);
int rt_silu_split_bf16(const float* x, void* hi, void* lo, int64_t n, int32_t apply_silu, void* stream);
int rt_masked_accumulate(const void* x, void* y, const float* rowscale, float alpha,
                         int32_t batch, int32_t rows, int32_t D, int32_t accumulate, int32_t y_f32, void* stream);

int64_t rt_groupnorm_ws_bytes(int32_t B, int32_t H, int32_t W, int32_t G);
int rt_groupnorm_silu_nhwc(const void* x, void* y, const void* gamma, const void* beta, void* stats_ws,
                           int32_t B, int32_t H, int32_t W, int32_t C, int32_t G, float eps, int32_t silu, void* stream);
int rt_conv2d_nhwc(const void* x, const void* w, const void* bias, const void* res, void* y,
                   int32_t B, int32_t Hs, int32_t Ws, int32_t Cin, int32_t Cout, int32_t ksize, int32_t stride,
                   int32_t upsample2x, int32_t out_f32, void* stream);
int rt_conv2d_variant(int32_t mode);
int rt_softmax_rows(const float* s, void* p, int32_t rows, int32_t cols, float scale, void* stream);
int rt_vae_attention(const void* q, const void* k, const void* v, void* o, int64_t ld, int64_t stride_b, int64_t ldo, int64_t stride_ob,
                     int32_t B, int32_t HW, int32_t C, float scale, void* stream);
int rt_transpose_bf16(const void* in, void* out, int32_t R, int32_t C, int64_t ld_in, int64_t ld_out, void* stream);
int rt_image_out(const float* x, float* nchw, uint8_t* u8, int32_t B, int32_t H, int32_t W, int32_t Cp, int32_t C, void* stream);
int rt_nchw_to_haloed_nhwc(const float* x, void* y, int32_t B, int32_t C, int32_t H, int32_t W, int32_t Cp, void* stream);
int rt_haloed_nhwc_to_nchw(const void* x, float* y, int32_t B, int32_t C, int32_t H, int32_t W, int32_t Cp, void* stream);
int rt_unpack_latents_haloed(const void* packed, void* y, int32_t B, int32_t C, int32_t H2, int32_t W2, int32_t Cp,
                             float inv_scale, float shift, void* stream);


int rt_resize2d(const void* in, int32_t in_u8, float in_scale, float* out, int32_t planes, int32_t H, int32_t W, int32_t OH, int32_t OW,
                float scale_h, float scale_w, int32_t bilinear, void* stream);
int rt_glyph_blend(const float* image, const float* latents, const float* noise, float* out, int32_t B, int32_t Cimg, int32_t H, int32_t W,
                   int32_t Cl, int32_t OH, int32_t OW, void* stream);

int64_t rt_canny_ws_bytes(int32_t H, int32_t W);
int rt_canny_u8(const uint8_t* img, int32_t H, int32_t W, int32_t C, float low, float high, uint8_t* out, int32_t out_channels,
                int32_t invert, void* ws, int64_t ws_bytes, void* stream);
int rt_preprocess_u8(const uint8_t* img, float* out, int32_t B, int32_t H, int32_t W, int32_t C, int32_t normalize, void* stream);

#ifdef __cplusplus
}
#endif
#endif
```

Baseline: 0.5095 images/sec.

## Restrict last ControlNet double block to mask's active image-row window

Computes the bounding row span of the nonzero mask rows, caching it by tensor identity. When that span covers at most half the image, the last evaluated tower double block runs attention, out-proj and FFN only for query rows inside the window, and the head writes only those rows. Rows outside the window are multiplied by a zero row scale anyway, so the skipped work should not change the output. The attention kernels gain a templated row-range skip, and sample buffers are zeroed whenever the window changes. The cost is extra complexity, a host sync to read the span, and a dependence on mask sparsity that may not hold for the test hint.

```diff
diff --git a/arabic-text-image-generation-reptext_amd/controlnet.py b/arabic-text-image-generation-reptext_amd/controlnet.py
--- a/arabic-text-image-generation-reptext_amd/controlnet.py
+++ b/arabic-text-image-generation-reptext_amd/controlnet.py
@@ -1,5 +1,6 @@
 from __future__ import annotations
 
+from collections import OrderedDict
 from dataclasses import dataclass
 from typing import Any, Dict, List, Optional, Sequence, Tuple, Union
 
@@ -21,6 +22,42 @@
     def __iter__(self):
         yield self.controlnet_block_samples
         yield self.controlnet_single_block_samples
+
+
+ROW_WINDOW_ALIGN = 16
+_ROW_SPAN_CACHE: "OrderedDict" = OrderedDict()
+
+
+def _nonzero_row_span(mask: torch.Tensor) -> Optional[Tuple[int, int]]:
+    key = (mask.data_ptr(), tuple(mask.shape), tuple(mask.stride()), str(mask.dtype), str(mask.device), mask._version)
+    hit = _ROW_SPAN_CACHE.get(key)
+    if hit is not None:
+        _ROW_SPAN_CACHE.move_to_end(key)
+        return hit[0]
+    m = mask.reshape(mask.shape[0], -1) if mask.dim() == 3 else mask.reshape(1, -1) if mask.dim() == 1 else mask
+    nz = (m != 0).any(dim=0)
+    pos = torch.arange(nz.numel(), device=nz.device)
+    lo, hi = torch.stack([torch.where(nz, pos, nz.numel()).min(), torch.where(nz, pos, -1).max()]).tolist()
+    span = None if hi < 0 else (int(lo), int(hi))
+    _ROW_SPAN_CACHE[key] = (span, mask)
+    while len(_ROW_SPAN_CACHE) > 8:
+        _ROW_SPAN_CACHE.popitem(last=False)
+    return span
+
+
+def active_row_window(masks: Sequence[torch.Tensor], N: int) -> Optional[Tuple[int, int]]:
+    lo, hi = N, -1
+    for m in masks:
+        if m.numel() == 0 or m.numel() % N:
+            return None
+        span = _nonzero_row_span(m)
+        if span is not None:
+            lo, hi = min(lo, span[0]), max(hi, span[1])
+    if hi < 0:
+        return None
+    a = ROW_WINDOW_ALIGN
+    r0, r1 = lo // a * a, min(N, (hi + a) // a * a)
+    return None if (r1 - r0) * 2 > N else (r0, r1)
 
 
 class FluxControlNetModel(_MMDiTBase):
@@ -107,6 +144,9 @@
             why = f"in-features {lin.in_features} are not a multiple of 64: the K-padded copy of _padded_hint would go stale"
         return why
 
+    def supports_row_window(self) -> bool:
+        return not getattr(self, "_fp8_linears", False) and not getattr(self, "_fp8_attention", False)
+
     def _invalidate_derived(self):
         self._cx_pad = None
 
@@ -133,7 +173,8 @@
                 _rowscale: Optional[torch.Tensor] = None, _accumulate_into: Optional[Sequence[torch.Tensor]] = None,
                 _accumulate_single_into: Optional[Sequence[torch.Tensor]] = None, _mods: Optional["mmdit.StepMods"] = None,
                 _overwrite: bool = False, _sample_events: Optional[Sequence["torch.cuda.Event"]] = None, _ws_tag: str = "",
-                _static: Optional[StaticEmbeds] = None, _blocks_needed: Optional[Tuple[int, int]] = None):
+                _static: Optional[StaticEmbeds] = None, _blocks_needed: Optional[Tuple[int, int]] = None,
+                _window: Optional[Tuple[int, int]] = None):
         doubles, singles = self._ensure_plans()
         self._apply_lora_scale(joint_attention_kwargs)
         cfg = self.config
@@ -167,8 +208,13 @@
         scale = float(conditioning_scale)
 
         def head(lin, dst_list, i):
-            a = mmdit.image_rows_bf16(ws)
-            if dst_list is not None:
+            a = mmdit.image_rows_bf16(ws, _window)
+            if _window is not None:
+                r0, r1 = _window
+                out = dst_list[i]
+                ops.linear(a, lin.weight.data, out[:, r0:r1], bias=lin.bias.data, alpha=scale, rowscale=_rowscale[..., r0:r1],
+                           res=None if _overwrite else out[:, r0:r1])
+            elif dst_list is not None:
                 out = dst_list[i]
                 ops.linear(a, lin.weight.data, out, bias=lin.bias.data, alpha=scale, rowscale=_rowscale, res=None if _overwrite else out)
             else:
@@ -180,12 +226,19 @@
         ns = len(singles) if _blocks_needed is None else min(len(singles), int(_blocks_needed[1]))
         if ns > 0:
             nd = len(doubles)
+        if _window is not None:
+            if _rowscale is None or _accumulate_into is None or ns > 0 or nd < 1 or not self.supports_row_window():
+                raise ValueError("_window needs a row scale, sample buffers and a bf16 tower whose single blocks are not evaluated")
+            _window = (int(_window[0]), int(_window[1]))
+            if not (0 <= _window[0] < _window[1] <= N):
+                raise ValueError(f"_window {_window} is not inside the {N} image rows")
         block_samples: List[Optional[torch.Tensor]] = []
         for i, pl in enumerate(doubles):
             if i >= nd:
                 block_samples.append(None)
                 continue
-            mmdit.run_double(pl, ws, temb, cos, sin, H, mods=None if _mods is None else _mods.double[i])
+            mmdit.run_double(pl, ws, temb, cos, sin, H, mods=None if _mods is None else _mods.double[i],
+                             window=_window if i == nd - 1 else None)
             block_samples.append(head(self.controlnet_blocks[i], _accumulate_into, i))
             if _sample_events is not None:
                 _sample_events[i].record(torch.cuda.current_stream())
diff --git a/arabic-text-image-generation-reptext_amd/csrc/attention.hip b/arabic-text-image-generation-reptext_amd/csrc/attention.hip
--- a/arabic-text-image-generation-reptext_amd/csrc/attention.hip
+++ b/arabic-text-image-generation-reptext_amd/csrc/attention.hip
@@ -21,7 +21,7 @@
 __global__ __launch_bounds__(ATT_THREADS, 2) void attention_fwd_kernel(
     const bf16_t* __restrict__ Q, const bf16_t* __restrict__ K, const bf16_t* __restrict__ V, bf16_t* O,
     int64_t ld, int64_t stride_b, int64_t ldo, int64_t stride_ob, float scale_log2, const SplitGeom G,
-    int* counters, char* records) {
+    const int row_lo, const int row_hi, int* counters, char* records) {
   __shared__ __attribute__((aligned(16))) char smem[4 * TILE_B];
   const int tid = threadIdx.x;
   const int lane = tid & 63;
@@ -85,6 +85,7 @@
     if (te <= tb) break;
     const int head = item / G.nqb;
     const int q0 = (item - head * G.nqb) * BQ;
+    if (q0 + BQ <= row_lo || q0 >= row_hi) continue;
     const bf16_t* Qb = Q + b * stride_b + head * DH;
     const bf16_t* Kb = K + b * stride_b + head * DH;
     const bf16_t* Vb = V + b * stride_b + head * DH;
@@ -385,10 +386,19 @@
 
 extern "C" int rt_attention_variant(int32_t mode) { return rt_attention_v3_mode(mode); }
 
+extern "C" int rt_attention_fwd_rows(const void* q, const void* k, const void* v, void* o, int64_t ld, int64_t stride_b, int64_t ldo,
+                                     int64_t stride_ob, int32_t B, int32_t S, int32_t H, float scale, int32_t row_lo, int32_t row_hi, void* ws,
+                                     int64_t ws_bytes, void* stream);
 extern "C" int rt_attention_fwd(const void* q, const void* k, const void* v, void* o, int64_t ld, int64_t stride_b,
                                 int64_t ldo, int64_t stride_ob, int32_t B, int32_t S, int32_t H, float scale,
                                 void* ws, int64_t ws_bytes, void* stream) {
-  if (!q || !k || !v || !o || B < 1 || S < 1 || H < 1) return RT_E_BADARG;
+  return rt_attention_fwd_rows(q, k, v, o, ld, stride_b, ldo, stride_ob, B, S, H, scale, 0, S, ws, ws_bytes, stream);
+}
+
+extern "C" int rt_attention_fwd_rows(const void* q, const void* k, const void* v, void* o, int64_t ld, int64_t stride_b,
+                                     int64_t ldo, int64_t stride_ob, int32_t B, int32_t S, int32_t H, float scale,
+                                     int32_t row_lo, int32_t row_hi, void* ws, int64_t ws_bytes, void* stream) {
+  if (!q || !k || !v || !o || B < 1 || S < 1 || H < 1 || row_lo < 0 || row_hi > S || row_lo >= row_hi) return RT_E_BADARG;
   if (!RT_ALIGNED(q, 16) || !RT_ALIGNED(k, 16) || !RT_ALIGNED(v, 16) || !RT_ALIGNED(o, 8) || ld % 8 || stride_b % 8 ||
       ldo % 4 || stride_ob % 4)
     return RT_E_ALIGN;
@@ -397,7 +407,7 @@
   if (!split_fits_32bit(make_geom(S, H, true))) return RT_E_SHAPE;
   {
     int taken = 0;
-    const int st = rt_attention_v3_try(q, k, v, o, ld, stride_b, ldo, stride_ob, B, S, H, scale, ws, ws_bytes, stream, &taken);
+    const int st = rt_attention_v3_try(q, k, v, o, ld, stride_b, ldo, stride_ob, B, S, H, scale, row_lo, row_hi, ws, ws_bytes, stream, &taken);
     if (taken || st != RT_OK) return st;
   }
   const int64_t need = rt_attention_ws_bytes(B, S, H);
@@ -409,7 +419,7 @@
   const dim3 grid(8 * wmax, B);
   hipLaunchKernelGGL(attention_fwd_kernel, grid, dim3(ATT_THREADS), 0, (hipStream_t)stream, (const bf16_t*)q,
                      (const bf16_t*)k, (const bf16_t*)v, (bf16_t*)o, ld, stride_b, ldo, stride_ob,
-                     scale * 1.4426950408889634f, G, split ? (int*)ws : nullptr,
+                     scale * 1.4426950408889634f, G, row_lo, row_hi, split ? (int*)ws : nullptr,
                      split ? (char*)ws + split_cnt_bytes(B, S, H) : nullptr);
   return rt_hip_status();
 }
diff --git a/arabic-text-image-generation-reptext_amd/csrc/attention_split.h b/arabic-text-image-generation-reptext_amd/csrc/attention_split.h
--- a/arabic-text-image-generation-reptext_amd/csrc/attention_split.h
+++ b/arabic-text-image-generation-reptext_amd/csrc/attention_split.h
@@ -110,5 +110,6 @@
 
 int64_t rt_attention_v3_ws_bytes(int32_t B, int32_t S, int32_t H);
 int rt_attention_v3_try(const void* q, const void* k, const void* v, void* o, int64_t ld, int64_t stride_b, int64_t ldo, int64_t stride_ob,
-                        int32_t B, int32_t S, int32_t H, float scale, void* ws, int64_t ws_bytes, void* stream, int* taken);
+                        int32_t B, int32_t S, int32_t H, float scale, int32_t row_lo, int32_t row_hi, void* ws, int64_t ws_bytes, void* stream,
+                        int* taken);
 int rt_attention_v3_mode(int mode);
diff --git a/arabic-text-image-generation-reptext_amd/csrc/attention_v3.hip b/arabic-text-image-generation-reptext_amd/csrc/attention_v3.hip
--- a/arabic-text-image-generation-reptext_amd/csrc/attention_v3.hip
+++ b/arabic-text-image-generation-reptext_amd/csrc/attention_v3.hip
@@ -81,10 +81,11 @@
 constexpr int REC3_WAVE_B = 8 * 16 * 64 * 4 + 64 * 16;
 constexpr int REC3_B = 4 * REC3_WAVE_B;
 
+template <bool ROWS>
 __global__ __launch_bounds__(V3_THREADS, 1) void attention_v3_kernel(const bf16_t* __restrict__ Q, const bf16_t* __restrict__ K,
                                                                      const bf16_t* __restrict__ V, bf16_t* O, int64_t ld, int64_t stride_b,
                                                                      int64_t ldo, int64_t stride_ob, float scale_log2, const SplitGeom G,
-                                                                     int* counters, char* records) {
+                                                                     int* counters, char* records, const int row_lo, const int row_hi) {
   extern __shared__ __attribute__((aligned(16))) char smem[];
   const int tid = threadIdx.x;
   const int lane = tid & 63;
@@ -124,6 +125,7 @@
     }
     const int head = item / G.nqb;
     const int q0 = (item - head * G.nqb) * BQ3;
+    if (ROWS && (q0 + BQ3 <= row_lo || q0 >= row_hi)) continue;
     const bf16_t* Qb = Q + b * stride_b + head * DH;
     const rt_srd_t rsrcK = rt_make_srd(K + b * stride_b + head * DH), rsrcV = rt_make_srd(V + b * stride_b + head * DH);
     const uint32_t wdst = lds0 + wave * 4096;
@@ -459,7 +461,8 @@
 }
 
 int rt_attention_v3_try(const void* q, const void* k, const void* v, void* o, int64_t ld, int64_t stride_b, int64_t ldo, int64_t stride_ob,
-                        int32_t B, int32_t S, int32_t H, float scale, void* ws, int64_t ws_bytes, void* stream, int* taken) {
+                        int32_t B, int32_t S, int32_t H, float scale, int32_t row_lo, int32_t row_hi, void* ws, int64_t ws_bytes, void* stream,
+                        int* taken) {
   *taken = 0;
   if (!v3_mode_now() || S % BQ3 != 0 || (ldo % 8) || (stride_ob % 8) || !RT_ALIGNED(o, 16)) return RT_OK;
   if (v3_mode_now() == 1 && S < 1536) return RT_OK;
@@ -469,11 +472,13 @@
   if (!split_fits_32bit(G)) return RT_OK;
   *taken = 1;
   const int lds = NSTAGE * STAGE_B;
-  static bool attr_done = false;
-  if (!attr_done) {
-    hipError_t e = hipFuncSetAttribute(reinterpret_cast<const void*>(attention_v3_kernel), hipFuncAttributeMaxDynamicSharedMemorySize, lds);
+  const bool ranged = row_lo > 0 || row_hi < S;
+  auto kernel = ranged ? attention_v3_kernel<true> : attention_v3_kernel<false>;
+  static bool attr_done[2] = {false, false};
+  if (!attr_done[ranged]) {
+    hipError_t e = hipFuncSetAttribute(reinterpret_cast<const void*>(kernel), hipFuncAttributeMaxDynamicSharedMemorySize, lds);
     if (e != hipSuccess) return (int)e;
-    attr_done = true;
+    attr_done[ranged] = true;
   }
   int slots = 0;
   for (int x = 0; x < 8; ++x) {
@@ -481,9 +486,9 @@
     const int s = c.rem ? G.spx : (c.nfull < G.spx ? c.nfull : G.spx);
     slots = s > slots ? s : slots;
   }
-  hipLaunchKernelGGL(attention_v3_kernel, dim3(8 * slots, B), dim3(V3_THREADS), lds, (hipStream_t)stream, (const bf16_t*)q, (const bf16_t*)k,
-                     (const bf16_t*)v, (bf16_t*)o, ld, stride_b, ldo, stride_ob, scale * 1.4426950408889634f, G, split ? (int*)ws : nullptr,
-                     split ? (char*)ws + split_cnt_bytes(B, S, H) : nullptr);
+  hipLaunchKernelGGL(kernel, dim3(8 * slots, B), dim3(V3_THREADS), lds, (hipStream_t)stream, (const bf16_t*)q, (const bf16_t*)k,
+                     (const bf16_t*)v, (bf16_t*)o, ld, stride_b, ldo, stride_ob, scale * 1.4426950408889634f, G,
+                     split ? (int*)ws : nullptr, split ? (char*)ws + split_cnt_bytes(B, S, H) : nullptr, (int)row_lo, (int)row_hi);
   return rt_hip_status();
 }
 
diff --git a/arabic-text-image-generation-reptext_amd/mmdit.py b/arabic-text-image-generation-reptext_amd/mmdit.py
--- a/arabic-text-image-generation-reptext_amd/mmdit.py
+++ b/arabic-text-image-generation-reptext_amd/mmdit.py
@@ -310,8 +310,13 @@
 
 
 def run_double(pl: DoublePlan, ws: Workspace, temb: torch.Tensor, cos, sin, H: int, inject: Optional[torch.Tensor] = None,
-               mods: Optional[tuple] = None, ip: Optional[tuple] = None, ip_inside: bool = False) -> None:
+               mods: Optional[tuple] = None, ip: Optional[tuple] = None, ip_inside: bool = False,
+               window: Optional[tuple] = None) -> None:
     T, d = ws.T, ws.d
+    if window is not None:
+        if ip is not None or inject is not None or pl.qkv_img_w8 is not None or pl.fp8_attention or pl.mx:
+            raise ValueError("run_double: the windowed mode is the bf16 path without ip / inject")
+        return _run_double_window(pl, ws, temb, cos, sin, H, mods, int(window[0]), int(window[1]))
     x_t, x_i = ws.x[:, :T], ws.x[:, T:]
     xn_t, xn_i = ws.xn[:, :T], ws.xn[:, T:]
     if mods is not None:
@@ -400,6 +405,36 @@
             ops.masked_accumulate_(ws.x[b, T:].unsqueeze(0), ip_out[b : b + 1], None, 1.0, True)
 
 
+def _run_double_window(pl: DoublePlan, ws: Workspace, temb, cos, sin, H: int, mods: Optional[tuple], r0: int, r1: int) -> None:
+    T, d = ws.T, ws.d
+    if not (0 <= r0 < r1 <= ws.N):
+        raise ValueError(f"window [{r0}, {r1}) is not inside the {ws.N} image rows")
+    x_t, x_i = ws.x[:, :T], ws.x[:, T:]
+    xn_t, xn_i = ws.xn[:, :T], ws.xn[:, T:]
+    if mods is not None:
+        mi, mt = mods
+    else:
+        mi, mt = ws.mod_a, ws.mod_b
+        ops.gemv(temb, pl.ada_img_w, pl.ada_img_b, mi, silu_in=True)
+        ops.gemv(temb, pl.ada_txt_w, pl.ada_txt_b, mt, silu_in=True)
+    ch = lambda m, i: m[:, i * d : (i + 1) * d]
+    ops.layernorm_modulate_pair(x_i, xn_i, ch(mi, 0), ch(mi, 1), x_t, xn_t, ch(mt, 0), ch(mt, 1))
+    fused_rope = FUSED_QK_ROPE and ops.QKRope.covers(d)
+    ri = ops.QKRope(0, d, d, pl.nq_img, pl.nk_img, cos, sin, pos0=T) if fused_rope else None
+    rt = ops.QKRope(0, d, d, pl.nq_txt, pl.nk_txt, cos, sin, pos0=0) if fused_rope else None
+    ops.linear_grouped([P(xn_i, pl.qkv_img_w, ws.qkv[:, T:], bias=pl.qkv_img_b, rope=ri), P(xn_t, pl.qkv_txt_w, ws.qkv[:, :T], bias=pl.qkv_txt_b, rope=rt)])
+    if not fused_rope:
+        ops.qk_rmsnorm_rope(ws.qkv, 0, d, H, T, pl.nq_txt, pl.nk_txt, pl.nq_img, pl.nk_img, cos, sin)
+    q, k, v = ws.qkv[..., :d], ws.qkv[..., d : 2 * d], ws.qkv[..., 2 * d :]
+    ops.attention(q, k, v, q, H, rows=(T + r0, T + r1))
+    qw = q[:, T + r0 : T + r1]
+    xw, xnw, hw = x_i[:, r0:r1], xn_i[:, r0:r1], ws.ffh[:, T + r0 : T + r1]
+    ops.linear(qw, pl.out_img_w, xw, bias=pl.out_img_b, gate=ch(mi, 2), res=xw)
+    ops.layernorm_modulate(xw, xnw, ch(mi, 3), ch(mi, 4))
+    ops.linear(xnw, pl.ff1_img_w, hw, bias=pl.ff1_img_b, gelu_from=0)
+    ops.linear(hw, pl.ff2_img_w, xw, bias=pl.ff2_img_b, gate=ch(mi, 5), res=xw)
+
+
 def run_single(pl: SinglePlan, ws: Workspace, temb: torch.Tensor, cos, sin, H: int, inject: Optional[torch.Tensor] = None,
                mods: Optional[torch.Tensor] = None, ip: Optional[tuple] = None) -> None:
     T, d = ws.T, ws.d
@@ -453,11 +488,12 @@
             ops.masked_accumulate_(ws.x[b, T:].unsqueeze(0), inject[b : b + 1].contiguous(), None, 1.0, True)
 
 
-def image_rows_bf16(ws: Workspace) -> torch.Tensor:
+def image_rows_bf16(ws: Workspace, rows: Optional[tuple] = None) -> torch.Tensor:
     T = ws.T
+    r0, r1 = (0, ws.N) if rows is None else (int(rows[0]), int(rows[1]))
     if ws.x.dtype == BF16:
-        return ws.x[:, T:]
+        return ws.x[:, T + r0 : T + r1]
     for b in range(ws.B):
-        src, dst = ws.x[b, T:], ws.xn[b, T:]
+        src, dst = ws.x[b, T + r0 : T + r1], ws.xn[b, T + r0 : T + r1]
         native.check("rt_cast_f32_to_bf16", native.load().rt_cast_f32_to_bf16(src.data_ptr(), dst.data_ptr(), src.numel(), ops._stream()))
-    return ws.xn[:, T:]
+    return ws.xn[:, T + r0 : T + r1]
diff --git a/arabic-text-image-generation-reptext_amd/native.py b/arabic-text-image-generation-reptext_amd/native.py
--- a/arabic-text-image-generation-reptext_amd/native.py
+++ b/arabic-text-image-generation-reptext_amd/native.py
@@ -138,6 +138,8 @@
 RT_ATTENTION_HD72_MAX_S = 1024
 SIGNATURES["rt_attention_hd72"] = [_vp, _i64, _i64, _vp, _vp, _i64, _i64, _vp, _i64, _i64, _i32, _i32, _i32, _i32, _f32, _vp]
 
+SIGNATURES["rt_attention_fwd_rows"] = [_vp, _vp, _vp, _vp, _i64, _i64, _i64, _i64, _i32, _i32, _i32, _f32, _i32, _i32, _vp, _i64, _vp]
+
 SIGNATURES["rt_gemm_skinny_bf16"] = [_vp, _vp, _i64, _i32, _i32, C.POINTER(SkinnyGroup), _i32, _vp]
 SIGNATURES["rt_layernorm_modulate_pair"] = [C.POINTER(LnSegment), _i32, _i32, _f32, _vp]
 SIGNATURES["rt_add_rows_f32"] = [_vp, _vp, _vp, _i32, _i32, _i32, _vp]
diff --git a/arabic-text-image-generation-reptext_amd/ops.py b/arabic-text-image-generation-reptext_amd/ops.py
--- a/arabic-text-image-generation-reptext_amd/ops.py
+++ b/arabic-text-image-generation-reptext_amd/ops.py
@@ -477,7 +477,7 @@
 
 
 def attention(q: torch.Tensor, k: torch.Tensor, v: torch.Tensor, out: torch.Tensor, H: int, scale: Optional[float] = None,
-              split: bool = True) -> torch.Tensor:
+              split: bool = True, rows: Optional[tuple] = None) -> torch.Tensor:
     for name, t in (("q", q), ("k", k), ("v", v), ("out", out)):
         if t.dim() != 3 or t.stride(2) != 1 or t.shape[2] != H * 128:
             raise ValueError(f"{name}: need [B,S,{H*128}] with unit inner stride")
@@ -486,9 +486,10 @@
         raise ValueError("q,k,v must share shape and strides")
     sc = (128 ** -0.5) if scale is None else float(scale)
     ws = _attention_workspace(B, S, H, q.device) if split else None
-    native.check("rt_attention_fwd", native.load().rt_attention_fwd(
+    r0, r1 = (0, S) if rows is None else (int(rows[0]), int(rows[1]))
+    native.check("rt_attention_fwd_rows", native.load().rt_attention_fwd_rows(
         _dev(q, "q", BF16), _dev(k, "k", BF16), _dev(v, "v", BF16), _dev(out, "out", BF16), q.stride(1), q.stride(0),
-        out.stride(1), out.stride(0), B, S, H, sc, None if ws is None else ws.data_ptr(), 0 if ws is None else ws.numel(), _stream()))
+        out.stride(1), out.stride(0), B, S, H, sc, r0, r1, None if ws is None else ws.data_ptr(), 0 if ws is None else ws.numel(), _stream()))
     return out
 
 
diff --git a/arabic-text-image-generation-reptext_amd/pipeline.py b/arabic-text-image-generation-reptext_amd/pipeline.py
--- a/arabic-text-image-generation-reptext_amd/pipeline.py
+++ b/arabic-text-image-generation-reptext_amd/pipeline.py
@@ -13,7 +13,7 @@
 import torch.nn.functional as F
 
 from . import ops
-from .controlnet import FluxControlNetModel, FluxMultiControlNetModel
+from .controlnet import FluxControlNetModel, FluxMultiControlNetModel, active_row_window
 from .image_processor import PipelineImageInput, VaeImageProcessor
 from .scheduler import FlowMatchEulerDiscreteScheduler, calculate_shift
 from .transformer import FluxTransformer2DModel
@@ -81,6 +81,7 @@
 
 OVERLAP_TOWER = os.environ.get("RT_OVERLAP_TOWER", "1") == "1"
 GRAPH_CAPTURE = os.environ.get("RT_GRAPH", "1") == "1"
+TOWER_WINDOW = os.environ.get("RT_TOWER_WINDOW", "1") == "1"
 GRAPH_CACHE_MAX = 2
 
 
@@ -666,10 +667,12 @@
                  cn_scale, cn_steps, control_mode, callback, callback_inputs, num_inference_steps):
         tvals = timesteps.to(torch.float32).cpu().tolist()
         ipe = getattr(self, "_ip_embeds", None)
+        win = active_row_window(masks, latents.shape[1]) if masks and len(masks) == len(hints) else None
 
         def eager(callback=None):
             return self._denoise_eager(latents, prompt_embeds, pooled, text_ids, image_ids, tvals, hints, masks, guidance_scale, cn_scale,
-                                       cn_steps, control_mode, callback, callback_inputs, num_inference_steps, timesteps, _ip_embeds=ipe)
+                                       cn_steps, control_mode, callback, callback_inputs, num_inference_steps, timesteps, _ip_embeds=ipe,
+                                       _tower_window=win)
 
         use_graph = (GRAPH_CAPTURE and getattr(self, "capture_graphs", True) and callback is None and latents.is_cuda
                      and not self.interrupt and isinstance(self.controlnet, (FluxControlNetModel, type(None)))
@@ -683,7 +686,8 @@
                         bool(getattr(m, "_fp8_attention", False))) for m in (self.transformer, self.controlnet) if m is not None)
         key = (sig(latents), sig(prompt_embeds), sig(pooled), sig(text_ids), sig(image_ids), tuple(sig(h) for h in hints), tuple(sig(m) for m in masks),
                tuple(tvals), tuple(self.scheduler.sigmas.tolist()), float(guidance_scale), repr(cn_scale), int(cn_steps), int(num_inference_steps),
-               str(latents.device), models, bool(self.reference_bf16_scalars), bool(_mm.RESIDUAL_F32), bool(OVERLAP_TOWER), bool(_mm.FUSED_QK_ROPE))
+               str(latents.device), models, bool(self.reference_bf16_scalars), bool(_mm.RESIDUAL_F32), bool(OVERLAP_TOWER), bool(_mm.FUSED_QK_ROPE),
+               win, bool(TOWER_WINDOW))
         if ipe is not None:
             adapter = self.transformer._ip_adapter
             key += (sig(ipe), adapter.version, tuple(adapter.scales))
@@ -710,7 +714,7 @@
                 with torch.cuda.graph(graph, capture_error_mode="thread_local"):
                     out = self._denoise_eager(static[0], static[1], static[2], static[3], static[4], tvals, static[5 : 5 + nh], static[5 + nh : 5 + nh + nm],
                                               guidance_scale, cn_scale, cn_steps, control_mode, None, callback_inputs, num_inference_steps, timesteps,
-                                              _quiet=True, _ip_embeds=static[-1] if ipe is not None else None)
+                                              _quiet=True, _ip_embeds=static[-1] if ipe is not None else None, _tower_window=win)
                     out32 = self._master_latents
             except Exception as e:
                 import sys
@@ -718,6 +722,8 @@
                 cache[key] = "failed"
                 _mm.CAPTURE_KEEP = ops.CAPTURE_KEEP = None
                 ops.drop_attention_workspaces(set(ops._ATTN_WS) - attn_keys)
+                if getattr(self, "_sample_cache", None) is not None:
+                    self._sample_cache[3][0] = None
                 torch.cuda.synchronize()
                 self.scheduler._step_index = step_index
                 return eager()
@@ -725,10 +731,12 @@
             keep.append(getattr(self, "_sample_cache", None))
             keep.extend(dict(m._rope_cache) for m in (self.transformer, self.controlnet) if m is not None and hasattr(m, "_rope_cache"))
             self.scheduler._step_index = step_index
-            ent = cache[key] = {"graph": graph, "static": static, "out": out, "out32": out32, "keep": keep}
+            ent = cache[key] = {"graph": graph, "static": static, "out": out, "out32": out32, "keep": keep,
+                                "samples": getattr(self, "_sample_cache", None), "window": self._tower_window_used}
         for dst, src in zip(ent["static"], ins):
             if dst.data_ptr() != src.data_ptr():
                 dst.copy_(src)
+        self._zero_samples_for(ent["samples"], ent["window"])
         ent["graph"].replay()
         self.scheduler._step_index = (self.scheduler._step_index or 0) + len(tvals)
         self._master_latents = ent["out32"].clone()
@@ -736,9 +744,19 @@
             bar.update(num_inference_steps)
         return ent["out"].clone()
 
+    @staticmethod
+    def _zero_samples_for(cache, window) -> None:
+        if cache is None:
+            return
+        state = cache[3]
+        if window is not None and state[0] != window:
+            for buf in cache[1]:
+                buf.zero_()
+        state[0] = window
+
     def _denoise_eager(self, latents, prompt_embeds, pooled, text_ids, image_ids, tvals, hints, masks, guidance_scale,
                        cn_scale, cn_steps, control_mode, callback, callback_inputs, num_inference_steps, timesteps, _quiet=False,
-                       _ip_embeds=None, _extra_towers=(), _velocity=None):
+                       _ip_embeds=None, _extra_towers=(), _velocity=None, _tower_window=None):
         device = latents.device
         B = latents.shape[0]
         guidance = torch.full((B,), float(guidance_scale), device=device, dtype=torch.float32) if self.transformer.config.guidance_embeds else None
@@ -773,8 +791,15 @@
             key = (Bc, N_, d_, n_cd, n_cs, str(device))
             if getattr(self, "_sample_cache", None) is None or self._sample_cache[0] != key:
                 mk = lambda n: [torch.empty(Bc, N_, d_, device=device, dtype=torch.bfloat16) for _ in range(n)]
-                self._sample_cache = (key, mk(n_cd), mk(n_cs))
+                self._sample_cache = (key, mk(n_cd), mk(n_cs), [None])
             sample_buf, single_buf = self._sample_cache[1], self._sample_cache[2]
+        window = None
+        if (TOWER_WINDOW and _tower_window is not None and towers and not _extra_towers and blocks_needed is not None
+                and blocks_needed[0] >= 1 and blocks_needed[1] == 0 and self.controlnet.supports_row_window()):
+            window = _tower_window
+        self._tower_window_used = window
+        if fused_cn:
+            self._zero_samples_for(self._sample_cache, window)
         lat32 = latents.to(torch.float32).contiguous()
         latents = latents.to(torch.bfloat16).contiguous().clone()
         overlap = (OVERLAP_TOWER and bool(towers) and not _extra_towers and device.type == "cuda"
@@ -803,7 +828,7 @@
                                 txt_ids=text_ids, img_ids=image_ids, joint_attention_kwargs=self.joint_attention_kwargs,
                                 return_dict=False, _rowscale=rowscale, _accumulate_into=sample_buf, _accumulate_single_into=single_buf,
                                 _overwrite=(k == 0), _sample_events=events if k == len(towers) - 1 else None, _mods=table.step(i),
-                                _ws_tag="tower" if overlap else "", _static=static, _blocks_needed=blocks_needed)
+                                _ws_tag="tower" if overlap else "", _static=static, _blocks_needed=blocks_needed, _window=window)
                             if k == 0:
                                 merged, merged_single = samples
                 noise_pred = self.transformer(
diff --git a/arabic-text-image-generation-reptext_amd/torch_ops.py b/arabic-text-image-generation-reptext_amd/torch_ops.py
--- a/arabic-text-image-generation-reptext_amd/torch_ops.py
+++ b/arabic-text-image-generation-reptext_amd/torch_ops.py
@@ -64,8 +64,9 @@
             return out
 
         ops.linear = linear
-        ops.attention = lambda q, k, v, out, H, scale=None, split=True: (t.attention(q, k, v, out, H, 0.0 if scale is None else float(scale)) if split
-                                                                          else _direct["attention"](q, k, v, out, H, scale, split=False)) or out
+        ops.attention = lambda q, k, v, out, H, scale=None, split=True, rows=None: (
+            t.attention(q, k, v, out, H, 0.0 if scale is None else float(scale)) if split and rows is None
+            else _direct["attention"](q, k, v, out, H, scale, split=split, rows=rows)) or out
         ops.layernorm_modulate = lambda x, out, shift, scale, eps=1e-6: t.layernorm_modulate(x, out, shift, scale, eps) or out
         ops.qk_rmsnorm_rope = lambda buf, q_off, k_off, H, T, a, b, c, d, cos, sin, eps=1e-6: t.qk_rmsnorm_rope(buf, q_off, k_off, H, T, a, b, c, d, cos, sin, eps)
     else:
diff --git a/include/reptext_hip.h b/include/reptext_hip.h
--- a/include/reptext_hip.h
+++ b/include/reptext_hip.h
@@ -115,6 +115,11 @@
                      int32_t B, int32_t S, int32_t H, float scale,
                      void* ws, int64_t ws_bytes, void* stream);
 
+int rt_attention_fwd_rows(const void* q, const void* k, const void* v, void* o,
+                          int64_t ld, int64_t stride_b, int64_t ldo, int64_t stride_ob,
+                          int32_t B, int32_t S, int32_t H, float scale, int32_t row_lo, int32_t row_hi,
+                          void* ws, int64_t ws_bytes, void* stream);
+
 int rt_attention_variant(int32_t mode);
 
 int64_t rt_attention_fp8_vt_bytes(int32_t B, int32_t S, int32_t H);
```

Measured after the change: 0.5171 images/sec, median of 6. +1.5%, better.
